# tusen-ai/RangeDet

Measured on AMD Instinct MI355X. Metric: range-image frames/sec (64x2650, 8ch) at 1/2/4/8 GPU; Meta-Kernel HBM GB/s vs peak, higher is better.
Workload: dtype bf16

## Files before the change

rangedet_amd/csrc/k_block.h:

```cpp
#pragma once
#include "k_conv3.h"

namespace rd {

struct BlockArgs {
  const bf16_t* x; int x_cs, x_co; long x_bs;
  const unsigned char* w;
  const float* shift1; const float* shift2;
  const unsigned char* scw;
  bf16_t* y; int y_cs, y_co; long y_bs;
  const unsigned char* zero16;
  int H, W, B, ncol, nrow, ntiles, xcd;
  int nslots1;
};

constexpr int BK_R = 6;
constexpr int BK_XP = 36;
constexpr int BK_XPIECES = 7;
constexpr int BK_BUF = 4 * BK_XPIECES * 1024;
constexpr int BK_TP = 34;
constexpr int BK_SLAB = 4096;
constexpr size_t BK_LDS = 2 * BK_BUF + BK_R * BK_SLAB;

constexpr int bk_nsteps(bool first) { return first ? 23 : 36; }
constexpr int bk_unit(bool first, int g) { return first ? (g < 5 ? 0 : g < 14 ? 2 : 3) : g / 9; }
constexpr int bk_ord(bool first, int g) { return first ? (g < 5 ? g : (g - 5) % 9) : g % 9; }
constexpr bool bk_fetches(bool first, int g) { return bk_unit(first, g) == 3 || (!first && bk_unit(first, g) == 0); }
constexpr int bk_pieces_u(int s) { return s <= 1 ? 2 : s <= 4 ? 1 : 0; }
constexpr int bk_first_u(int s) { int n = 0; for (int t = 0; t < s; ++t) n += bk_pieces_u(t); return n; }
constexpr int bk_pieces(bool first, int g) { return bk_fetches(first, g) ? bk_pieces_u(bk_ord(first, g)) : 0; }
constexpr int bk_younger(bool first, int g) {
  const int G = bk_nsteps(first);
  int n = BK_R - 3;
  for (int d = 1; d <= BK_R - 2; ++d) n += bk_pieces(first, ((g - d) % G + G) % G);
  const int cap = 9 - 3 - 4;
  return (bk_fetches(first, g) && bk_ord(first, g) == 7 && n > cap) ? cap : n;
}

template <int DT, bool SC, bool FIRST = false, bool M16 = false>
__global__ __launch_bounds__(256, 2) void block64_stream_kernel(BlockArgs a) {
  static_assert(!FIRST || SC, "the first block changes the channel count: projection shortcut");
  static_assert(!(FIRST && M16), "the first block (five two-tap steps on one 16-channel slot) stays in the 32 x 32 x 16 form");
  HIP_DYNAMIC_SHARED(unsigned char, smem);
  constexpr int R = BK_R, SLAB = BK_SLAB, RING = 2 * BK_BUF, NCT = 2;
  constexpr int ROWB2 = BK_TP * 64;
  const int tid = threadIdx.x, lane = tid & 63, wave = __builtin_amdgcn_readfirstlane(tid >> 6);
  const int m = lane & 31, hi = lane >> 5;

  unsigned bz1[NCT], bz2[NCT];
#pragma unroll
  for (int j = 0; j < NCT; ++j) {
    const float t1 = a.shift1[32 * j + conv_row_perm(m)], t2 = a.shift2[32 * j + conv_row_perm(m)];
    const bf16_t h1 = H16<DT>::from_f32(t1), h2 = H16<DT>::from_f32(t2);
    const bf16_t l1 = H16<DT>::from_f32(t1 - H16<DT>::to_f32(h1)), l2 = H16<DT>::from_f32(t2 - H16<DT>::to_f32(h2));
    bz1[j] = hi ? 0u : ((unsigned)h1 | ((unsigned)l1 << 16));
    bz2[j] = hi ? 0u : ((unsigned)h2 | ((unsigned)l2 << 16));
  }

  unsigned bz1m = 0u, bz2m = 0u;
  if constexpr (M16) {
    const float t1 = a.shift1[conv_row16(lane >> 4, lane & 15)], t2 = a.shift2[conv_row16(lane >> 4, lane & 15)];
    const bf16_t h1 = H16<DT>::from_f32(t1), h2 = H16<DT>::from_f32(t2);
    const bf16_t l1 = H16<DT>::from_f32(t1 - H16<DT>::to_f32(h1)), l2 = H16<DT>::from_f32(t2 - H16<DT>::to_f32(h2));
    bz1m = (unsigned)h1 | ((unsigned)l1 << 16);
    bz2m = (unsigned)h2 | ((unsigned)l2 << 16);
  }

  const int G = gridDim.x, wg = blockIdx.x;
  const int ntl = (a.ntiles - wg + G - 1) / G;
  const int tiles_img = a.ncol * a.nrow;

#if defined(__HIP_DEVICE_COMPILE__)
  const unsigned lds0 = __builtin_amdgcn_readfirstlane((unsigned)(uintptr_t)(__attribute__((address_space(3))) void*)smem);
#endif
  auto dma_s = [&](const unsigned char* sbase, unsigned voff, int lds_off) {
#if defined(__HIP_DEVICE_COMPILE__)
    asm volatile("s_mov_b32 m0, %2\n\ts_nop 0\n\tglobal_load_lds_dwordx4 %0, %1"
                 :: "v"(voff), "s"(sbase), "s"(__builtin_amdgcn_readfirstlane(lds0 + (unsigned)lds_off)) : "memory");
#else
    __builtin_amdgcn_global_load_lds(sbase + voff, smem + lds_off, 16, 0, 0);
#endif
  };
  auto dma_v = [&](const void* vptr, int lds_off) {
#if defined(__HIP_DEVICE_COMPILE__)
    asm volatile("s_mov_b32 m0, %1\n\ts_nop 0\n\tglobal_load_lds_dwordx4 %0, off"
                 :: "v"(vptr), "s"(__builtin_amdgcn_readfirstlane(lds0 + (unsigned)lds_off)) : "memory");
#else
    __builtin_amdgcn_global_load_lds(vptr, smem + lds_off, 16, 0, 0);
#endif
  };

  const int xdq = (G >> 3) / a.nrow;
  const int g_ct = a.xcd ? (8 * xdq) % a.ncol : G % a.ncol, g_rb = a.xcd ? (G >> 3) % a.nrow : (G / a.ncol) % a.nrow,
            g_b = a.xcd ? (8 * xdq) / a.ncol : G / tiles_img;
  const int g_ct1 = (8 * xdq + 8) % a.ncol, g_b1 = (8 * xdq + 8) / a.ncol;
  auto tile_advance = [&](int& ct, int& rb, int& b) __attribute__((always_inline)) {
    int& d0 = a.xcd ? rb : ct;
    int& d1 = a.xcd ? ct : rb;
    const int r0 = a.xcd ? a.nrow : a.ncol, r1 = a.xcd ? a.ncol : a.nrow;
    d0 += a.xcd ? g_rb : g_ct;
    const int c1 = d0 >= r0 ? 1 : 0;
    d0 -= c1 ? r0 : 0;
    d1 += a.xcd ? (c1 ? g_ct1 : g_ct) : g_rb + c1;
    const int c2 = d1 >= r1 ? 1 : 0;
    d1 -= c2 ? r1 : 0;
    b += (a.xcd && c1 ? g_b1 : g_b) + c2;
  };
  const int xs0 = ((wg >> 3) / a.nrow) * 8 + (wg & 7);
  int f_ct = a.xcd ? xs0 % a.ncol : wg % a.ncol, f_rb = a.xcd ? (wg >> 3) % a.nrow : (wg / a.ncol) % a.nrow,
      f_b = a.xcd ? xs0 / a.ncol : wg / tiles_img;
  int c_ct = f_ct, c_rb = f_rb, c_b = f_b;

  int hk = 0, hc = 0;
  int hh0 = 0, hw0 = 0;
  const unsigned char* htile = nullptr;
  const unsigned char* hbase = nullptr;
  bool hnew = true;
  auto halo_begin = [&]() {
    if (hnew) {
      hh0 = f_rb * 8 - 2; hw0 = f_ct * 32 - 2;
      htile = (const unsigned char*)(a.x + (size_t)f_b * a.x_bs + a.x_co) + ((long)hh0 * a.W + hw0) * (long)a.x_cs * 2;
      hnew = false;
    }
    hbase = htile + hc * 64;
    if (!FIRST && hc == 0) hc = 1;
    else if (hk + 1 < ntl) { ++hk; hc = 0; tile_advance(f_ct, f_rb, f_b); hnew = true; }
  };
  auto halo_piece = [&](int buf, int j) {
    const int q = wave * BK_XPIECES + j;
    int ol = lane;
    asm volatile("" : "+v"(ol));
    const int pp = 16 * q + (ol >> 2), r = (pp * 1821) >> 16, cc = pp - BK_XP * r;
    const int hs = (ol & 3) ^ ((ol >> 4) & 3);
    const bool ok = pp < 12 * BK_XP && (unsigned)(hh0 + r) < (unsigned)a.H && (unsigned)(hw0 + cc) < (unsigned)a.W && (!FIRST || hs < a.nslots1);
    const unsigned char* src = hbase + (long)((r * a.W + cc) * a.x_cs * 2 + hs * 16);
    dma_v(ok ? (const void*)src : (const void*)a.zero16, buf + q * 1024);
  };
  int fslot = 0, fslab = 0;
  auto slab_piece = [&]() { dma_s(a.w + (size_t)fslab * SLAB + wave * 1024, lane * 16, RING + fslot * SLAB + wave * 1024); };
  auto slab_advance = [&]() {
    fslot = fslot + 1 == R ? 0 : fslot + 1;
    fslab = fslab + 1 == bk_nsteps(FIRST) ? 0 : fslab + 1;
  };

  int a1[3][3], a2[3];
#pragma unroll
  for (int dh = 0; dh < 3; ++dh)
#pragma unroll
    for (int dw = 0; dw < 3; ++dw) {
      const int P = 96 * wave + m + BK_XP * dh + dw;
      a1[dh][dw] = P * 64 + (((hi ^ (P >> 2)) & 3) << 4);
    }
#pragma unroll
  for (int d = 0; d < 3; ++d) {
    const int c = d + m;
    a2[d] = c * 64 + (((hi ^ (c >> 2)) & 3) << 4) + wave * 2 * ROWB2;
  }
  if constexpr (M16) {
    const int n16 = lane & 15, q16 = lane >> 4;
#pragma unroll
    for (int dh = 0; dh < 3; ++dh)
#pragma unroll
      for (int dw = 0; dw < 3; ++dw) {
        const int P = 96 * wave + n16 + BK_XP * dh + dw;
        a1[dh][dw] = P * 64 + (((q16 ^ (P >> 2)) & 3) << 4);
      }
#pragma unroll
    for (int d = 0; d < 3; ++d) {
      const int c = d + n16;
      a2[d] = c * 64 + (((q16 ^ (c >> 2)) & 3) << 4) + wave * 2 * ROWB2;
    }
  }
  const int boff = RING + lane * 16;

  f32x16 acc[M16 ? 1 : 3][M16 ? 1 : NCT];
  f32x4 acc6[M16 ? 6 : 1][M16 ? 4 : 1];
  s16x8 fa[2][3], fb[2][NCT];
  s16x8 fa16[6];
#define BK_FENCE() __builtin_amdgcn_sched_barrier(0)
#define BK_RD(F, FS, BUF, K, AADDR, BADDR, KS)                                                              \
  {                                                                                                         \
    if ((K) == 0) fa[BUF][0] = *(const s16x8*)(smem + (AADDR));                                              \
    else if ((K) <= NCT) fb[BUF][(K) - 1] = *(const s16x8*)(smem + (BADDR) + ((KS) * NCT + (K) - 1) * 1024);  \
    else fa[BUF][(K) - NCT] = *(const s16x8*)(smem + (AADDR) + ((K) - NCT) * (FS));                          \
    BK_FENCE();                                                                                             \
  }
#define BK_MM(BUF, N)                                                                                       \
  {                                                                                                         \
    acc[(N) / NCT][(N) % NCT] = H16<DT>::mfma(fb[BUF][(N) % NCT], fa[BUF][(N) / NCT], acc[(N) / NCT][(N) % NCT]); \
    BK_FENCE();                                                                                             \
  }
#define BK_SYNC(VMCNT, LGKM)                                      \
  {                                                               \
    asm volatile("" ::: "memory");                                \
    __builtin_amdgcn_s_waitcnt(C3_WAIT_IMM(VMCNT, LGKM));         \
    __builtin_amdgcn_s_barrier();                                 \
    asm volatile("" ::: "memory");                                \
    BK_FENCE();                                                   \
  }
#define BK_STEP(F, FS, G_, HB_, NF_, NFS_, A1_, ANEXT_)                                                            \
  {                                                                                                                \
    constexpr int NM_ = (F) * NCT, NR_ = (F) + NCT, NRN_ = (NF_) ? (NF_) + NCT : 0;                                \
    constexpr int NH_ = bk_pieces(FIRST, G_), NP_ = 1 + NH_, HF_ = bk_first_u(bk_ord(FIRST, G_)), YG_ = bk_younger(FIRST, G_); \
    const int acur_ = (A1_);                                                                                       \
    const int bcur_ = boff + rslot * SLAB;                                                                         \
    const int rnext_ = rslot + 1 == R ? 0 : rslot + 1;                                                             \
    const int anext_ = (ANEXT_);                                                                                   \
    const int bnext_ = boff + rnext_ * SLAB;                                                                       \
    BK_FENCE();                                                                                                    \
    _Pragma("unroll") for (int n = 0; n < NM_; ++n) {                                                              \
      BK_MM(0, n)                                                                                                  \
      if (n < NR_) BK_RD(F, FS, 1, n, acur_, bcur_, 1)                                                             \
    }                                                                                                              \
    _Pragma("unroll") for (int n = 0; n < NM_ / 2; ++n) {                                                          \
      BK_MM(1, n)                                                                                                  \
      if (n < NRN_) BK_RD(NF_, NFS_, 0, n, anext_, bnext_, 0)                                                      \
    }                                                                                                              \
    { _Pragma("unroll") for (int n = NM_ / 2; n < NRN_; ++n) BK_RD(NF_, NFS_, 0, n, anext_, bnext_, 0) }           \
    BK_SYNC(YG_, NRN_)                                                                                             \
    if (NH_ > 0 && bk_ord(FIRST, G_) == 0) halo_begin();                                                           \
    _Pragma("unroll") for (int n = NM_ / 2; n < NM_; ++n) {                                                        \
      BK_MM(1, n)                                                                                                  \
      _Pragma("unroll") for (int p = 0; p < NP_; ++p)                                                              \
        if (p * (NM_ / 2) / NP_ == n - NM_ / 2) {                                                                  \
          if (p == 0) slab_piece(); else halo_piece(HB_, HF_ + p - 1);                                             \
          BK_FENCE();                                                                                              \
        }                                                                                                          \
    }                                                                                                              \
    slab_advance();                                                                                                \
    rslot = rnext_;                                                                                                \
  }
#define BK_C1(U_, S_)                                                                                              \
  BK_STEP(3, 2048, 9 * (U_) + (S_), BK_BUF, (((U_) == 1 && (S_) == 8) ? 0 : 3), 2048,                              \
          (a1[(S_) / 3][(S_) % 3] + (U_) * BK_BUF) ^ 32,                                                           \
          ((S_) == 8 ? a1[0][0] + BK_BUF : a1[(((S_) + 1) % 9) / 3][((S_) + 1) % 3] + (U_) * BK_BUF))
#define BK_P1(S_)                                                                                                  \
  BK_STEP(3, 2048, (S_), 0, ((S_) == 4 ? 0 : 3), 2048, a1[((2 * (S_) + 1) % 9) / 3][(2 * (S_) + 1) % 3],           \
          a1[((2 * (S_) + 2) % 9) / 3][(2 * (S_) + 2) % 3])
#define BK_C2(C_, S_)                                                                                              \
  BK_STEP(2, ROWB2, (FIRST ? 5 : 18) + 9 * (C_) + (S_), 0, (((C_) == 1 && (S_) == 8) ? 3 : 2), (((C_) == 1 && (S_) == 8) ? 2048 : ROWB2), \
          (a2[(S_) % 3] + ((S_) / 3) * ROWB2 + (C_) * BK_BUF) ^ 32,                                                \
          ((S_) == 8 ? ((C_) == 1 ? a1[0][0] : a2[0] + BK_BUF) : a2[((S_) + 1) % 3] + ((((S_) + 1) % 9) / 3) * ROWB2 + (C_) * BK_BUF))

#define BK_RDW16(BUF, C, BADDR) { fb[BUF][C] = *(const s16x8*)(smem + (BADDR) + (C) * 1024); BK_FENCE(); }
#define BK_RDP16(HX, AADDR, FS) { fa16[HX] = *(const s16x8*)(smem + (AADDR) + ((HX) >> 1) * (FS) + ((HX) & 1) * 1024); BK_FENCE(); }
#define BK_MM16(BK, N)                                                                                             \
  {                                                                                                                \
    acc6[(N) >> 1][2 * (BK) + ((N) & 1)] = H16<DT>::mfma16(fb[BK][(N) & 1], fa16[(N) >> 1], acc6[(N) >> 1][2 * (BK) + ((N) & 1)]); \
    BK_FENCE();                                                                                                    \
  }
#define BK_STEP16(F, G_, HB_, NF_, NFS_, ANEXT_)                                                                   \
  {                                                                                                                \
    constexpr int NM_ = 2 * (F);                                                                                   \
    constexpr int NX_ = (NF_) > (F) ? (NF_) - (F) : 0;                                                             \
    constexpr int LG_ = (NF_) ? 2 + NX_ + ((NF_) < (F) / 2 ? (NF_) : (F) / 2) : 0;                                 \
    constexpr int NH_ = bk_pieces(FIRST, G_), NP_ = 1 + NH_, HF_ = bk_first_u(bk_ord(FIRST, G_)), YG_ = bk_younger(FIRST, G_); \
    const int bcur_ = boff + rslot * SLAB;                                                                         \
    const int rnext_ = rslot + 1 == R ? 0 : rslot + 1;                                                             \
    const int anext_ = (ANEXT_);                                                                                   \
    const int bnext_ = boff + rnext_ * SLAB;                                                                       \
    BK_FENCE();                                                                                                    \
    _Pragma("unroll") for (int n = 0; n < NM_; ++n) {                                                              \
      BK_MM16(0, n)                                                                                                \
      if (n < 2) BK_RDW16(1, n, bcur_ + 2048)                                                                      \
    }                                                                                                              \
    _Pragma("unroll") for (int n = 0; n < NM_ / 2; ++n) {                                                          \
      BK_MM16(1, n)                                                                                                \
      if ((NF_) && n < 2) BK_RDW16(0, n, bnext_)                                                                   \
      if (n < NX_) BK_RDP16((F) + n, anext_, NFS_)                                                                 \
      if ((n & 1) && (n >> 1) < (NF_)) BK_RDP16(n >> 1, anext_, NFS_)                                              \
    }                                                                                                              \
    BK_SYNC(YG_, LG_)                                                                                              \
    if (NH_ > 0 && bk_ord(FIRST, G_) == 0) halo_begin();                                                           \
    _Pragma("unroll") for (int n = NM_ / 2; n < NM_; ++n) {                                                        \
      BK_MM16(1, n)                                                                                                \
      _Pragma("unroll") for (int p = 0; p < NP_; ++p)                                                              \
        if (p * (NM_ / 2) / NP_ == n - NM_ / 2) {                                                                  \
          if (p == 0) slab_piece(); else halo_piece(HB_, HF_ + p - 1);                                             \
          BK_FENCE();                                                                                              \
        }                                                                                                          \
      if ((n & 1) && (n >> 1) < (NF_) && (n >> 1) < (F)) BK_RDP16(n >> 1, anext_, NFS_)                            \
    }                                                                                                              \
    slab_advance();                                                                                                \
    rslot = rnext_;                                                                                                \
  }
#define BK_C1M(U_, S_)                                                                                             \
  BK_STEP16(6, 9 * (U_) + (S_), BK_BUF, (((U_) == 1 && (S_) == 8) ? 0 : 6), 2048,                                  \
            ((S_) == 8 ? a1[0][0] + BK_BUF : a1[(((S_) + 1) % 9) / 3][((S_) + 1) % 3] + (U_) * BK_BUF))
#define BK_C2M(C_, S_)                                                                                             \
  BK_STEP16(4, 18 + 9 * (C_) + (S_), 0, (((C_) == 1 && (S_) == 8) ? 6 : 4), (((C_) == 1 && (S_) == 8) ? 2048 : ROWB2), \
            ((S_) == 8 ? ((C_) == 1 ? a1[0][0] : a2[0] + BK_BUF) : a2[((S_) + 1) % 3] + ((((S_) + 1) % 9) / 3) * ROWB2 + (C_) * BK_BUF))

  halo_begin();
#pragma unroll
  for (int j = 0; j < BK_XPIECES; ++j) halo_piece(0, j);
#pragma unroll 1
  for (int s0 = 0; s0 < R; ++s0) { slab_piece(); slab_advance(); }
  BK_SYNC(0, 0)
  int rslot = 0;
  if constexpr (M16) {
#pragma unroll
    for (int kk = 0; kk < 2; ++kk) BK_RDW16(0, kk, boff + rslot * SLAB)
#pragma unroll
    for (int kk = 0; kk < 6; ++kk) BK_RDP16(kk, a1[0][0], 2048)
  } else {
#pragma unroll
  for (int kk = 0; kk < 3 + NCT; ++kk) BK_RD(3, 2048, 0, kk, a1[0][0], boff + rslot * SLAB, 0)
  }

  for (int k = 0; k < ntl; ++k) {
    if constexpr (M16) {
      unsigned z0 = 0u, b1 = bz1m, b2 = bz2m;
      int oq = lane >> 4;
      asm volatile("" : "+v"(z0), "+v"(b1), "+v"(b2), "+v"(oq));
      typedef short s16x2 __attribute__((ext_vector_type(2)));
      typedef float f32x2 __attribute__((ext_vector_type(2)));
      auto init_acc = [&](unsigned bz, int NH) {
#pragma unroll
        for (int cb = 0; cb < 4; ++cb) {
          unsigned ob[4] = {oq == cb ? H16<DT>::ONE * 0x10001u : z0, z0, z0, z0};
          unsigned ab[4] = {bz, z0, z0, z0};
          s16x8 ones, bzv;
          memcpy(&ones, ob, 16);
          memcpy(&bzv, ab, 16);
          acc6[0][cb] = H16<DT>::mfma16(bzv, ones, f32x4{});
          BK_FENCE();
        }
#pragma unroll
        for (int h = 1; h < 6; ++h)
          if (h < NH) {
#pragma unroll
            for (int cb = 0; cb < 4; ++cb) acc6[h][cb] = acc6[0][cb];
          }
        BK_FENCE();
      };
      init_acc(b1, 6);
      BK_C1M(0, 0) BK_C1M(0, 1) BK_C1M(0, 2) BK_C1M(0, 3) BK_C1M(0, 4) BK_C1M(0, 5) BK_C1M(0, 6) BK_C1M(0, 7) BK_C1M(0, 8)
      BK_C1M(1, 0) BK_C1M(1, 1) BK_C1M(1, 2) BK_C1M(1, 3) BK_C1M(1, 4) BK_C1M(1, 5) BK_C1M(1, 6) BK_C1M(1, 7) BK_C1M(1, 8)
      const int ct = c_ct, rb = c_rb, b = c_b;
      tile_advance(c_ct, c_rb, c_b);
      {
        int el = lane;
        asm volatile("" : "+v"(el));
        const int en = el & 15, eq = el >> 4;
#pragma unroll
        for (int h = 0; h < 6; ++h) {
          const int J = 96 * wave + 16 * h + en, rr = (J * 1821) >> 16, cc = J - BK_XP * rr;
          const bool keep = cc < BK_TP && rr < 10;
          const bool inside = (unsigned)(rb * 8 - 1 + rr) < (unsigned)a.H && (unsigned)(ct * 32 - 1 + cc) < (unsigned)a.W;
          const int doff = (rr * BK_TP + cc) * 64 + (((eq ^ (cc >> 2)) & 3) << 4);
#pragma unroll
          for (int j = 0; j < 2; ++j) {
            BK_FENCE();
            unsigned pk[4];
#pragma unroll
            for (int w2 = 0; w2 < 4; ++w2) {
              const f32x4 av = acc6[h][2 * j + (w2 >> 1)];
              unsigned p2 = H16<DT>::pk(av[2 * (w2 & 1)], av[2 * (w2 & 1) + 1]);
              p2 = __builtin_bit_cast(unsigned, __builtin_elementwise_max(__builtin_bit_cast(s16x2, p2), (s16x2){0, 0}));
              pk[w2] = inside ? p2 : 0u;
            }
            if (keep) *(Slot16*)(smem + j * BK_BUF + doff) = Slot16{pk[0], pk[1], pk[2], pk[3]};
          }
        }
      }
      init_acc(b2, 4);
      BK_SYNC(63, 0)
#pragma unroll
      for (int kk = 0; kk < 2; ++kk) BK_RDW16(0, kk, boff + rslot * SLAB)
#pragma unroll
      for (int kk = 0; kk < 4; ++kk) BK_RDP16(kk, a2[0], ROWB2)
      BK_C2M(0, 0) BK_C2M(0, 1) BK_C2M(0, 2) BK_C2M(0, 3) BK_C2M(0, 4) BK_C2M(0, 5) BK_C2M(0, 6) BK_C2M(0, 7) BK_C2M(0, 8)
      BK_C2M(1, 0) BK_C2M(1, 1) BK_C2M(1, 2) BK_C2M(1, 3) BK_C2M(1, 4) BK_C2M(1, 5) BK_C2M(1, 6) BK_C2M(1, 7) BK_C2M(1, 8)
      {
        const int oh0 = rb * 8 + 2 * wave;
        int el = lane;
        asm volatile("" : "+v"(el));
        const int en = el & 15, eq = el >> 4;
        unsigned char* scr = smem + BK_BUF + wave * (BK_BUF / 4);
        bf16_t* __restrict__ yrow0 = a.y + (size_t)b * a.y_bs + (size_t)oh0 * a.W * a.y_cs + a.y_co;
        const bf16_t* __restrict__ rimg0 = a.x + (size_t)b * a.x_bs + a.x_co;
        if constexpr (SC) {
          const unsigned char* __restrict__ wq = a.scw + el * 16;
          s16x8 sxq[4][2];
#pragma unroll
          for (int h = 0; h < 4; ++h) {
            const int ow = ct * 32 + 16 * (h & 1) + en, oh = oh0 + (h >> 1);
            const bool live = ow < a.W && oh < a.H;
            const bf16_t* sp = rimg0 + (live ? ((size_t)oh * a.W + ow) * a.x_cs : 0) + 8 * eq;
#pragma unroll
            for (int ks = 0; ks < 2; ++ks) sxq[h][ks] = *(const s16x8*)(sp + 32 * ks);
          }
#pragma unroll
          for (int ks = 0; ks < 2; ++ks)
#pragma unroll
            for (int cb = 0; cb < 4; ++cb) {
              const s16x8 wf = *(const s16x8*)(wq + (size_t)(ks * 4 + cb) * 1024);
#pragma unroll
              for (int h = 0; h < 4; ++h) acc6[h][cb] = H16<DT>::mfma16(wf, sxq[h][ks], acc6[h][cb]);
            }
          BK_FENCE();
        }
        Slot16 rv[2][2][2];
        auto res_load = [&](int i, Slot16 (&dst)[2][2]) {
#pragma unroll
          for (int hf = 0; hf < 2; ++hf) {
            const int ow = ct * 32 + 16 * hf + en, oh = oh0 + i;
            const bool live = ow < a.W && oh < a.H;
            const bf16_t* rp = rimg0 + (live ? ((size_t)oh * a.W + (size_t)ow) * a.x_cs : 0) + 8 * eq;
#pragma unroll
            for (int p2 = 0; p2 < 2; ++p2) dst[hf][p2] = *(const Slot16*)(rp + 32 * p2);
          }
        };
        if constexpr (!SC) res_load(0, rv[0]);
#pragma unroll
        for (int i = 0; i < 2; ++i) {
          if constexpr (!SC) { if (i + 1 < 2) res_load(i + 1, rv[(i + 1) & 1]); }
#pragma unroll
          for (int hf = 0; hf < 2; ++hf)
#pragma unroll
            for (int p2 = 0; p2 < 2; ++p2) {
              BK_FENCE();
              unsigned pk[4];
#pragma unroll
              for (int w2 = 0; w2 < 4; ++w2) {
                const f32x4 av = acc6[2 * i + hf][2 * p2 + (w2 >> 1)];
                f32x2 v = {av[2 * (w2 & 1)], av[2 * (w2 & 1) + 1]};
                if constexpr (!SC) v += H16<DT>::unpk(rv[i & 1][hf][p2][w2]);
                const unsigned q2 = H16<DT>::pk(v[0], v[1]);
                pk[w2] = __builtin_bit_cast(unsigned, __builtin_elementwise_max(__builtin_bit_cast(s16x2, q2), (s16x2){0, 0}));
              }
              const int px = 16 * hf + en;
              *(Slot16*)(scr + px * 128 + (((4 * p2 + eq) ^ (px & 7)) << 4)) = Slot16{pk[0], pk[1], pk[2], pk[3]};
            }
          BK_FENCE();
          __builtin_amdgcn_wave_barrier();
#pragma unroll
          for (int it = 0; it < 4; ++it) {
            const int pr = it * 8 + el / 8, sl = el % 8;
            const Slot16 v = *(const Slot16*)(scr + pr * 128 + ((sl ^ (pr & 7)) << 4));
            const int ows = ct * 32 + pr;
            if (ows < a.W && oh0 + i < a.H)
              __builtin_nontemporal_store(v, (Slot16*)(yrow0 + (size_t)i * a.W * a.y_cs + (size_t)ows * a.y_cs + sl * 8));
          }
          __builtin_amdgcn_wave_barrier();
          BK_FENCE();
        }
      }
    } else {
    unsigned z0 = 0u;
    asm volatile("" : "+v"(z0));
    const unsigned one2 = hi ? z0 : H16<DT>::ONE * 0x10001u;
    s16x8 ones;
    {
      unsigned ob[4] = {one2, z0, z0, z0};
      memcpy(&ones, ob, 16);
    }
#pragma unroll
    for (int n = 0; n < 3 * NCT; ++n) {
      unsigned ab[4] = {bz1[n % NCT], z0, z0, z0};
      s16x8 bz;
      memcpy(&bz, ab, 16);
      acc[n / NCT][n % NCT] = H16<DT>::mfma(bz, ones, f32x16{});
    }
    BK_FENCE();
    if constexpr (FIRST) {
      BK_P1(0) BK_P1(1) BK_P1(2) BK_P1(3) BK_P1(4)
    } else {
      BK_C1(0, 0) BK_C1(0, 1) BK_C1(0, 2) BK_C1(0, 3) BK_C1(0, 4) BK_C1(0, 5) BK_C1(0, 6) BK_C1(0, 7) BK_C1(0, 8)
      BK_C1(1, 0) BK_C1(1, 1) BK_C1(1, 2) BK_C1(1, 3) BK_C1(1, 4) BK_C1(1, 5) BK_C1(1, 6) BK_C1(1, 7) BK_C1(1, 8)
    }

    const int ct = c_ct, rb = c_rb, b = c_b;
    tile_advance(c_ct, c_rb, c_b);
    {
      int em = m, ehi = hi;
      asm volatile("" : "+v"(em), "+v"(ehi));
      typedef short s16x2 __attribute__((ext_vector_type(2)));
#pragma unroll
      for (int i = 0; i < 3; ++i) {
        const int J = 96 * wave + 32 * i + em, rr = (J * 1821) >> 16, cc = J - BK_XP * rr;
        const bool keep = cc < BK_TP && rr < 10;
        const bool inside = (unsigned)(rb * 8 - 1 + rr) < (unsigned)a.H && (unsigned)(ct * 32 - 1 + cc) < (unsigned)a.W;
        const int doff = (rr * BK_TP + cc) * 64 + ((((2 * ehi) ^ (cc >> 2)) & 3) << 4);
#pragma unroll
        for (int j = 0; j < NCT; ++j) {
          BK_FENCE();
          unsigned pk[8];
#pragma unroll
          for (int q = 0; q < 8; ++q) {
            unsigned p2 = H16<DT>::pk(acc[i][j][2 * q], acc[i][j][2 * q + 1]);
            p2 = __builtin_bit_cast(unsigned, __builtin_elementwise_max(__builtin_bit_cast(s16x2, p2), (s16x2){0, 0}));
            pk[q] = inside ? p2 : 0u;
          }
          if (keep) {
            *(Slot16*)(smem + j * BK_BUF + doff) = Slot16{pk[0], pk[1], pk[2], pk[3]};
            *(Slot16*)(smem + j * BK_BUF + (doff ^ 16)) = Slot16{pk[4], pk[5], pk[6], pk[7]};
          }
        }
      }
    }
#pragma unroll
    for (int n = 0; n < 2 * NCT; ++n) {
      unsigned ab[4] = {bz2[n % NCT], z0, z0, z0};
      s16x8 bz;
      memcpy(&bz, ab, 16);
      acc[n / NCT][n % NCT] = H16<DT>::mfma(bz, ones, f32x16{});
    }
    BK_FENCE();
    BK_SYNC(63, 0)
#pragma unroll
    for (int kk = 0; kk < 2 + NCT; ++kk) BK_RD(2, ROWB2, 0, kk, a2[0], boff + rslot * SLAB, 0)
    BK_C2(0, 0) BK_C2(0, 1) BK_C2(0, 2) BK_C2(0, 3) BK_C2(0, 4) BK_C2(0, 5) BK_C2(0, 6) BK_C2(0, 7) BK_C2(0, 8)
    BK_C2(1, 0) BK_C2(1, 1) BK_C2(1, 2) BK_C2(1, 3) BK_C2(1, 4) BK_C2(1, 5) BK_C2(1, 6) BK_C2(1, 7) BK_C2(1, 8)

    {
      const int oh0 = rb * 8 + 2 * wave;
      int em = m, ehi = hi, el = lane;
      asm volatile("" : "+v"(em), "+v"(ehi), "+v"(el));
      typedef float f32x2 __attribute__((ext_vector_type(2)));
      typedef short s16x2 __attribute__((ext_vector_type(2)));
      unsigned char* scr = smem + BK_BUF + wave * (BK_BUF / 4);
      bf16_t* __restrict__ yrow0 = a.y + (size_t)b * a.y_bs + (size_t)oh0 * a.W * a.y_cs + a.y_co;
      const bf16_t* __restrict__ rimg0 = a.x + (size_t)b * a.x_bs + a.x_co;
      if constexpr (SC) {
        const bf16_t* __restrict__ sb = a.x + (size_t)b * a.x_bs + a.x_co + 8 * ehi;
        const unsigned char* __restrict__ wq = a.scw + el * 16;
        constexpr int SNK = FIRST ? 1 : 4;
        s16x8 sxq[2][SNK];
#pragma unroll
        for (int i = 0; i < 2; ++i) {
          const int ow = ct * 32 + em, oh = oh0 + i;
          const bool live = ow < a.W && oh < a.H;
          const bf16_t* sp = sb + (live ? ((size_t)oh * a.W + ow) * a.x_cs : 0);
#pragma unroll
          for (int ks = 0; ks < SNK; ++ks) sxq[i][ks] = *(const s16x8*)(sp + 16 * ks);
        }
#pragma unroll
        for (int ks = 0; ks < SNK; ++ks)
#pragma unroll
          for (int j = 0; j < NCT; ++j) {
            const s16x8 wf = *(const s16x8*)(wq + (size_t)(ks * NCT + j) * 1024);
#pragma unroll
            for (int i = 0; i < 2; ++i) acc[i][j] = H16<DT>::mfma(wf, sxq[i][ks], acc[i][j]);
          }
        BK_FENCE();
      }
      Slot16 rv[2][NCT][2];
      auto res_load = [&](int i, Slot16 (&dst)[NCT][2]) {
        const int ow = ct * 32 + em, oh = oh0 + i;
        const bool live = ow < a.W && oh < a.H;
        const bf16_t* rp = rimg0 + (live ? ((size_t)oh * a.W + (size_t)ow) * a.x_cs : 0) + 16 * ehi;
#pragma unroll
        for (int j = 0; j < NCT; ++j) {
          dst[j][0] = *(const Slot16*)(rp + j * 32);
          dst[j][1] = *(const Slot16*)(rp + j * 32 + 8);
        }
      };
      if constexpr (!SC) res_load(0, rv[0]);
#pragma unroll
      for (int i = 0; i < 2; ++i) {
        if constexpr (!SC) { if (i + 1 < 2) res_load(i + 1, rv[(i + 1) & 1]); }
#pragma unroll
        for (int j = 0; j < NCT; ++j) {
          BK_FENCE();
          const int cb = j * 32 + 16 * ehi;
          unsigned pk[8];
#pragma unroll
          for (int q = 0; q < 8; ++q) {
            f32x2 v = {acc[i][j][2 * q], acc[i][j][2 * q + 1]};
            if constexpr (!SC) v += H16<DT>::unpk(rv[i & 1][j][q >> 2][q & 3]);
            unsigned p2 = H16<DT>::pk(v[0], v[1]);
            pk[q] = __builtin_bit_cast(unsigned, __builtin_elementwise_max(__builtin_bit_cast(s16x2, p2), (s16x2){0, 0}));
          }
#pragma unroll
          for (int u = 0; u < 2; ++u)
            *(Slot16*)(scr + em * 128 + ((((cb >> 3) + u) ^ (em & 7)) << 4)) = Slot16{pk[4 * u], pk[4 * u + 1], pk[4 * u + 2], pk[4 * u + 3]};
        }
        BK_FENCE();
        __builtin_amdgcn_wave_barrier();
#pragma unroll
        for (int it = 0; it < 4; ++it) {
          const int pr = it * 8 + el / 8, sl = el % 8;
          const Slot16 v = *(const Slot16*)(scr + pr * 128 + ((sl ^ (pr & 7)) << 4));
          const int ows = ct * 32 + pr;
          if (ows < a.W && oh0 + i < a.H)
            __builtin_nontemporal_store(v, (Slot16*)(yrow0 + (size_t)i * a.W * a.y_cs + (size_t)ows * a.y_cs + sl * 8));
        }
        __builtin_amdgcn_wave_barrier();
        BK_FENCE();
      }
    }
    }
  }
  __builtin_amdgcn_s_waitcnt(RD_VMCNT_IMM(0));
#undef BK_C2M
#undef BK_C1M
#undef BK_STEP16
#undef BK_MM16
#undef BK_RDP16
#undef BK_RDW16
#undef BK_C2
#undef BK_P1
#undef BK_C1
#undef BK_STEP
#undef BK_SYNC
#undef BK_MM
#undef BK_RD
#undef BK_FENCE
}

inline bool block64_first(int cin) { return cin <= 16; }
inline size_t block64_body_bytes(int cin) { return (size_t)bk_nsteps(block64_first(cin)) * BK_SLAB; }
inline size_t block64_packed_bytes(int cin) { return block64_body_bytes(cin) + RD_CONV_TAIL; }
inline void pack_block64_m16(const float* w1, const float* s1, const float* w2, const float* s2, int dt, void* out) {
  memset(out, 0, block64_packed_bytes(64));
  pack_taps_frag16(9, 64, 64, out, [&](int co, int ci, int t) { return (s1 ? s1[co] : 1.f) * w1[((size_t)co * 64 + ci) * 9 + t]; }, dt);
  pack_taps_frag16(9, 64, 64, (unsigned char*)out + 18 * BK_SLAB, [&](int co, int ci, int t) { return (s2 ? s2[co] : 1.f) * w2[((size_t)co * 64 + ci) * 9 + t]; }, dt);
}
inline void pack_sc_frag16(const float* w, const float* scale, void* out, int dt = RD_BF16) {
  bf16_t* o = (bf16_t*)out;
  for (int ks = 0; ks < 2; ++ks)
    for (int cb = 0; cb < 4; ++cb)
      for (int lane = 0; lane < 64; ++lane) {
        const int co = conv_row16(cb, lane & 15);
        for (int j = 0; j < 8; ++j) {
          const int ci = 32 * ks + 8 * (lane >> 4) + j;
          *o++ = h16_from_f32(dt, (scale ? scale[co] : 1.f) * w[(size_t)co * 64 + ci]);
        }
      }
}
inline void pack_block64(const float* w1, const float* s1, const float* w2, const float* s2, int cin, int dt, void* out) {
  memset(out, 0, block64_packed_bytes(cin));
  if (block64_first(cin))
    pack_body_frag(3, cin, 64, out, [&](int co, int ci, int dh, int dw) { return (s1 ? s1[co] : 1.f) * w1[(((size_t)co * cin + ci) * 3 + dh) * 3 + dw]; }, dt);
  else
    pack_taps_frag(9, 64, 64, out, [&](int co, int ci, int t) { return (s1 ? s1[co] : 1.f) * w1[((size_t)co * 64 + ci) * 9 + t]; }, dt);
  pack_taps_frag(9, 64, 64, (unsigned char*)out + block64_body_bytes(cin) - 18 * BK_SLAB,
                 [&](int co, int ci, int t) { return (s2 ? s2[co] : 1.f) * w2[((size_t)co * 64 + ci) * 9 + t]; }, dt);
}

inline int launch_block64(const void* x, int x_cs, int x_co, int cin, const void* w, const float* shift1, const float* shift2, const void* sc_w,
                          void* y, int y_cs, int y_co, int B, int H, int W, int dt, hipStream_t st, bool m16 = false) {
  RD_REQUIRE(is_h16(dt), RD_EINVAL, "block64: dtype %d (RD_BF16 or RD_F16)", dt);
  const bool first = block64_first(cin);
  RD_REQUIRE(!m16 || !first, RD_ESHAPE, "block64: the 16 x 16 x 32 form takes 64 input channels");
  RD_REQUIRE(cin == 64 || (first && cin >= 1), RD_ESHAPE, "block64: %d input channels (64, or at most 16 for the network's first block)", cin);
  RD_REQUIRE(!first || sc_w, RD_EINVAL, "block64: a block that changes the channel count needs its projection shortcut");
  BlockArgs a;
  memset(&a, 0, sizeof(a));
  a.x = (const bf16_t*)x; a.x_cs = x_cs; a.x_co = x_co; a.x_bs = (long)H * W * x_cs;
  a.w = (const unsigned char*)w; a.shift1 = shift1; a.shift2 = shift2; a.scw = (const unsigned char*)sc_w;
  a.y = (bf16_t*)y; a.y_cs = y_cs; a.y_co = y_co; a.y_bs = (long)H * W * y_cs;
  a.zero16 = (const unsigned char*)w + block64_body_bytes(cin);
  a.H = H; a.W = W; a.B = B;
  a.nslots1 = std::min(2, (x_cs - x_co) / 8);
  a.ncol = (W + 31) / 32; a.nrow = (H + 7) / 8; a.ntiles = a.ncol * a.nrow * B;
  const int grid = std::min(a.ntiles, conv_num_cus() * 2);
  a.xcd = dev_switches().conv_xcd && (a.ncol * B) % 8 == 0 && grid % 8 == 0;
  ProfScope ps(RD_PROF_BLOCK, st);
  static std::atomic<unsigned long long> seen{0};
  once_per_device(seen, [] {
    allow_big_lds(block64_stream_kernel<RD_F16, false>); allow_big_lds(block64_stream_kernel<RD_BF16, false>);
    allow_big_lds(block64_stream_kernel<RD_F16, true>); allow_big_lds(block64_stream_kernel<RD_BF16, true>);
    allow_big_lds(block64_stream_kernel<RD_F16, true, true>); allow_big_lds(block64_stream_kernel<RD_BF16, true, true>);
    allow_big_lds(block64_stream_kernel<RD_F16, false, false, true>); allow_big_lds(block64_stream_kernel<RD_BF16, false, false, true>);
    allow_big_lds(block64_stream_kernel<RD_F16, true, false, true>); allow_big_lds(block64_stream_kernel<RD_BF16, true, false, true>);
  });
#define BK_GO(DT_)                                                                                                         \
  {                                                                                                                        \
    if (m16 && sc_w) hipLaunchKernelGGL((block64_stream_kernel<DT_, true, false, true>), dim3(grid), dim3(256), BK_LDS, st, a);  \
    else if (m16) hipLaunchKernelGGL((block64_stream_kernel<DT_, false, false, true>), dim3(grid), dim3(256), BK_LDS, st, a);    \
    else if (first) hipLaunchKernelGGL((block64_stream_kernel<DT_, true, true>), dim3(grid), dim3(256), BK_LDS, st, a);    \
    else if (sc_w) hipLaunchKernelGGL((block64_stream_kernel<DT_, true>), dim3(grid), dim3(256), BK_LDS, st, a);           \
    else hipLaunchKernelGGL((block64_stream_kernel<DT_, false>), dim3(grid), dim3(256), BK_LDS, st, a);                    \
  }
  if (dt == RD_F16) BK_GO(RD_F16) else BK_GO(RD_BF16)
#undef BK_GO
  return check_launch("block64_stream_kernel");
}

}
```

rangedet_amd/csrc/k_conv3.h:

```cpp
#pragma once
#include "k_conv.h"

namespace rd {

struct Conv3Args {
  const bf16_t* x; int x_cs, x_co; long x_bs;
  const unsigned char* w;
  const float* scale; const float* shift;
  const bf16_t* res; int r_cs, r_co; long r_bs;
  bf16_t* y; int y_cs, y_co; long y_bs;
  const unsigned char* zero16;
  int H, W, B, nslots, nchunk, flags, ncol, nrow, ntiles;
  int sw, Wo;
  int xcd;
  unsigned long long* trace;
  const unsigned char* hw;
  const float* hb;
  float* ho; long ho_bs, ho_off; int hn;
  const bf16_t* sx; int s_cs, s_co; long s_bs;
  const unsigned char* scw;
  int s_nks;
  int ngrp;
  long g_x, g_res, g_y, g_w, g_shift, g_hw, g_hb, g_ho, g_ho_bs;
  int g_hn;
  int nph, ts_mask, y_pc, r_pc;
  long w_pb;
  const bf16_t* x2; int x2_cs, x2_co, nchunk1, nslots2; long x2_bs;
};

enum C3Tile { C3_8x62 = 0, C3_8x32 = 1 };
template <int NCT, C3Tile TILE = C3_8x62> struct C3Cfg {
  static constexpr bool WIDE = TILE == C3_8x32;
  static constexpr int RW = 2;
  static constexpr int FC = WIDE ? 1 : 2;
  static constexpr int FPW = RW * FC;
  static constexpr int TH = 4 * RW;
  static constexpr int COLS = WIDE ? 34 : 64;
  static constexpr int TW = WIDE ? 32 : 62;
  static constexpr int ROWB = COLS * 64;
  static constexpr int HROWS = TH + 2;
  static constexpr int NPX = HROWS * COLS;
  static constexpr int HPW = (NPX + 63) / 64;
  static constexpr int HALO = HPW * 4096;
  static constexpr int R = WIDE ? (NCT == 4 ? 4 : 8) : (NCT == 4 ? 7 : 10);
  static constexpr int IPW = NCT / 2;
  static constexpr int SLAB = NCT * 2048;
  static constexpr size_t LDS = 2 * (size_t)HALO + (size_t)R * SLAB + (WIDE ? 0 : 2 * NCT * 32 * sizeof(float));
};

template <class F>
inline void pack_taps_frag(int ntaps, int cin, int cout, void* out, F get, int dt = RD_BF16) {
  const int nchunk = (cin + 31) / 32, ncb = cout / 32;
  bf16_t* o = (bf16_t*)out;
  for (int c = 0; c < nchunk; ++c)
    for (int t = 0; t < ntaps; ++t)
      for (int ks = 0; ks < 2; ++ks)
        for (int cb = 0; cb < ncb; ++cb)
          for (int lane = 0; lane < 64; ++lane) {
            const int co = cb * 32 + conv_row_perm(lane & 31);
            for (int j = 0; j < 8; ++j) {
              const int ci = c * 32 + ks * 16 + (lane >> 5) * 8 + j;
              *o++ = h16_from_f32(dt, ci < cin ? get(co, ci, t) : 0.f);
            }
          }
}

__host__ __device__ inline int conv_row16(int cb, int mm) { return 32 * (cb >> 1) + 8 * (mm >> 2) + 4 * (cb & 1) + (mm & 3); }
template <class F>
inline void pack_taps_frag16(int ntaps, int cin, int cout, void* out, F get, int dt = RD_BF16) {
  const int nchunk = (cin + 31) / 32, ncb = cout / 16;
  bf16_t* o = (bf16_t*)out;
  for (int c = 0; c < nchunk; ++c)
    for (int t = 0; t < ntaps; ++t)
      for (int cb = 0; cb < ncb; ++cb)
        for (int lane = 0; lane < 64; ++lane) {
          const int co = conv_row16(cb, lane & 15);
          for (int j = 0; j < 8; ++j) {
            const int ci = c * 32 + (lane >> 4) * 8 + j;
            *o++ = h16_from_f32(dt, ci < cin ? get(co, ci, t) : 0.f);
          }
        }
}

inline void pack_head_frag(const float* w, int nout, int cin, void* out, int dt = RD_BF16) {
  bf16_t* o = (bf16_t*)out;
  for (int part = 0; part < 2; ++part)
    for (int ks = 0; ks < 8; ++ks)
      for (int lane = 0; lane < 64; ++lane)
        for (int j = 0; j < 8; ++j) {
          const int mm = lane & 31, c = 16 * ks + 8 * (lane >> 5) + j;
          const float v = (mm < nout && c < cin) ? w[(size_t)mm * cin + c] : 0.f;
          const bf16_t h = h16_from_f32(dt, v);
          *o++ = part == 0 ? h : h16_from_f32(dt, v - h16_to_f32(dt, h));
        }
}

inline void pack_head_frag16(const float* w, int nout, int cin, void* out, int dt = RD_BF16) {
  bf16_t* o = (bf16_t*)out;
  for (int part = 0; part < 2; ++part)
    for (int p = 0; p < 4; ++p)
      for (int lane = 0; lane < 64; ++lane)
        for (int j = 0; j < 8; ++j) {
          const int mm = lane & 15, c = 32 * p + 8 * (lane >> 4) + j;
          const float v = (mm < nout && c < cin) ? w[(size_t)mm * cin + c] : 0.f;
          const bf16_t h = h16_from_f32(dt, v);
          *o++ = part == 0 ? h : h16_from_f32(dt, v - h16_to_f32(dt, h));
        }
}

inline size_t sc_frag_bytes(int cin, int cout) { return (size_t)((cin + 15) / 16) * (cout / 32) * 1024; }
inline void pack_sc_frag(const float* w, const float* scale, int cin, int cout, void* out, int dt = RD_BF16) {
  bf16_t* o = (bf16_t*)out;
  const int nks = (cin + 15) / 16;
  for (int ks = 0; ks < nks; ++ks)
    for (int cb = 0; cb < cout / 32; ++cb)
      for (int lane = 0; lane < 64; ++lane) {
        const int co = cb * 32 + conv_row_perm(lane & 31);
        for (int j = 0; j < 8; ++j) {
          const int ci = ks * 16 + (lane >> 5) * 8 + j;
          *o++ = h16_from_f32(dt, ci < cin ? (scale ? scale[co] : 1.f) * w[(size_t)co * cin + ci] : 0.f);
        }
      }
}

constexpr int c3_nsteps(int TS) { return TS == 0 ? 9 : 6; }
constexpr int c3_tap(int TS, int s) {
  return TS == 0 ? s : 3 * (s / 2) + (s % 2) + (TS == 2 ? 1 : 0);
}
constexpr int c3_halo_last(int NS) { return NS == 9 ? 4 : 2; }
constexpr int c3_halo_pieces(int s, int NS, C3Tile tile) {
  return tile == C3_8x32 ? (NS == 9 ? (s == 0 ? 2 : s <= 4 ? 1 : 0) : (s <= 2 ? 2 : 0))
                         : (NS == 9 ? (s <= 4 ? 2 : 0) : (s <= 1 ? 4 : (s == 2 ? 2 : 0)));
}
constexpr int c3_halo_first(int s, int NS, C3Tile tile) { int n = 0; for (int t = 0; t < s; ++t) n += c3_halo_pieces(t, NS, tile); return n; }
constexpr int c3_younger(int R, int IPW, int s, int NS, C3Tile tile) {
  int n = (R - 3) * IPW;
  for (int d = 1; d <= R - 2; ++d) n += c3_halo_pieces((((s - d) % NS) + NS) % NS, NS, tile);
  const int cap = (NS - 3 - c3_halo_last(NS)) * IPW;
  if (s == NS - 2 && n > cap) n = cap;
  return n;
}
constexpr int C3_BODY_M16 = 16;
enum { UK_T9 = 0, UK_T6A = 1, UK_T6B = 2, UK_T6R = 3, UK_T3 = 4, UK_P5 = 5 };
constexpr int uk_nsteps(int k) { return k == UK_T9 ? 9 : k == UK_T3 ? 3 : k == UK_P5 ? 5 : 6; }
struct C3KStep { int dh, dw, slot; };
constexpr C3KStep uk_kstep(int k, int s, int ks) {
  if (k == UK_P5) { const int t = 2 * s + ks > 8 ? 8 : 2 * s + ks; return C3KStep{t / 3, t % 3, 0}; }
  const int T = k == UK_T9 ? s : k == UK_T3 ? 3 * s + 1 : 3 * (s / 2) + (s % 2) + (k == UK_T6B ? 1 : 0);
  return C3KStep{T / 3, T % 3, ks};
}
struct C3Body { int nu; int kind[4]; };
constexpr C3Body c3_body(int BODY) {
  return BODY == 1 ? C3Body{4, {UK_T6A, UK_T3, UK_T3, UK_T6A}} : BODY == 2 ? C3Body{3, {UK_T9, UK_T9, UK_P5, 0}} : C3Body{1, {UK_P5, 0, 0, 0}};
}
constexpr int c3b_steps(int BODY) { int n = 0; for (int u = 0; u < c3_body(BODY).nu; ++u) n += uk_nsteps(c3_body(BODY).kind[u]); return n; }
constexpr int c3b_unit(int BODY, int g) { int u = 0; while (g >= uk_nsteps(c3_body(BODY).kind[u])) { g -= uk_nsteps(c3_body(BODY).kind[u]); ++u; } return u; }
constexpr int c3b_ord(int BODY, int g) { int u = 0; while (g >= uk_nsteps(c3_body(BODY).kind[u])) { g -= uk_nsteps(c3_body(BODY).kind[u]); ++u; } return g; }
constexpr int uk_halo_pieces(int NS, int s) {
  return NS == 9 ? (s == 0 ? 2 : s <= 4 ? 1 : 0) : NS == 6 ? (s <= 2 ? 2 : 0) : NS == 5 ? (s <= 1 ? 3 : 0) : (s == 0 ? 6 : 0);
}
constexpr int uk_halo_last(int NS) { return NS == 9 ? 4 : NS == 6 ? 2 : NS == 5 ? 1 : 0; }
constexpr int c3b_pieces(int BODY, int g) { return uk_halo_pieces(uk_nsteps(c3_body(BODY).kind[c3b_unit(BODY, g)]), c3b_ord(BODY, g)); }
constexpr int c3b_first(int BODY, int g) { int n = 0; for (int t = g - c3b_ord(BODY, g); t < g; ++t) n += c3b_pieces(BODY, t); return n; }
constexpr int c3b_younger(int BODY, int R, int IPW, int g) {
  const int G = c3b_steps(BODY);
  int n = (R - 3) * IPW;
  for (int d = 1; d <= R - 2; ++d) n += c3b_pieces(BODY, ((g - d) % G + G) % G);
  const int NS = uk_nsteps(c3_body(BODY).kind[c3b_unit(BODY, g)]), s = c3b_ord(BODY, g);
  const int cap = (NS - 3 - uk_halo_last(NS)) * IPW;
  return (s == NS - 2 && n > cap) ? cap : n;
}
__host__ __device__ inline int c3b_chunk(int BODY, int i, int nchunk) {
  if (BODY != 1) return i;
  const int r2 = (i >> 2) * 2, j = i & 3, ne = nchunk >> 1;
  return j == 0 ? ne + r2 : j == 1 ? r2 : j == 2 ? r2 + 1 : ne + r2 + 1;
}
template <class F>
inline void pack_body_frag(int BODY, int cin, int cout, void* out, F get, int dt = RD_BF16) {
  const C3Body bd = c3_body(BODY);
  const int nchunk = (cin + 31) / 32, ncb = cout / 32;
  bf16_t* o = (bf16_t*)out;
  for (int i = 0; i < nchunk; ++i) {
    const int kind = bd.kind[i % bd.nu], chunk = c3b_chunk(BODY, i, nchunk);
    for (int s = 0; s < uk_nsteps(kind); ++s)
      for (int ks = 0; ks < 2; ++ks) {
        const C3KStep k = uk_kstep(kind, s, ks);
        const bool zero_tap = kind == UK_P5 && 2 * s + ks > 8;
        for (int cb = 0; cb < ncb; ++cb)
          for (int lane = 0; lane < 64; ++lane) {
            const int co = cb * 32 + conv_row_perm(lane & 31);
            for (int j = 0; j < 8; ++j) {
              const int ci = chunk * 32 + k.slot * 16 + (lane >> 5) * 8 + j;
              *o++ = h16_from_f32(dt, (ci < cin && !zero_tap) ? get(co, ci, k.dh, k.dw) : 0.f);
            }
          }
      }
  }
}
inline bool conv3_bodies_on() { return dev_switches().conv_body && !dev_switches().conv_v1; }
inline int conv3_body_s2(int cin, int x_cstride, bool folded) { return folded && conv3_bodies_on() && x_cstride % 64 == 0 && cin == x_cstride ? 1 : 0; }
inline int conv3_body_small(int cin, bool folded) { return folded && conv3_bodies_on() && cin <= 16 ? 3 : 0; }
inline int conv3_body_cat(int cin1, int cin2, bool folded) { return folded && conv3_bodies_on() && cin1 == 64 && cin2 <= 16 ? 2 : 0; }
#define C3_WAIT_IMM(vm, lgkm) (((vm) & 15) | (((vm) >> 4) << 14) | (7 << 4) | ((lgkm) << 8))

template <int NCT, int DBG = 0, int TS = 0, bool HEAD = false, bool SC = false, bool FOLD = false, C3Tile TILE = C3_8x62,
          int DT = RD_BF16, bool GRP = false, int BODY = 0, bool M16 = false>
__global__ __launch_bounds__(256, (TILE == C3_8x32 ? 2 : 1)) void conv3x3_stream_kernel(Conv3Args a) {
  using Cfg = C3Cfg<NCT, TILE>;
  constexpr bool WD = Cfg::WIDE;
  constexpr int FPW = Cfg::FPW, FC = Cfg::FC;
  static_assert(!M16 || (NCT == 4 && WD && FOLD && !SC && !GRP && TS == 0 && BODY == 0 && DBG == 0),
                "16 x 16 x 32 form: cout 128 on the 8 x 32 tiles, folded scales, all nine taps");
  static_assert(BODY == 0 || (WD && FOLD && !GRP && !HEAD && (TS == 0 || TS == 1)), "heterogeneous tile bodies: 8 x 32 tiles, folded scales");
  static_assert(!GRP || (WD && FOLD && !SC), "two problems per launch: 8 x 32 tiles (output-conv weights from L2), folded scales, no shortcut");
  static_assert(!WD || FOLD, "8 x 32 tile: no room for the scale / shift array");
  static_assert(!HEAD || (NCT == 4 && TS == 0), "fused output conv: cout 128, all nine taps");
  constexpr bool PH = TS == 3;
  static_assert(!PH || (FOLD && !SC && !HEAD && !GRP), "all-phase transposed conv: folded scales, no shortcut / output conv / second problem");
  static_assert(!(HEAD && SC), "a head tower has no shortcut");
  constexpr int R = Cfg::R, IPW = Cfg::IPW, SLAB = Cfg::SLAB, COUT = NCT * 32;
  constexpr int C3_HALO = Cfg::HALO, C3_HPW = Cfg::HPW, C3_TH = Cfg::TH;
  constexpr int C3_TW = Cfg::TW, C3_ROWB = Cfg::ROWB, RW = Cfg::RW;
  constexpr int NR = FPW + NCT;
  constexpr int NM = FPW * NCT;
  constexpr int NS = c3_nsteps(TS);
  constexpr int BG = BODY ? c3b_steps(BODY) : NS;
  constexpr int BNU = BODY ? c3_body(BODY).nu : 1;
  HIP_DYNAMIC_SHARED(unsigned char, smem);
  const int tid = threadIdx.x, lane = tid & 63, wave = __builtin_amdgcn_readfirstlane(tid >> 6);
  const int m = lane & 31, hi = lane >> 5;
  constexpr int RING = 2 * C3_HALO;
  auto hflip = [](int a_) { return C3_HALO - a_; };
  float* Sc = (float*)(smem + RING + R * SLAB);
  constexpr int HWOFF = RING + R * SLAB + 2 * COUT * (int)sizeof(float);
  if (!WD && tid < COUT) {
    Sc[tid] = a.scale ? a.scale[tid] : 1.f;
    Sc[COUT + tid] = a.shift ? a.shift[tid] : 0.f;
  }
  unsigned bzw[NCT];
  auto load_shift = [&](const float* shp) {
#pragma unroll
    for (int j = 0; j < NCT; ++j) {
      const float t = shp ? shp[32 * j + conv_row_perm(m)] : 0.f;
      const bf16_t th = H16<DT>::from_f32(t);
      const bf16_t tl = H16<DT>::from_f32(t - H16<DT>::to_f32(th));
      bzw[j] = hi ? 0u : ((unsigned)th | ((unsigned)tl << 16));
    }
  };
  if constexpr (FOLD && !GRP && !M16) load_shift(a.shift);
  unsigned bzw1[GRP ? NCT : 1];
  if constexpr (GRP) {
    load_shift(a.shift ? a.shift + a.g_shift : nullptr);
#pragma unroll
    for (int j = 0; j < NCT; ++j) bzw1[j] = bzw[j];
    load_shift(a.shift);
  }
  unsigned bzw16[M16 ? 2 : 1];
  if constexpr (M16) {
#pragma unroll
    for (int g = 0; g < 2; ++g) {
      const float t = a.shift ? a.shift[conv_row16(4 * g + (lane >> 4), lane & 15)] : 0.f;
      const bf16_t th = H16<DT>::from_f32(t);
      const bf16_t tl = H16<DT>::from_f32(t - H16<DT>::to_f32(th));
      bzw16[g] = (unsigned)th | ((unsigned)tl << 16);
    }
  }
  int tpt = 0;
#define C3_TRACE() { if (a.trace && tid == 0 && tpt < 7) a.trace[(size_t)blockIdx.x * 8 + tpt++] = wall_clock64(); }
  C3_TRACE()
  const unsigned long long clk0 = __builtin_readcyclecounter();

  const int G = gridDim.x, wg = blockIdx.x;
  const int nph = PH ? a.nph : 1;
  const int ntl = ((a.ntiles - wg + G - 1) / G) * nph;
  const int tiles_img = a.ncol * a.nrow;

#if defined(__HIP_DEVICE_COMPILE__)
  const unsigned lds0 = __builtin_amdgcn_readfirstlane((unsigned)(uintptr_t)(__attribute__((address_space(3))) void*)smem);
#endif
  auto dma_s = [&](const unsigned char* sbase, unsigned voff, int lds_off) {
#if defined(__HIP_DEVICE_COMPILE__)
    asm volatile("s_mov_b32 m0, %2\n\ts_nop 0\n\tglobal_load_lds_dwordx4 %0, %1"
                 :: "v"(voff), "s"(sbase), "s"(__builtin_amdgcn_readfirstlane(lds0 + (unsigned)lds_off)) : "memory");
#else
    __builtin_amdgcn_global_load_lds(sbase + voff, smem + lds_off, 16, 0, 0);
#endif
  };
  auto dma_v = [&](const void* vptr, int lds_off) {
#if defined(__HIP_DEVICE_COMPILE__)
    asm volatile("s_mov_b32 m0, %1\n\ts_nop 0\n\tglobal_load_lds_dwordx4 %0, off"
                 :: "v"(vptr), "s"(__builtin_amdgcn_readfirstlane(lds0 + (unsigned)lds_off)) : "memory");
#else
    __builtin_amdgcn_global_load_lds(vptr, smem + lds_off, 16, 0, 0);
#endif
  };
  const int hs = (lane & 3) ^ ((lane >> 4) & 3);
  const int l4 = lane >> 2;
  const unsigned hlane = (unsigned)(l4 * a.x_cs + hs * 8) * 2;
  int hk = 0, hc = 0;
  int hh0 = 0, hlo = 0, hlim = 0;
  const unsigned char* hbase = nullptr;
  bool hsok = false;
  int hcur = 0;
  const int xdq = (G >> 3) / a.nrow;
  const int g_ct = a.xcd ? (8 * xdq) % a.ncol : G % a.ncol, g_rb = a.xcd ? (G >> 3) % a.nrow : (G / a.ncol) % a.nrow,
            g_b = a.xcd ? (8 * xdq) / a.ncol : G / tiles_img;
  const int g_ct1 = (8 * xdq + 8) % a.ncol, g_b1 = (8 * xdq + 8) / a.ncol;
  auto tile_advance = [&](int& ct, int& rb, int& b) __attribute__((always_inline)) {
    int& d0 = a.xcd ? rb : ct;
    int& d1 = a.xcd ? ct : rb;
    const int r0 = a.xcd ? a.nrow : a.ncol, r1 = a.xcd ? a.ncol : a.nrow;
    d0 += a.xcd ? g_rb : g_ct;
    const int c1 = d0 >= r0 ? 1 : 0;
    d0 -= c1 ? r0 : 0;
    d1 += a.xcd ? (c1 ? g_ct1 : g_ct) : g_rb + c1;
    const int c2 = d1 >= r1 ? 1 : 0;
    d1 -= c2 ? r1 : 0;
    b += (a.xcd && c1 ? g_b1 : g_b) + c2;
  };
  const int xs0 = ((wg >> 3) / a.nrow) * 8 + (wg & 7);
  int f_ct = a.xcd ? xs0 % a.ncol : wg % a.ncol, f_rb = a.xcd ? (wg >> 3) % a.nrow : (wg / a.ncol) % a.nrow,
      f_b = a.xcd ? xs0 / a.ncol : wg / tiles_img;
  int c_ct = f_ct, c_rb = f_rb, c_b = f_b;
  int f_ph = 0, c_ph = 0, s_ph = 0;
  const unsigned char* htile = nullptr;
  const unsigned char* htile2 = nullptr;
  int hpxb = a.x_cs * 2, hns = 0;
  auto halo_tile = [&]() {
    const int hw0 = f_ct * C3_TW - 1;
    hh0 = f_rb * C3_TH - 1;
    hlo = hw0 < 0 ? -hw0 : 0;
    hlim = a.W - hw0;
    const bool fg = GRP && f_b >= a.B;
    htile = (const unsigned char*)(a.x + (size_t)(fg ? f_b - a.B : f_b) * a.x_bs + a.x_co + (fg ? a.g_x : 0)) +
            ((long)hh0 * a.W + hw0) * (long)a.x_cs * 2;
    if constexpr (WD) {
      if (a.x2) htile2 = (const unsigned char*)(a.x2 + (size_t)f_b * a.x2_bs + a.x2_co) + ((long)hh0 * a.W + hw0) * (long)a.x2_cs * 2;
    }
  };
  bool hnew = true;
  auto halo_begin = [&]() {
    if (hnew) { halo_tile(); hnew = false; }
    const int hcm = c3b_chunk(BODY, hc, a.nchunk);
    hbase = htile + hcm * 64;
    hsok = hcm * 4 + hs < a.nslots;
    hcur = hcm;
    if constexpr (WD) {
      hpxb = a.x_cs * 2; hns = a.nslots - 4 * hcm;
      if (a.x2 && hcm >= a.nchunk1) { hbase = htile2 + (hcm - a.nchunk1) * 64; hpxb = a.x2_cs * 2; hns = a.nslots2 - 4 * (hcm - a.nchunk1); }
    }
    if (hc + 1 < a.nchunk) ++hc;
    else if (hk + 1 < ntl) {
      ++hk; hc = 0;
      if constexpr (PH) {
        if (++f_ph == nph) { f_ph = 0; tile_advance(f_ct, f_rb, f_b); hnew = true; }
      } else { tile_advance(f_ct, f_rb, f_b); hnew = true; }
    }
  };
  auto halo_piece = [&](int buf, int j) {
    const int q = wave * C3_HPW + j;
    bool ok;
    const unsigned char* src;
    if constexpr (WD) {
      int ol = lane;
      asm volatile("" : "+v"(ol));
      const int pp = 16 * q + (ol >> 2), r = (pp * 1928) >> 16, cc = pp - 34 * r;
      const int hsp = (ol & 3) ^ ((cc >> 2) & 3);
      ok = hsp < hns && (unsigned)(hh0 + r) < (unsigned)a.H && cc >= hlo && cc < hlim && pp < Cfg::NPX && !(DBG & 16);
      src = hbase + (long)((r * a.W + cc) * hpxb + hsp * 16);
    } else {
    const int r = q >> 2, c16 = (q & 3) * 16;
    const int cc = c16 + l4;
    ok = hsok && (unsigned)(hh0 + r) < (unsigned)a.H && cc >= hlo && cc < hlim && !(DBG & 16);
    const unsigned char* sp = hbase + ((long)r * a.W + c16) * (long)a.x_cs * 2;
    src = sp + hlane;
    }
    if constexpr ((DBG & 256) != 0)
      src = (const unsigned char*)a.x + ((size_t)(src - (const unsigned char*)a.x) & 0xFFFF0);
    dma_v(ok ? (const void*)src : (const void*)a.zero16, buf + q * 1024);
  };
  int fslot = 0, fslab = 0;
  const int nslab_tile = BODY ? (a.nchunk / BNU) * BG : a.nchunk * NS;
  const int t0_ = tiles_img * a.B;
  const int n0 = GRP ? (wg < t0_ ? (t0_ - wg + G - 1) / G : 0) : 0;
  int stile = 0;
  const unsigned char* wsrc = a.w + (GRP && n0 == 0 ? a.g_w : 0);
  auto slab_piece = [&](int j) {
    dma_s(wsrc + (size_t)fslab * SLAB + (wave * IPW + j) * 1024, lane * 16, RING + fslot * SLAB + (wave * IPW + j) * 1024);
  };
  auto slab_advance = [&]() {
    fslot = fslot + 1 == R ? 0 : fslot + 1;
    fslab = fslab + 1 == nslab_tile ? 0 : fslab + 1;
    if constexpr (GRP) {
      if (fslab == 0) {
        ++stile;
        wsrc = a.w + (stile >= n0 ? a.g_w : 0);
      }
    }
    if constexpr (PH) {
      if (fslab == 0) {
        s_ph = s_ph + 1 == nph ? 0 : s_ph + 1;
        wsrc = a.w + (size_t)s_ph * a.w_pb;
      }
    }
  };

  int aoff[3];
#pragma unroll
  for (int d = 0; d < 3; ++d) {
    const int c = d + m;
    aoff[d] = c * 64 + (((hi ^ (c >> 2)) & 3) << 4) + wave * RW * C3_ROWB;
    if constexpr (M16) {
      const int c16 = d + (lane & 15);
      aoff[d] = c16 * 64 + ((((lane >> 4) ^ (c16 >> 2)) & 3) << 4) + wave * RW * C3_ROWB;
    }
  }
  const int boff = RING + lane * 16;
  auto side2 = [&](int ph) { return (a.ts_mask >> ph) & 1; };
  int pcol[2] = {aoff[0], aoff[1]}, pq0 = aoff[0];
  if constexpr (PH) {
    const int s0_ = side2(0), s1_ = side2(nph > 1 ? 1 : 0);
    pcol[0] = s0_ ? aoff[1] : aoff[0]; pcol[1] = s0_ ? aoff[2] : aoff[1];
    pq0 = s1_ ? aoff[1] : aoff[0];
  }
  bool lastc = false;
#define C3_AO(D) (PH ? pcol[(D)] : aoff[(D)])

  f32x16 acc[M16 ? 1 : FPW][M16 ? 1 : NCT];
  f32x4 acc6[M16 ? 4 : 1][M16 ? 8 : 1];
  s16x8 fa[2][FPW], fb[2][NCT];
  s16x8 fa16[4];
#define C3_FENCE() __builtin_amdgcn_sched_barrier(0)
#define C3_RD(BUF, K, AADDR, BADDR, KS)                                                                   \
  {                                                                                                       \
    if ((K) == 0) fa[BUF][0] = *(const s16x8*)(smem + (AADDR));                                            \
    else if ((K) <= NCT) fb[BUF][(K) - 1] = *(const s16x8*)(smem + (BADDR) + ((KS) * NCT + (K) - 1) * 1024); \
    else fa[BUF][(K) - NCT] = *(const s16x8*)(smem + (AADDR) + (((K) - NCT) / FC) * C3_ROWB + (((K) - NCT) % FC) * 2048); \
    C3_FENCE();                                                                                           \
  }
#define C3_MM(BUF, N)                                                                                     \
  {                                                                                                       \
    if (!(DBG & 8))                                                                                       \
      acc[(N) / NCT][(N) % NCT] = H16<DT>::mfma(fb[BUF][(N) % NCT], fa[BUF][(N) / NCT], \
                                                                          acc[(N) / NCT][(N) % NCT]);    \
    C3_FENCE();                                                                                           \
  }
#define C3_MMZ(BUF, N)                                                                                    \
  {                                                                                                       \
    if (!(DBG & 8))                                                                                       \
      acc[(N) / NCT][(N) % NCT] = H16<DT>::mfma(fb[BUF][(N) % NCT], fa[BUF][(N) / NCT], \
                                                                          f32x16{});             \
    C3_FENCE();                                                                                           \
  }
#define C3_RDW16(BUF, C, BADDR) { fb[BUF][C] = *(const s16x8*)(smem + (BADDR) + (C) * 1024); C3_FENCE(); }
#define C3_RDP16(HX, AADDR) { fa16[HX] = *(const s16x8*)(smem + (AADDR) + ((HX) >> 1) * C3_ROWB + ((HX) & 1) * 1024); C3_FENCE(); }
#define C3_MM16(BK, N)                                                                                                   \
  {                                                                                                                      \
    acc6[(N) >> 2][4 * (BK) + ((N) & 3)] = H16<DT>::mfma16(fb[BK][(N) & 3], fa16[(N) >> 2], acc6[(N) >> 2][4 * (BK) + ((N) & 3)]); \
    C3_FENCE();                                                                                                          \
  }
#define C3_SYNC(VMCNT, LGKM)                                      \
  {                                                               \
    asm volatile("" ::: "memory");                                \
    __builtin_amdgcn_s_waitcnt(C3_WAIT_IMM((DBG & 32) ? 63 : (VMCNT), LGKM)); \
    if (!(DBG & 2)) __builtin_amdgcn_s_barrier();                 \
    asm volatile("" ::: "memory");                                \
    C3_FENCE();                                                   \
  }

  halo_begin();
#pragma unroll
  for (int j = 0; j < C3_HPW; ++j) halo_piece(0, j);
  if constexpr (HEAD && !WD) {
#pragma unroll
    for (int j = 0; j < 4; ++j) dma_s(a.hw + (wave * 4 + j) * 1024, lane * 16, HWOFF + (wave * 4 + j) * 1024);
  }
#pragma unroll 1
  for (int s0 = 0; s0 < R; ++s0) {
#pragma unroll
    for (int j = 0; j < IPW; ++j) slab_piece(j);
    slab_advance();
  }
  C3_SYNC(0, 0)
  C3_TRACE()
  constexpr C3KStep K00 = BODY ? uk_kstep(c3_body(BODY ? BODY : 3).kind[0], 0, 0) : C3KStep{c3_tap(TS, 0) / 3, c3_tap(TS, 0) % 3, 0};
  constexpr int K00DW = K00.dw, K00DH = K00.dh;
  int rslot = 0;
  int abuf = 0;
  if constexpr (M16) {
#pragma unroll
    for (int k = 0; k < 4; ++k) C3_RDW16(0, k, boff + rslot * SLAB)
#pragma unroll
    for (int k = 0; k < 4; ++k) C3_RDP16(k, aoff[K00DW] + abuf + K00DH * C3_ROWB)
  } else {
#pragma unroll
  for (int k = 0; k < NR; ++k)
    C3_RD(0, k, C3_AO(K00DW) + abuf + K00DH * C3_ROWB, boff + rslot * SLAB, 0)
  }

#define C3_STEP(S) C3_STEP_(S, C3_MM)
#define C3_STEP_(S, MM0)                                                                                             \
  {                                                                                                                  \
    constexpr int T_ = c3_tap(TS, (S)), TN_ = c3_tap(TS, ((S) + 1) % NS);                                            \
    constexpr int dh_ = T_ / 3, dw_ = T_ % 3, ndh_ = TN_ / 3, ndw_ = TN_ % 3;                                        \
    constexpr int NH_ = c3_halo_pieces((S), NS, TILE), NP_ = IPW + NH_;                       \
    const int acur_ = (C3_AO(dw_) + abuf + dh_ * C3_ROWB) ^ 32;                                                        \
    const int bcur_ = boff + rslot * SLAB;                                                                           \
    const int rnext_ = rslot + 1 == R ? 0 : rslot + 1;                                                               \
    const int anext_ = ((S) == NS - 1 && PH && lastc ? pq0 : C3_AO(ndw_)) + ((S) == NS - 1 ? hflip(abuf) : abuf) + ndh_ * C3_ROWB; \
    const int bnext_ = boff + rnext_ * SLAB;                                                                         \
    const int hbuf_ = hflip(abuf);                                                    \
    C3_FENCE();                                                                                                      \
    _Pragma("unroll") for (int n = 0; n < NM; ++n) {                                                                 \
      MM0(0, n)                                                                                                      \
      if (n < NR) C3_RD(1, n, acur_, bcur_, 1)                                                                       \
    }                                                                                                                \
    _Pragma("unroll") for (int n = 0; n < NM / 2; ++n) {                                                             \
      C3_MM(1, n)                                                                                                    \
      if (n < NR) C3_RD(0, n, anext_, bnext_, 0)                                                                     \
    }                                                                                                                \
    if (NR > NM / 2) { _Pragma("unroll") for (int n = NM / 2; n < NR; ++n) C3_RD(0, n, anext_, bnext_, 0) }          \
    C3_SYNC(c3_younger(R, IPW, (S), NS, TILE), NR)                                                            \
    if ((S) == 0) halo_begin();                                                                                      \
    _Pragma("unroll") for (int n = NM / 2; n < NM; ++n) {                                                            \
      C3_MM(1, n)                                                                                                    \
      if (!(DBG & 4)) {    \
        _Pragma("unroll") for (int p = 0; p < NP_; ++p)                                                              \
          if (p * (NM / 2) / NP_ == n - NM / 2) {                                                                    \
            if (p < IPW) slab_piece(p); else halo_piece(hbuf_, c3_halo_first((S), NS, TILE) + p - IPW);                    \
            C3_FENCE();                                                                                              \
          }                                                                                                          \
      }                                                                                                              \
    }                                                                                                                \
    slab_advance();                                                                                                  \
    rslot = rnext_;                                                                                                  \
  }

#define C3_STEP16(S)                                                                                                 \
  {                                                                                                                  \
    constexpr int TN_ = c3_tap(TS, ((S) + 1) % NS), ndh_ = TN_ / 3, ndw_ = TN_ % 3;                                  \
    constexpr int NH_ = c3_halo_pieces((S), NS, TILE), NP_ = IPW + NH_;                                               \
    const int bcur_ = boff + rslot * SLAB;                                                                           \
    const int rnext_ = rslot + 1 == R ? 0 : rslot + 1;                                                               \
    const int anext_ = aoff[ndw_] + ((S) == NS - 1 ? hflip(abuf) : abuf) + ndh_ * C3_ROWB;                           \
    const int bnext_ = boff + rnext_ * SLAB;                                                                         \
    const int hbuf_ = hflip(abuf);                                                                                   \
    C3_FENCE();                                                                                                      \
    _Pragma("unroll") for (int n = 0; n < 16; ++n) {                                                                 \
      C3_MM16(0, n)                                                                                                  \
      if (n < 4) C3_RDW16(1, n, bcur_ + 4096)                                                                        \
    }                                                                                                                \
    _Pragma("unroll") for (int n = 0; n < 8; ++n) {                                                                  \
      C3_MM16(1, n)                                                                                                  \
      if (n < 4) C3_RDW16(0, n, bnext_)                                                                              \
      if (n == 3) C3_RDP16(0, anext_)                                                                                \
      if (n == 7) C3_RDP16(1, anext_)                                                                                \
    }                                                                                                                \
    C3_SYNC(c3_younger(R, IPW, (S), NS, TILE), 6)                                                                \
    if ((S) == 0) halo_begin();                                                                                      \
    _Pragma("unroll") for (int n = 8; n < 16; ++n) {                                                                 \
      C3_MM16(1, n)                                                                                                  \
      _Pragma("unroll") for (int p = 0; p < NP_; ++p)                                                                \
        if (p * 8 / NP_ == n - 8) {                                                                                  \
          if (p < IPW) slab_piece(p); else halo_piece(hbuf_, c3_halo_first((S), NS, TILE) + p - IPW);                 \
          C3_FENCE();                                                                                                \
        }                                                                                                            \
      if (n == 11) C3_RDP16(2, anext_)                                                                               \
      if (n == 15) C3_RDP16(3, anext_)                                                                               \
    }                                                                                                                \
    slab_advance();                                                                                                  \
    rslot = rnext_;                                                                                                  \
  }

#define C3_GSTEP(G_, MM0)                                                                                            \
  if constexpr (BODY != 0 && (G_) < BG) {                                                                            \
    constexpr int U_ = c3b_unit(BODY, (G_)), S_ = c3b_ord(BODY, (G_)), K_ = c3_body(BODY).kind[U_], NSU_ = uk_nsteps(K_); \
    constexpr int GN_ = ((G_) + 1) % BG, KN_ = c3_body(BODY).kind[c3b_unit(BODY, GN_)];                              \
    constexpr C3KStep k1_ = uk_kstep(K_, S_, 1), kn_ = uk_kstep(KN_, c3b_ord(BODY, GN_), 0);                         \
    constexpr bool lastS_ = S_ == NSU_ - 1;                                                                          \
    constexpr int NH_ = c3b_pieces(BODY, (G_)), NP_ = IPW + NH_, HF_ = c3b_first(BODY, (G_)), YG_ = c3b_younger(BODY, R, IPW, (G_)); \
    const int acur_ = (aoff[k1_.dw] + abuf + k1_.dh * C3_ROWB) ^ (k1_.slot << 5);                                    \
    const int bcur_ = boff + rslot * SLAB;                                                                           \
    const int rnext_ = rslot + 1 == R ? 0 : rslot + 1;                                                               \
    const int anext_ = (aoff[kn_.dw] + (lastS_ ? hflip(abuf) : abuf) + kn_.dh * C3_ROWB) ^ (kn_.slot << 5);          \
    const int bnext_ = boff + rnext_ * SLAB;                                                                         \
    const int hbuf_ = hflip(abuf);                                                                                   \
    C3_FENCE();                                                                                                      \
    _Pragma("unroll") for (int n = 0; n < NM; ++n) {                                                                 \
      MM0(0, n)                                                                                                      \
      if (n < NR) C3_RDX(1, n, acur_, bcur_, 1)                                                                      \
    }                                                                                                                \
    _Pragma("unroll") for (int n = 0; n < NM / 2; ++n) {                                                             \
      C3_MM(1, n)                                                                                                    \
      if (n < NR) C3_RDX(0, n, anext_, bnext_, 0)                                                                    \
    }                                                                                                                \
    if (NR > NM / 2) { _Pragma("unroll") for (int n = NM / 2; n < NR; ++n) C3_RDX(0, n, anext_, bnext_, 0) }         \
    C3_SYNC(YG_, NR)                                                                                                 \
    if (S_ == 0) halo_begin();                                                                                       \
    _Pragma("unroll") for (int n = NM / 2; n < NM; ++n) {                                                            \
      C3_MM(1, n)                                                                                                    \
      _Pragma("unroll") for (int p = 0; p < NP_; ++p)                                                                \
        if (p * (NM / 2) / NP_ == n - NM / 2) {                                                                      \
          if (p < IPW) slab_piece(p); else halo_piece(hbuf_, HF_ + p - IPW);                                         \
          C3_FENCE();                                                                                                \
        }                                                                                                            \
    }                                                                                                                \
    slab_advance();                                                                                                  \
    rslot = rnext_;                                                                                                  \
    if (lastS_) abuf = hflip(abuf);                                                                                  \
  }
#define C3_RDX(BUF, K, AADDR, BADDR, KS) C3_RD(BUF, K, AADDR, BADDR, KS)
#define C3_GBODY_FROM1(MM) C3_GSTEP(1, MM) C3_GSTEP(2, MM) C3_GSTEP(3, MM) C3_GSTEP(4, MM) C3_GSTEP(5, MM) C3_GSTEP(6, MM) C3_GSTEP(7, MM) \
  C3_GSTEP(8, MM) C3_GSTEP(9, MM) C3_GSTEP(10, MM) C3_GSTEP(11, MM) C3_GSTEP(12, MM) C3_GSTEP(13, MM) C3_GSTEP(14, MM) C3_GSTEP(15, MM)      \
  C3_GSTEP(16, MM) C3_GSTEP(17, MM) C3_GSTEP(18, MM) C3_GSTEP(19, MM) C3_GSTEP(20, MM) C3_GSTEP(21, MM) C3_GSTEP(22, MM)
  static_assert(BG <= 23, "C3_GBODY_FROM1 unrolls 23 steps");

  for (int k = 0; k < ntl; ++k) {
    if constexpr (PH) lastc = a.nchunk == 1;
    if constexpr (M16) {
      unsigned z0 = 0u;
      asm volatile("" : "+v"(z0));
      int oq = lane >> 4;
      asm volatile("" : "+v"(oq));
      unsigned bq2[2] = {bzw16[0], bzw16[1]};
      asm volatile("" : "+v"(bq2[0]), "+v"(bq2[1]));
#pragma unroll
      for (int cb = 0; cb < 8; ++cb) {
        unsigned ob[4] = {oq == (cb & 3) ? H16<DT>::ONE * 0x10001u : z0, z0, z0, z0};
        unsigned ab[4] = {bq2[cb >> 2], z0, z0, z0};
        s16x8 ones, bz;
        memcpy(&ones, ob, 16);
        memcpy(&bz, ab, 16);
        acc6[0][cb] = H16<DT>::mfma16(bz, ones, f32x4{});
        C3_FENCE();
      }
#pragma unroll
      for (int h = 1; h < 4; ++h)
#pragma unroll
        for (int cb = 0; cb < 8; ++cb) acc6[h][cb] = acc6[0][cb];
      C3_FENCE();
#pragma unroll 1
      for (int c = 0; c < a.nchunk; ++c) {
        C3_STEP16(0) C3_STEP16(1) C3_STEP16(2) C3_STEP16(3) C3_STEP16(4) C3_STEP16(5) C3_STEP16(6) C3_STEP16(7) C3_STEP16(8)
        abuf = hflip(abuf);
      }
    } else {
    {
      if constexpr (FOLD) {
        unsigned z0 = 0u;
        asm volatile("" : "+v"(z0));
        const unsigned one2 = hi ? z0 : H16<DT>::ONE * 0x10001u;
        unsigned ob[4] = {one2, z0, z0, z0};
        s16x8 ones;
        memcpy(&ones, ob, 16);
#pragma unroll
        for (int n = 0; n < NM; ++n) {
          unsigned ab[4] = {GRP && k >= n0 ? bzw1[GRP ? n % NCT : 0] : bzw[n % NCT], z0, z0, z0};
          s16x8 bz;
          memcpy(&bz, ab, 16);
          acc[n / NCT][n % NCT] = H16<DT>::mfma(bz, ones, f32x16{});
        }
        C3_FENCE();
        if constexpr (BODY != 0) { C3_GSTEP(0, C3_MM) } else {
        C3_STEP(0)
        }
      } else {
        C3_STEP_(0, C3_MMZ)
      }
      if constexpr (BODY != 0) { C3_GBODY_FROM1(C3_MM) } else {
      C3_STEP(1) C3_STEP(2) C3_STEP(3) C3_STEP(4) C3_STEP(5)
      if constexpr (NS == 9) { C3_STEP(6) C3_STEP(7) C3_STEP(8) }
      abuf = hflip(abuf);
      }
    }
    if constexpr (BODY != 0) {
#pragma unroll 1
      for (int c = BNU; c < a.nchunk; c += BNU) { C3_GSTEP(0, C3_MM) C3_GBODY_FROM1(C3_MM) }
    } else {
#pragma unroll 1
    for (int c = 1; c < a.nchunk; ++c) {
      if constexpr (PH) lastc = c == a.nchunk - 1;
      C3_STEP(0) C3_STEP(1) C3_STEP(2) C3_STEP(3) C3_STEP(4) C3_STEP(5)
      if constexpr (NS == 9) { C3_STEP(6) C3_STEP(7) C3_STEP(8) }
      abuf = hflip(abuf);
    }
    }
    }
    if (k == 0) C3_TRACE()

    const int ct = c_ct, rb = c_rb;
    const bool eg = GRP && c_b >= a.B;
    const int b = eg ? c_b - a.B : c_b;
    const int e_ph = c_ph;
    if constexpr (PH) {
      if (++c_ph == nph) { c_ph = 0; tile_advance(c_ct, c_rb, c_b); }
      const int sn_ = side2(c_ph), sq_ = side2(c_ph + 1 == nph ? 0 : c_ph + 1);
      pcol[0] = sn_ ? aoff[1] : aoff[0]; pcol[1] = sn_ ? aoff[2] : aoff[1];
      pq0 = sq_ ? aoff[1] : aoff[0];
    } else
    tile_advance(c_ct, c_rb, c_b);
    const int oh0 = rb * C3_TH + RW * wave;
    int em = m, ehi = hi, el = lane;
    if constexpr (M16) {
      asm volatile("" : "+v"(el));
      em = el & 31; ehi = el >> 5;
    } else
    asm volatile("" : "+v"(em), "+v"(ehi), "+v"(el));
    constexpr int JW = (32 * COUT * 2 <= C3_HALO / 4) ? NCT : NCT / 2, CW = JW * 32, NPASS = NCT / JW;
    static_assert(32 * CW * 2 <= C3_HALO / 4, "transpose scratch");
    constexpr int ROWB = CW * 2, SPR = CW / 8, RPI = 64 / SPR;
    unsigned char* scr = smem + hflip(abuf) + wave * (C3_HALO / 4);
    bf16_t* __restrict__ yrow0 = a.y + (eg ? a.g_y : 0) + (size_t)b * a.y_bs + (size_t)oh0 * a.Wo * a.y_cs + a.y_co + (PH ? e_ph * a.y_pc : 0);
    const bf16_t* __restrict__ rimg0 = a.res + (eg ? a.g_res : 0) + (size_t)b * a.r_bs + a.r_co + (PH ? e_ph * a.r_pc : 0);
    const unsigned char* __restrict__ e_hw = a.hw + (eg ? a.g_hw : 0);
    const float* __restrict__ e_hb = a.hb + (eg ? a.g_hb : 0);
    float* __restrict__ e_ho = a.ho + (eg ? a.g_ho : 0);
    const long e_ho_bs = a.ho_bs + (eg ? a.g_ho_bs : 0);
    const int e_hn = a.hn + (eg ? a.g_hn : 0);
    const int sh = a.sw - 1;
    if constexpr (SC) {
      const bf16_t* __restrict__ sb = a.sx + (size_t)b * a.s_bs + a.s_co + 8 * ehi;
      const unsigned char* __restrict__ wq = a.scw + el * 16;
      auto shortcut = [&](auto MKc) {
        constexpr int MK = decltype(MKc)::value;
#pragma unroll
        for (int kh = 0; kh < 8 / MK; ++kh) {
          if (kh * MK < a.s_nks) {
            s16x8 sxq[FPW][MK];
#pragma unroll
            for (int i = 0; i < FPW; ++i) {
              const int tc = 32 * (i % FC) + em, ow = ct * C3_TW + tc, oh = oh0 + i / FC;
              const bool live = tc < C3_TW && ow < a.W && oh < a.H;
              const bf16_t* sp = sb + (live ? ((size_t)oh * a.W + ow) * a.s_cs : 0) + 16 * MK * kh;
#pragma unroll
              for (int ks = 0; ks < MK; ++ks)
                if (kh * MK + ks < a.s_nks) sxq[i][ks] = *(const s16x8*)(sp + 16 * ks);
            }
#pragma unroll
            for (int ks = 0; ks < MK; ++ks)
              if (kh * MK + ks < a.s_nks) {
#pragma unroll
                for (int j = 0; j < NCT; ++j) {
                  const s16x8 wf = *(const s16x8*)(wq + (size_t)((kh * MK + ks) * NCT + j) * 1024);
#pragma unroll
                  for (int i = 0; i < FPW; ++i)
                    acc[i][j] = H16<DT>::mfma(wf, sxq[i][ks], acc[i][j]);
                }
              }
          }
          C3_FENCE();
        }
      };
      shortcut(std::integral_constant<int, 4>{});
      C3_FENCE();
    }
    auto epilogue = [&](auto FL) {
      constexpr int F = decltype(FL)::value;
      const bool relu_pre = F >= 0 ? (F & RD_RELU_PRE) != 0 : (a.flags & RD_RELU_PRE) != 0;
      const bool do_add = F >= 0 ? (F & RD_ADD) != 0 : (a.flags & RD_ADD) != 0;
      const bool relu_post = F >= 0 ? (F & RD_RELU_POST) != 0 : (a.flags & RD_RELU_POST) != 0;
      Slot16 rv[2][NCT][2];
      auto res_load = [&](int i, Slot16 (&dst)[NCT][2]) {
        const int tc = 32 * (i % FC) + em, ow = ct * C3_TW + tc, oh = oh0 + i / FC;
        const bool live = tc < C3_TW && ow < a.W && oh < a.H && !(ow & sh) && !(DBG & 64);
        const bf16_t* rp = rimg0 + (live ? ((size_t)oh * a.Wo + (size_t)(ow >> sh)) * a.r_cs : 0) + 16 * ehi;
#pragma unroll
        for (int j = 0; j < NCT; ++j) {
          if (DBG & 128) { dst[j][0] = Slot16{0, 0, 0, 0}; dst[j][1] = Slot16{0, 0, 0, 0}; continue; }
          dst[j][0] = *(const Slot16*)(rp + j * 32);
          dst[j][1] = *(const Slot16*)(rp + j * 32 + 8);
        }
      };
      if (do_add) res_load(0, rv[0]);
      const bool relu_f32 = relu_pre && do_add;
      const bool relu_i16 = relu_post || (relu_pre && !do_add);
      typedef float f32x2 __attribute__((ext_vector_type(2)));
      typedef short s16x2 __attribute__((ext_vector_type(2)));
      constexpr bool SC_HOIST = NCT == 2;
      f32x4 scq[2][4], shq[2][4];
      auto sc_load = [&](int j, f32x4 (&sc)[4], f32x4 (&sh)[4]) {
#pragma unroll
        for (int g4 = 0; g4 < 4; ++g4) {
          sc[g4] = *(const f32x4*)(Sc + j * 32 + 16 * ehi + 4 * g4);
          sh[g4] = *(const f32x4*)(Sc + COUT + j * 32 + 16 * ehi + 4 * g4);
        }
      };
      if constexpr (!FOLD) {
        sc_load(0, scq[0], shq[0]);
        if constexpr (SC_HOIST) sc_load(1, scq[1], shq[1]);
      }
#pragma unroll
      for (int i = 0; i < FPW; ++i) {
        if (do_add && i + 1 < FPW) res_load(i + 1, rv[(i + 1) & 1]);
        f32x16 h0, h1;
        if constexpr (HEAD) {
#pragma unroll
          for (int r = 0; r < 16; ++r) { h0[r] = 0.f; h1[r] = 0.f; }
        }
#pragma unroll
        for (int jp = 0; jp < NPASS; ++jp) {
        constexpr int KSP = 8 / NPASS;
        s16x8 hwq[HEAD && NPASS == 2 ? 2 : 1][HEAD && NPASS == 2 ? KSP : 1];
        if constexpr (HEAD && NPASS == 2) {
#pragma unroll
          for (int part = 0; part < 2; ++part)
#pragma unroll
            for (int ks = 0; ks < KSP; ++ks)
              hwq[part][ks] = *(const s16x8*)(e_hw + part * 8192 + (jp * KSP + ks) * 1024 + el * 16);
        }
#pragma unroll
        for (int j = jp * JW; j < (jp + 1) * JW; ++j) {
          C3_FENCE();
          const int cur = SC_HOIST ? j : (i * NCT + j) & 1;
          if constexpr (!SC_HOIST && !FOLD) sc_load((j + 1) % NCT, scq[cur ^ 1], shq[cur ^ 1]);
          const int cb = j * 32 + 16 * ehi;
          unsigned pk[8];
#pragma unroll
          for (int g4 = 0; g4 < 4; ++g4) {
#pragma unroll
            for (int h2 = 0; h2 < 2; ++h2) {
              const int r = 4 * g4 + 2 * h2;
              const f32x2 av = {acc[i][j][r], acc[i][j][r + 1]};
              f32x2 v = av;
              if constexpr (!FOLD) {
                const f32x2 s2 = {scq[cur][g4][2 * h2], scq[cur][g4][2 * h2 + 1]};
                const f32x2 t2 = {shq[cur][g4][2 * h2], shq[cur][g4][2 * h2 + 1]};
                v = av * s2 + t2;
              }
              if (relu_f32) v = f32x2{fmaxf(v[0], 0.f), fmaxf(v[1], 0.f)};
              if (do_add) {
                const unsigned w2 = rv[i & 1][j][r >> 3][(r >> 1) & 3];
                v += H16<DT>::unpk(w2);
              }
              unsigned p2 = H16<DT>::pk(v[0], v[1]);
              if (relu_i16) p2 = __builtin_bit_cast(unsigned, __builtin_elementwise_max(__builtin_bit_cast(s16x2, p2), (s16x2){0, 0}));
              pk[2 * g4 + h2] = p2;
            }
          }
#pragma unroll
          for (int u = 0; u < 2; ++u)
            *(Slot16*)(scr + em * ROWB + (((((cb - jp * CW) >> 3) + u) ^ (em & (SPR - 1))) << 4)) =
                Slot16{pk[4 * u], pk[4 * u + 1], pk[4 * u + 2], pk[4 * u + 3]};
        }
        C3_FENCE();
        __builtin_amdgcn_wave_barrier();
        if constexpr (HEAD) {
#pragma unroll
          for (int ks = 0; ks < KSP; ++ks) {
            const s16x8 bq = *(const s16x8*)(scr + em * ROWB + (((2 * ks + ehi) ^ (em & (SPR - 1))) << 4));
            s16x8 wh, wl;
            if constexpr (NPASS == 2) { wh = hwq[0][ks]; wl = hwq[1][ks]; }
            else {
              wh = *(const s16x8*)(smem + HWOFF + ks * 1024 + el * 16);
              wl = *(const s16x8*)(smem + HWOFF + 8192 + ks * 1024 + el * 16);
            }
            h0 = H16<DT>::mfma(wl, bq, h0);
            h1 = H16<DT>::mfma(wh, bq, h1);
          }
          const int tcs = 32 * (i % FC) + em, ows = ct * C3_TW + tcs, ohs = oh0 + i / FC;
          if (jp == NPASS - 1 && tcs < C3_TW && ows < a.W && ohs < a.H) {
            float* o = e_ho + (size_t)b * e_ho_bs + (a.ho_off + (size_t)ohs * a.W + ows) * e_hn + 4 * ehi;
            if (e_hn == 8 && !((size_t)o & 15)) {
              const f32x4 bv = *(const f32x4*)(e_hb + 4 * ehi);
              *(f32x4*)o = f32x4{(h0[0] + h1[0]) + bv[0], (h0[1] + h1[1]) + bv[1], (h0[2] + h1[2]) + bv[2], (h0[3] + h1[3]) + bv[3]};
            } else {
#pragma unroll
              for (int r = 0; r < 4; ++r)
                if (4 * ehi + r < e_hn) o[r] = (h0[r] + h1[r]) + e_hb[4 * ehi + r];
            }
          }
        } else {
#pragma unroll
          for (int it = 0; it < 32 / RPI; ++it) {
            const int pr = it * RPI + el / SPR, sl = el % SPR;
            const Slot16 v = *(const Slot16*)(scr + pr * ROWB + ((sl ^ (pr & (SPR - 1))) << 4));
            const int tcs = 32 * (i % FC) + pr, ows = ct * C3_TW + tcs;
            if (tcs < C3_TW && ows < a.W && oh0 + i / FC < a.H && !(ows & sh) && (!(DBG & 1) || a.B < 0))
              __builtin_nontemporal_store(v, (Slot16*)(yrow0 + (size_t)(i / FC) * a.Wo * a.y_cs + (size_t)(ows >> sh) * a.y_cs + jp * CW + sl * 8));
          }
        }
        __builtin_amdgcn_wave_barrier();
        C3_FENCE();
        }
      }
    };
    auto epilogue16 = [&](auto FL) {
      constexpr int F = decltype(FL)::value;
      const bool relu_pre = F >= 0 ? (F & RD_RELU_PRE) != 0 : (a.flags & RD_RELU_PRE) != 0;
      const bool do_add = F >= 0 ? (F & RD_ADD) != 0 : (a.flags & RD_ADD) != 0;
      const bool relu_post = F >= 0 ? (F & RD_RELU_POST) != 0 : (a.flags & RD_RELU_POST) != 0;
      const bool relu_f32 = relu_pre && do_add;
      const bool relu_i16 = relu_post || (relu_pre && !do_add);
      typedef float f32x2 __attribute__((ext_vector_type(2)));
      typedef short s16x2 __attribute__((ext_vector_type(2)));
      const int en = el & 15, eq = el >> 4;
      Slot16 rv[2][2][JW];
      auto res_load = [&](int t, Slot16 (&dst)[2][JW]) {
        const int i = t / NPASS, jp = t % NPASS;
#pragma unroll
        for (int hf = 0; hf < 2; ++hf) {
          const int ow = ct * C3_TW + 16 * hf + en, oh = oh0 + i;
          const bool live = ow < a.W && oh < a.H;
          const bf16_t* rp = rimg0 + (live ? ((size_t)oh * a.Wo + (size_t)ow) * a.r_cs : 0) + 8 * eq + jp * CW;
#pragma unroll
          for (int pp = 0; pp < JW; ++pp) dst[hf][pp] = *(const Slot16*)(rp + 32 * pp);
        }
      };
      if (do_add) res_load(0, rv[0]);
#pragma unroll
      for (int i = 0; i < FPW; ++i) {
        f32x4 hh[HEAD ? 2 : 1][HEAD ? 2 : 1];
        if constexpr (HEAD) {
#pragma unroll
          for (int hf = 0; hf < 2; ++hf)
#pragma unroll
            for (int part = 0; part < 2; ++part) hh[hf][part] = f32x4{0.f, 0.f, 0.f, 0.f};
        }
#pragma unroll
        for (int jp = 0; jp < NPASS; ++jp) {
          const int t = NPASS * i + jp;
          if (do_add && t + 1 < NPASS * FPW) res_load(t + 1, rv[(t + 1) & 1]);
          s16x8 hwq[HEAD ? 2 : 1][HEAD ? JW : 1];
          if constexpr (HEAD) {
#pragma unroll
            for (int part = 0; part < 2; ++part)
#pragma unroll
              for (int pp = 0; pp < JW; ++pp)
                hwq[part][pp] = *(const s16x8*)(e_hw + part * 4096 + (jp * JW + pp) * 1024 + el * 16);
          }
#pragma unroll
          for (int hf = 0; hf < 2; ++hf)
#pragma unroll
            for (int pp = 0; pp < JW; ++pp) {
              C3_FENCE();
              const int p = jp * JW + pp, h = 2 * i + hf;
              unsigned pk[4];
#pragma unroll
              for (int w2 = 0; w2 < 4; ++w2) {
                const f32x4 av = acc6[h][2 * p + (w2 >> 1)];
                f32x2 v = {av[2 * (w2 & 1)], av[2 * (w2 & 1) + 1]};
                if (relu_f32) v = f32x2{fmaxf(v[0], 0.f), fmaxf(v[1], 0.f)};
                if (do_add) v += H16<DT>::unpk(rv[t & 1][hf][pp][w2]);
                unsigned p2 = H16<DT>::pk(v[0], v[1]);
                if (relu_i16) p2 = __builtin_bit_cast(unsigned, __builtin_elementwise_max(__builtin_bit_cast(s16x2, p2), (s16x2){0, 0}));
                pk[w2] = p2;
              }
              if constexpr (HEAD) {
                s16x8 bq;
                memcpy(&bq, pk, 16);
                hh[hf][0] = H16<DT>::mfma16(hwq[1][pp], bq, hh[hf][0]);
                hh[hf][1] = H16<DT>::mfma16(hwq[0][pp], bq, hh[hf][1]);
              } else {
                const int px = 16 * hf + en;
                *(Slot16*)(scr + px * ROWB + (((4 * pp + eq) ^ (px & (SPR - 1))) << 4)) = Slot16{pk[0], pk[1], pk[2], pk[3]};
              }
            }
          C3_FENCE();
          if constexpr (!HEAD) {
          __builtin_amdgcn_wave_barrier();
#pragma unroll
          for (int it = 0; it < 32 / RPI; ++it) {
            const int pr = it * RPI + el / SPR, sl = el % SPR;
            const Slot16 v = *(const Slot16*)(scr + pr * ROWB + ((sl ^ (pr & (SPR - 1))) << 4));
            const int ows = ct * C3_TW + pr;
            if (ows < a.W && oh0 + i < a.H)
              __builtin_nontemporal_store(v, (Slot16*)(yrow0 + (size_t)i * a.Wo * a.y_cs + (size_t)ows * a.y_cs + jp * CW + sl * 8));
          }
          __builtin_amdgcn_wave_barrier();
          C3_FENCE();
          }
        }
        if constexpr (HEAD) {
#pragma unroll
          for (int hf = 0; hf < 2; ++hf) {
            const int ows = ct * C3_TW + 16 * hf + en, ohs = oh0 + i;
            if (eq < 2 && ows < a.W && ohs < a.H) {
              float* o = e_ho + (size_t)b * e_ho_bs + (a.ho_off + (size_t)ohs * a.W + ows) * e_hn + 4 * eq;
              if (e_hn == 8 && !((size_t)o & 15)) {
                const f32x4 bv = *(const f32x4*)(e_hb + 4 * eq);
                *(f32x4*)o = f32x4{(hh[hf][0][0] + hh[hf][1][0]) + bv[0], (hh[hf][0][1] + hh[hf][1][1]) + bv[1],
                                   (hh[hf][0][2] + hh[hf][1][2]) + bv[2], (hh[hf][0][3] + hh[hf][1][3]) + bv[3]};
              } else {
#pragma unroll
                for (int r = 0; r < 4; ++r)
                  if (4 * eq + r < e_hn) o[r] = (hh[hf][0][r] + hh[hf][1][r]) + e_hb[4 * eq + r];
              }
            }
          }
          C3_FENCE();
        }
      }
    };
    if constexpr (M16) {
      static_assert(!M16 || (NPASS == 2 && JW == 2 && CW == 64), "M16 epilogue: two passes of 64 channels");
      if (a.flags == RD_RELU_POST) epilogue16(std::integral_constant<int, RD_RELU_POST>{});
      else if (a.flags == (RD_ADD | RD_RELU_POST)) epilogue16(std::integral_constant<int, RD_ADD | RD_RELU_POST>{});
      else epilogue16(std::integral_constant<int, -1>{});
    } else {
    if (a.flags == RD_RELU_POST) epilogue(std::integral_constant<int, RD_RELU_POST>{});
    else if (a.flags == (RD_ADD | RD_RELU_POST)) epilogue(std::integral_constant<int, RD_ADD | RD_RELU_POST>{});
    else if (TS != 0 && a.flags == (RD_RELU_PRE | RD_ADD)) epilogue(std::integral_constant<int, RD_RELU_PRE | RD_ADD>{});
    else epilogue(std::integral_constant<int, -1>{});
    }
    if (k == 0) C3_TRACE()
  }
  __builtin_amdgcn_s_waitcnt(RD_VMCNT_IMM(0));
  C3_TRACE()
  if (a.trace && tid == 0) a.trace[(size_t)blockIdx.x * 8 + 7] = __builtin_readcyclecounter() - clk0;
#undef C3_STEP16
#undef C3_MM16
#undef C3_RDP16
#undef C3_RDW16
#undef C3_GBODY_FROM1
#undef C3_RDX
#undef C3_GSTEP
#undef C3_AO
#undef C3_STEP
#undef C3_STEP_
#undef C3_MMZ
#undef C3_SYNC
#undef C3_MM
#undef C3_RD
#undef C3_FENCE
#undef C3_TRACE
}

inline int conv_num_cus() {
#ifdef RD_BUILD_NUM_CUS
  return RD_BUILD_NUM_CUS;
#else
  int dev = 0, v = 0;
  if (hipGetDevice(&dev) != hipSuccess || hipDeviceGetAttribute(&v, hipDeviceAttributeMultiprocessorCount, dev) != hipSuccess || v <= 0) v = 256;
  return v;
#endif
}

template <int NCT, int TS, bool HEAD, bool SC, bool FOLD, C3Tile TILE, int DT, bool GRP = false, int BODY = 0, bool M16 = false>
inline int c3_go(int grid, hipStream_t st, const Conv3Args& a) {
  auto k = conv3x3_stream_kernel<NCT, 0, TS, HEAD, SC, FOLD, TILE, DT, GRP, BODY, M16>;
  static std::atomic<unsigned long long> seen{0};
  once_per_device(seen, [&] { allow_big_lds(k); });
  constexpr size_t lds = C3Cfg<NCT, TILE>::LDS + (HEAD && TILE == C3_8x62 ? 16384 : 0);
  hipLaunchKernelGGL(k, dim3(grid), dim3(256), lds, st, a);
  return check_launch("conv3x3_stream_kernel");
}

#ifdef RD_BUILD_F16_PRODUCTION_FORMS_ONLY
constexpr bool kF16AllForms = false;
#else
constexpr bool kF16AllForms = true;
#endif
inline bool conv3_has_form(int dt, bool fold) { return kF16AllForms || dt == RD_BF16 || fold; }

inline bool conv3_eligible(const TapList& tl, int in_stride, int out_stride, int cout, int dt, int Win, int Wq, int Wout) {
  if (!is_h16(dt) || !conv3_has_form(dt, false) || tl.n != 9 || (in_stride != 1 && in_stride != 2) || out_stride != 1) return false;
  if (Wq != (Win - 1) / in_stride + 1 || Wout != Wq) return false;
  if (cout != 64 && cout != 128) return false;
  for (int t = 0; t < 9; ++t)
    if (tl.dh[t] != t / 3 - 1 || tl.dw[t] != t % 3 - 1) return false;
  return !dev_switches().conv_v1;
}

struct Conv3Second {
  const void* x; int x_co;
  const void* w; const float* shift;
  const void* res; int r_co;
  void* y; int y_co;
  const void* hw; const float* hb; float* ho; long ho_bs; int hn;
};
struct Conv3Phases { int nph, ts_mask, y_pc, r_pc; long w_pb; };
struct Conv3Src2 { const void* x; int cs, co, cin1, cin2; };
inline bool conv3_phases_eligible(int cout, int flags) {
  return (cout == 64 || cout == 128) && (flags & RD_SCALE_FOLDED) && !dev_switches().conv_v1;
}
inline bool conv3_mfma16_ok(int cin, int cout, int stride_w) {
  return cout == 128 && stride_w == 1 && cin >= 32 && cin % 32 == 0 && !dev_switches().conv_v1;
}

template <int DT>
inline int launch_conv3_dt(const void* x, int x_cs, int x_co, const void* w, const float* scale, const float* shift,
                           const void* res, int r_cs, int r_co, void* y, int y_cs, int y_co, int B, int H, int W, int cin,
                           int cout, int flags, int sw, hipStream_t st, int ts, const Conv3Args* head, const Conv3Second* g1,
                           const Conv3Phases* ph, const Conv3Src2* s2, int body);
inline int launch_conv3(const void* x, int x_cs, int x_co, const void* w, const float* scale, const float* shift,
                        const void* res, int r_cs, int r_co, void* y, int y_cs, int y_co, int B, int H, int W, int cin,
                        int cout, int flags, int sw, hipStream_t st, int ts, const Conv3Args* head, int dt,
                        const Conv3Second* g1, const Conv3Phases* ph, const Conv3Src2* s2, int body) {
  RD_REQUIRE(is_h16(dt), RD_EINVAL, "conv3: dtype %d (the persistent 3x3 kernel takes RD_BF16 or RD_F16)", dt);
  if (dt == RD_F16) return launch_conv3_dt<RD_F16>(x, x_cs, x_co, w, scale, shift, res, r_cs, r_co, y, y_cs, y_co, B, H, W, cin, cout, flags, sw, st, ts, head, g1, ph, s2, body);
  return launch_conv3_dt<RD_BF16>(x, x_cs, x_co, w, scale, shift, res, r_cs, r_co, y, y_cs, y_co, B, H, W, cin, cout, flags, sw, st, ts, head, g1, ph, s2, body);
}

template <int DT>
inline int launch_conv3_dt(const void* x, int x_cs, int x_co, const void* w, const float* scale, const float* shift,
                           const void* res, int r_cs, int r_co, void* y, int y_cs, int y_co, int B, int H, int W, int cin,
                           int cout, int flags, int sw, hipStream_t st, int ts, const Conv3Args* head, const Conv3Second* g1,
                           const Conv3Phases* ph, const Conv3Src2* s2, int body) {
  Conv3Args a;
  memset(&a, 0, sizeof(a));
  a.ngrp = g1 ? 2 : 1;
  a.nph = 1;
  if (ph) { a.nph = ph->nph; a.ts_mask = ph->ts_mask; a.y_pc = ph->y_pc; a.r_pc = ph->r_pc; a.w_pb = ph->w_pb; }
  if (head) { a.hw = head->hw; a.hb = head->hb; a.ho = head->ho; a.ho_bs = head->ho_bs; a.ho_off = head->ho_off; a.hn = head->hn; }
  const bool sc = head && head->sx;
  const bool fold = (flags & RD_SCALE_FOLDED) != 0;
  RD_REQUIRE(!fold || !scale, RD_EINVAL, "conv3: RD_SCALE_FOLDED takes no scale array (the packer folded it into the weights)");
  flags &= ~RD_SCALE_FOLDED;
  if (sc) { a.sx = head->sx; a.s_cs = head->s_cs; a.s_co = head->s_co; a.s_bs = head->s_bs; a.scw = head->scw; a.s_nks = head->s_nks; }
  a.sw = sw; a.Wo = (W - 1) / sw + 1;
  a.x = (const bf16_t*)x; a.x_cs = x_cs; a.x_co = x_co; a.x_bs = (long)H * W * x_cs;
  a.w = (const unsigned char*)w; a.scale = scale; a.shift = shift;
  a.res = (const bf16_t*)res; a.r_cs = r_cs; a.r_co = r_co; a.r_bs = (long)H * a.Wo * r_cs;
  a.y = (bf16_t*)y; a.y_cs = y_cs; a.y_co = y_co; a.y_bs = (long)H * a.Wo * y_cs;
  a.zero16 = (const unsigned char*)w + conv_packed_body_bytes(c3_nsteps(ts), cin, cout, RD_BF16);
  a.H = H; a.W = W; a.B = B; a.nslots = cin_slots(cin, RD_BF16); a.nchunk = (cin + 31) / 32; a.flags = flags;
  const bool headfuse = head && !sc;
  RD_REQUIRE(!headfuse || cout == 128, RD_ESHAPE, "conv3 + output conv: cout %d (128)", cout);
  const bool wide = fold && (!headfuse || W <= 1400 || body == C3_BODY_M16 || g1);
  const int tw = wide ? C3Cfg<4, C3_8x32>::TW : C3Cfg<4, C3_8x62>::TW, th = C3Cfg<4>::TH;
  a.ncol = (W + tw - 1) / tw; a.nrow = (H + th - 1) / th; a.ntiles = a.ncol * a.nrow * B * a.ngrp;
  if (g1) {
    RD_REQUIRE(wide && fold && !sc && ts == 0 && cout == 128 && sw == 1, RD_ESHAPE,
               "conv3: two problems per launch need the 8 x 32 tile form (cout 128, folded scales, stride 1, no shortcut)");
    RD_REQUIRE(!headfuse == !g1->hw && !res == !g1->res && !shift == !g1->shift, RD_EINVAL,
               "conv3: the two problems of a launch must have the same structure (output conv / residual / shift)");
    a.g_x = ((const bf16_t*)g1->x + g1->x_co) - ((const bf16_t*)x + x_co);
    a.g_w = (const unsigned char*)g1->w - (const unsigned char*)w;
    a.g_shift = shift ? g1->shift - shift : 0;
    a.g_res = res ? ((const bf16_t*)g1->res + g1->r_co) - ((const bf16_t*)res + r_co) : 0;
    a.g_y = y ? ((bf16_t*)g1->y + g1->y_co) - ((bf16_t*)y + y_co) : 0;
    if (headfuse) {
      a.g_hw = (const unsigned char*)g1->hw - a.hw; a.g_hb = g1->hb - a.hb; a.g_ho = g1->ho - a.ho;
      a.g_ho_bs = g1->ho_bs - a.ho_bs; a.g_hn = g1->hn - a.hn;
    }
  }
  if (s2) {
    RD_REQUIRE(wide && !g1 && sw == 1 && s2->cin1 > 0 && s2->cin1 % 32 == 0 && s2->cin1 + s2->cin2 == cin && s2->cin2 > 0, RD_ESHAPE,
               "conv3: a two-tensor input needs the 8 x 32 tile form and cin1 a multiple of 32 (cin1 %d, cin2 %d, cin %d)", s2->cin1, s2->cin2, cin);
    a.x2 = (const bf16_t*)s2->x; a.x2_cs = s2->cs; a.x2_co = s2->co; a.x2_bs = (long)H * W * s2->cs;
    a.nchunk1 = s2->cin1 / 32; a.nslots2 = cin_slots(s2->cin2, RD_BF16); a.nslots = a.nchunk1 * 4;
  }
  const int grid = std::min(a.ntiles, conv_num_cus() * (wide ? 2 : 1));
  a.xcd = dev_switches().conv_xcd && !g1 && (a.ncol * B) % 8 == 0 && grid % 8 == 0;
  if (conv_trace_buf() && (size_t)grid * 8 <= (1u << 20)) a.trace = conv_trace_buf();
  ProfScope ps(RD_PROF_CONV3, st);
#ifdef RD_CONV3_DEV
  static const int dbg = getenv("RD_CONV3_DBG") ? atoi(getenv("RD_CONV3_DBG")) : 0;
#define C3_DBG_CASE(D) if (cout == 128 && !fold && !head && ts == 0 && DT == RD_BF16 && dbg == D) { auto k = conv3x3_stream_kernel<4, D>; allow_big_lds(k); hipLaunchKernelGGL(k, dim3(grid), dim3(256), C3Cfg<4>::LDS, st, a); return check_launch("conv3x3_stream_kernel<dbg>"); }
  C3_DBG_CASE(2) C3_DBG_CASE(4) C3_DBG_CASE(16) C3_DBG_CASE(32)
#undef C3_DBG_CASE
#define C3_DBG(N, D)                                                                                                    \
  if (cout == 32 * N && wide && !head && !g1 && !ph && !s2 && !body && sw == 1 && ts == 0 && DT == RD_BF16 && dbg == D) { \
    auto k = conv3x3_stream_kernel<N, D, 0, false, false, true, C3_8x32>; allow_big_lds(k);                             \
    hipLaunchKernelGGL(k, dim3(grid), dim3(256), (C3Cfg<N, C3_8x32>::LDS), st, a);                                      \
    return check_launch("conv3x3_stream_kernel<dbg>");                                                                  \
  }
  C3_DBG(2, 4) C3_DBG(2, 8) C3_DBG(2, 16) C3_DBG(2, 64) C3_DBG(2, 128) C3_DBG(2, 256) C3_DBG(2, 257)
  C3_DBG(4, 4) C3_DBG(4, 8) C3_DBG(4, 16) C3_DBG(4, 2) C3_DBG(4, 32) C3_DBG(4, 256) C3_DBG(4, 257)
#undef C3_DBG
#endif
#ifdef RD_CONV3_DEV_M16_ONLY
  RD_REQUIRE(wide && !sc && !g1 && !ph && !s2 && sw == 1 && ts == 0 && cout == 128 && DT == RD_BF16 && (!headfuse || body == C3_BODY_M16), RD_ESHAPE, "conv16_dev: plain bf16 cout-128 form only");
  if (body == C3_BODY_M16 && headfuse) return c3_go<4, 0, true, false, true, C3_8x32, RD_BF16, false, 0, true>(grid, st, a);
  if (body == C3_BODY_M16) return c3_go<4, 0, false, false, true, C3_8x32, RD_BF16, false, 0, true>(grid, st, a);
  return c3_go<4, 0, false, false, true, C3_8x32, RD_BF16>(grid, st, a);
#else
  constexpr bool kAllForms = kF16AllForms || DT == RD_BF16;
  RD_REQUIRE(kAllForms || fold, RD_ESHAPE, "conv3: this fp16 launch form is not instantiated in the emulator build (conv3_has_form)");
  if (sc) {
    RD_REQUIRE(ts == 0 || ts == 1, RD_ESHAPE, "conv3 + shortcut: tap set %d", ts);
    RD_REQUIRE(fold, RD_EINVAL, "conv3 + shortcut: the weights must carry the folded scales (RD_SCALE_FOLDED)");
  }
  if (body == C3_BODY_M16) {
    RD_REQUIRE(wide && !sc && !g1 && !ph && !s2 && sw == 1 && ts == 0 && cout == 128 && cin % 32 == 0, RD_ESHAPE,
               "conv3: the 16 x 16 x 32 form needs the 8 x 32 tile form: cout 128, folded scales, stride 1, cin a multiple of 32 (cin %d)%s", cin,
               headfuse ? " (rd_conv3x3_mfma16_ok)" : "");
    if (headfuse) return c3_go<4, 0, true, false, true, C3_8x32, DT, false, 0, true>(grid, st, a);
    return c3_go<4, 0, false, false, true, C3_8x32, DT, false, 0, true>(grid, st, a);
  }
  if (body) {
    RD_REQUIRE(wide && !headfuse && !g1 && !ph && sw == 1 && a.nchunk % c3_body(body).nu == 0, RD_ESHAPE,
               "conv3: tile body %d needs the 8 x 32 tile form with folded scales (%d chunks)", body, a.nchunk);
    if (body == 1) {
      RD_REQUIRE(ts == 1 && !s2, RD_ESHAPE, "conv3: body 1 is the stride-2 pair view");
      if (sc) { if (cout == 128) return c3_go<4, 1, false, true, true, C3_8x32, DT, false, 1>(grid, st, a); return c3_go<2, 1, false, true, true, C3_8x32, DT, false, 1>(grid, st, a); }
      if (cout == 128) return c3_go<4, 1, false, false, true, C3_8x32, DT, false, 1>(grid, st, a);
      return c3_go<2, 1, false, false, true, C3_8x32, DT, false, 1>(grid, st, a);
    }
    RD_REQUIRE(ts == 0 && !sc, RD_ESHAPE, "conv3: tile body %d takes all nine taps, no shortcut", body);
    if (body == 2) { if (cout == 128) return c3_go<4, 0, false, false, true, C3_8x32, DT, false, 2>(grid, st, a); return c3_go<2, 0, false, false, true, C3_8x32, DT, false, 2>(grid, st, a); }
    if (cout == 128) return c3_go<4, 0, false, false, true, C3_8x32, DT, false, 3>(grid, st, a);
    return c3_go<2, 0, false, false, true, C3_8x32, DT, false, 3>(grid, st, a);
  }
  if (ph) {
    RD_REQUIRE(wide && !sc && !head && !g1 && ts == 3 && sw == 1 && ph->nph >= 1 && ph->nph <= 8, RD_ESHAPE,
               "conv3: all phases per launch need the 8 x 32 tile form (folded scales, no shortcut / output conv)");
    if (cout == 128) return c3_go<4, 3, false, false, true, C3_8x32, DT>(grid, st, a);
    return c3_go<2, 3, false, false, true, C3_8x32, DT>(grid, st, a);
  }
  if (wide && g1) {
    if (headfuse) return c3_go<4, 0, true, false, true, C3_8x32, DT, true>(grid, st, a);
    return c3_go<4, 0, false, false, true, C3_8x32, DT, true>(grid, st, a);
  }
  if (wide) {
    if (headfuse) return c3_go<4, 0, true, false, true, C3_8x32, DT>(grid, st, a);
#define C3_BODY(N)                                                                                        \
  {                                                                                                       \
    if (sc) return ts == 0 ? c3_go<N, 0, false, true, true, C3_8x32, DT>(grid, st, a)                     \
                           : c3_go<N, 1, false, true, true, C3_8x32, DT>(grid, st, a);                    \
    return ts == 0 ? c3_go<N, 0, false, false, true, C3_8x32, DT>(grid, st, a)                            \
         : ts == 1 ? c3_go<N, 1, false, false, true, C3_8x32, DT>(grid, st, a)                            \
                   : c3_go<N, 2, false, false, true, C3_8x32, DT>(grid, st, a);                           \
  }
    if (cout == 128) C3_BODY(4)
    C3_BODY(2)
#undef C3_BODY
  }
  if (headfuse && fold) return c3_go<4, 0, true, false, true, C3_8x62, DT>(grid, st, a);
  if constexpr (kAllForms) {
    if (headfuse) return c3_go<4, 0, true, false, false, C3_8x62, DT>(grid, st, a);
    RD_REQUIRE(!fold, RD_ESHAPE, "conv3: folded scales without an output conv take the 8 x 32 tile");
#define C3_PLAIN(N) return ts == 0 ? c3_go<N, 0, false, false, false, C3_8x62, DT>(grid, st, a) : ts == 1 ? c3_go<N, 1, false, false, false, C3_8x62, DT>(grid, st, a) : c3_go<N, 2, false, false, false, C3_8x62, DT>(grid, st, a);
    if (cout == 128) { C3_PLAIN(4) }
    C3_PLAIN(2)
#undef C3_PLAIN
  }
  return rd::fail(RD_ESHAPE, "conv3: launch form not available");
#endif
}

}
```

rangedet_amd/csrc/rd_api.hip:

```cpp
#include "k_conv1.h"
#include "k_block.h"
#include "k_assign.h"
#include "k_input.h"
#include "k_target.h"
#include "k_nms3d.h"
#include "k_meta.h"
#include "k_misc.h"
#include "k_riou.h"
#include "k_sort.h"
#include "k_wnms.h"

#include <algorithm>
#include <string>
#include <numeric>

using namespace rd;

namespace rd {
inline size_t align256(size_t v) { return (v + 255) & ~(size_t)255; }
inline size_t wnms_ws_bytes(int cap) {
  const size_t nw = (size_t)(cap + 63) / 64;
  return align256((size_t)cap * PREP_F * 4) + 3 * align256((size_t)cap * nw * 8) + 4 * align256((size_t)cap * 4) +
         align256(((size_t)cap + 2) * 8 + 3 * ((size_t)cap / 32 + 2) * 4) + align256(nw * 8) + 256 + align256(sort_ws_bytes(cap)) + 256;
}
inline WnmsWs wnms_ws_carve(void* ws, int cap) {
  WnmsWs w;
  const size_t nw = (size_t)(cap + 63) / 64;
  unsigned char* p = (unsigned char*)(((uintptr_t)ws + 255) & ~(uintptr_t)255);
  w.nwcap = (int)nw;
  w.prep = (float*)p; p += align256((size_t)cap * PREP_F * 4);
  w.thr = (unsigned long long*)p; p += align256((size_t)cap * nw * 8);
  w.vote = (unsigned long long*)p; p += align256((size_t)cap * nw * 8);
  w.snap = (unsigned long long*)p; p += align256((size_t)cap * nw * 8);
  w.keep_q = (int*)p; p += align256((size_t)cap * 4);
  w.order = (int*)p; p += align256((size_t)cap * 4);
  w.alive = (int*)p; p += align256((size_t)cap * 4);
  w.ovf = (int*)p; p += align256((size_t)cap * 4);
  w.scratch = (int*)p; p += align256(((size_t)cap + 2) * 8 + 3 * ((size_t)cap / 32 + 2) * 4);
  w.supp_state = (unsigned long long*)p; p += align256(nw * 8);
  w.nalive = (int*)p; w.novf = (int*)p + 1; p += 256;
  w.sort_ws = p;
  return w;
}
inline void allow_conv_lds() {
  static std::atomic<unsigned long long> seen{0};
  once_per_device(seen, [] {
    allow_big_lds(conv_taps_kernel<RD_BF16, 4, 3>); allow_big_lds(conv_taps_kernel<RD_BF16, 4, 8>);
    allow_big_lds(conv_taps_kernel<RD_F16, 4, 3>); allow_big_lds(conv_taps_kernel<RD_F16, 4, 8>);
    allow_big_lds(conv_taps_kernel<RD_F32, 4, 8>); allow_big_lds(conv_taps_kernel<RD_F32, 4, 3>);
  });
}
}

extern "C" {

int rd_version(void) { return 100; }
const char* rd_last_error_string(void) { return rd::err_buf(); }

int rd_nchw_to_nhwc(const float* src, void* dst, int B, int C, int H, int W, int dst_cstride, int dst_coff,
                    int zero_pad, int dst_dtype, void* stream) {
  RD_REQUIRE(src && dst, RD_EINVAL, "nchw_to_nhwc: null pointer");
  RD_REQUIRE(B > 0 && C > 0 && H > 0 && W > 0 && zero_pad >= 0, RD_ESHAPE, "nchw_to_nhwc: bad shape");
  RD_REQUIRE(dst_coff >= 0 && dst_coff + C + zero_pad <= dst_cstride, RD_ESHAPE, "nchw_to_nhwc: channels exceed stride");
  hipStream_t st = (hipStream_t)stream;
  const long HW = (long)H * W, total = (long)B * (C + zero_pad) * HW;
  const int grid = (int)std::min<long>((total + 255) / 256, 8192);
  ProfScope ps(RD_PROF_LAYOUT, st);
  {
    const int ch = ch_per_slot(dst_dtype), ctot = C + zero_pad;
    if ((is_h16(dst_dtype) || dst_dtype == RD_F32) && ctot % ch == 0 && ctot / ch <= 2 && dst_cstride % ch == 0 && dst_coff % ch == 0) {
      const long npix = (long)B * HW;
      const int g2 = (int)std::min<long>((npix + 255) / 256, 8192);
#define RD_PX(DT, NS) hipLaunchKernelGGL((nchw_to_nhwc_px_kernel<DT, NS>), dim3(g2), dim3(256), 0, st, src, dst, C, HW, dst_cstride, dst_coff, npix)
      if (dst_dtype == RD_BF16) { if (ctot / ch == 1) RD_PX(RD_BF16, 1); else RD_PX(RD_BF16, 2); }
      else if (dst_dtype == RD_F16) { if (ctot / ch == 1) RD_PX(RD_F16, 1); else RD_PX(RD_F16, 2); }
      else { if (ctot / ch == 1) RD_PX(RD_F32, 1); else RD_PX(RD_F32, 2); }
#undef RD_PX
      return check_launch("nchw_to_nhwc");
    }
  }
  if (dst_dtype == RD_BF16)
    hipLaunchKernelGGL(nchw_to_nhwc_kernel<RD_BF16>, dim3(grid), dim3(256), 0, st, src, dst, C, HW, dst_cstride, dst_coff, zero_pad, total);
  else if (dst_dtype == RD_F16)
    hipLaunchKernelGGL(nchw_to_nhwc_kernel<RD_F16>, dim3(grid), dim3(256), 0, st, src, dst, C, HW, dst_cstride, dst_coff, zero_pad, total);
  else if (dst_dtype == RD_F32)
    hipLaunchKernelGGL(nchw_to_nhwc_kernel<RD_F32>, dim3(grid), dim3(256), 0, st, src, dst, C, HW, dst_cstride, dst_coff, zero_pad, total);
  else
    return rd::fail(RD_EINVAL, "nchw_to_nhwc: dtype %d", dst_dtype);
  return check_launch("nchw_to_nhwc");
}
int rd_copy_rows(const void* src, long src_row_bytes, void* dst, long dst_row_bytes, long dst_offset_bytes, long bytes,
                 int rows, void* stream) {
  RD_REQUIRE(src && dst, RD_EINVAL, "copy_rows: null pointer");
  RD_REQUIRE(rows > 0 && bytes > 0 && src_row_bytes >= bytes && dst_row_bytes >= dst_offset_bytes + bytes && dst_offset_bytes >= 0,
             RD_ESHAPE, "copy_rows: bad geometry");
  ProfScope ps(RD_PROF_LAYOUT, (hipStream_t)stream);
  if (hipMemcpy2DAsync((char*)dst + dst_offset_bytes, (size_t)dst_row_bytes, src, (size_t)src_row_bytes, (size_t)bytes,
                       (size_t)rows, hipMemcpyDeviceToDevice, (hipStream_t)stream) != hipSuccess)
    return rd::fail(RD_EHIP, "copy_rows: hipMemcpy2DAsync failed");
  return RD_OK;
}
int rd_nhwc_to_nchw(const void* src, float* dst, int B, int C, int H, int W, int src_cstride, int src_coff,
                    int src_dtype, void* stream) {
  RD_REQUIRE(src && dst, RD_EINVAL, "nhwc_to_nchw: null pointer");
  RD_REQUIRE(B > 0 && C > 0 && H > 0 && W > 0, RD_ESHAPE, "nhwc_to_nchw: bad shape");
  RD_REQUIRE(src_coff >= 0 && src_coff + C <= src_cstride, RD_ESHAPE, "nhwc_to_nchw: channels exceed stride");
  hipStream_t st = (hipStream_t)stream;
  const long HW = (long)H * W, total = (long)B * C * HW;
  const int grid = (int)std::min<long>((total + 255) / 256, 8192);
  ProfScope ps(RD_PROF_LAYOUT, st);
  if (src_dtype == RD_BF16)
    hipLaunchKernelGGL(nhwc_to_nchw_kernel<RD_BF16>, dim3(grid), dim3(256), 0, st, src, dst, C, HW, src_cstride, src_coff, total);
  else if (src_dtype == RD_F16)
    hipLaunchKernelGGL(nhwc_to_nchw_kernel<RD_F16>, dim3(grid), dim3(256), 0, st, src, dst, C, HW, src_cstride, src_coff, total);
  else if (src_dtype == RD_F32)
    hipLaunchKernelGGL(nhwc_to_nchw_kernel<RD_F32>, dim3(grid), dim3(256), 0, st, src, dst, C, HW, src_cstride, src_coff, total);
  else
    return rd::fail(RD_EINVAL, "nhwc_to_nchw: dtype %d", src_dtype);
  return check_launch("nhwc_to_nchw");
}

size_t rd_conv_packed_bytes(int ntaps, int cin, int cout, int dtype) { return conv_packed_bytes(ntaps, cin, cout, dtype); }
int rd_pack_conv_weight_host(const float* w, int cout, int cin, int kh, int kw, int dtype, void* out) {
  RD_REQUIRE(w && out, RD_EINVAL, "pack_conv: null pointer");
  RD_REQUIRE(dtype == RD_F32 || is_h16(dtype), RD_EINVAL, "pack_conv: dtype");
  RD_REQUIRE(kh * kw >= 1 && kh * kw <= 9 && (kh & 1) && (kw & 1), RD_ESHAPE, "pack_conv: kernel (%d,%d)", kh, kw);
  TapList tl = conv_taps(kh, kw);
  auto get = [&](int co, int ci, int t) { return w[(((size_t)co * cin + ci) * kh + tl.kh[t]) * kw + tl.kw[t]]; };
  memset(out, 0, conv_packed_bytes(tl.n, cin, cout, dtype));
  if (is_h16(dtype)) pack_taps_frag(tl.n, cin, cout, out, get, dtype);
  else pack_taps(tl.n, cin, cout, dtype, out, get);
  return RD_OK;
}
static bool deconv_embeds_3x3(const TapList& tl) {
  for (int t = 0; t < tl.n; ++t)
    if (tl.dh[t] < -1 || tl.dh[t] > 1 || tl.dw[t] < -1 || tl.dw[t] > 1) return false;
  return tl.n >= 1 && tl.n <= 9;
}
static int deconv_tap_set(const TapList& tl) {
  if (tl.n != 6 || !deconv_embeds_3x3(tl)) return 0;
  for (int ts = 1; ts <= 2; ++ts) {
    bool seen[6] = {false, false, false, false, false, false};
    bool ok = true;
    for (int t = 0; t < 6 && ok; ++t) {
      const int c = tl.dw[t] - (ts == 1 ? -1 : 0);
      if (c < 0 || c > 1) ok = false;
      else seen[(tl.dh[t] + 1) * 2 + c] = true;
    }
    for (int i = 0; i < 6 && ok; ++i) ok = seen[i];
    if (ok) return ts;
  }
  return 0;
}
static TapList deconv_taps_sorted(int kh, int kw, int s, int pad_w, int phase) {
  TapList tl = deconv_taps(kh, kw, s, pad_w, phase);
  if (tl.n > 9) return tl;
  for (int i = 1; i < tl.n; ++i)
    for (int j = i; j > 0 && (tl.dh[j] < tl.dh[j - 1] || (tl.dh[j] == tl.dh[j - 1] && tl.dw[j] < tl.dw[j - 1])); --j) {
      std::swap(tl.dh[j], tl.dh[j - 1]); std::swap(tl.dw[j], tl.dw[j - 1]);
      std::swap(tl.kh[j], tl.kh[j - 1]); std::swap(tl.kw[j], tl.kw[j - 1]);
    }
  return tl;
}
int rd_deconv_phase_taps(int kh, int kw, int stride_w, int pad_w, int phase) {
  if (stride_w < 1 || phase < 0 || phase >= stride_w) return RD_EINVAL;
  TapList tl = deconv_taps(kh, kw, stride_w, pad_w, phase);
  if (tl.n > 9) return RD_ESHAPE;
  return (deconv_embeds_3x3(tl) && !deconv_tap_set(tl)) ? 9 : tl.n;
}
int rd_pack_deconv_weight_host(const float* w, int cin, int cout, int kh, int kw, int stride_w, int pad_w,
                               int phase, int dtype, void* out) {
  return rd_pack_deconv_weight_folded_host(w, nullptr, cin, cout, kh, kw, stride_w, pad_w, phase, dtype, out);
}
int rd_pack_deconv_weight_folded_host(const float* w, const float* fold_scale, int cin, int cout, int kh, int kw, int stride_w,
                                      int pad_w, int phase, int dtype, void* out) {
  RD_REQUIRE(w && out, RD_EINVAL, "pack_deconv: null pointer");
  RD_REQUIRE(dtype == RD_F32 || is_h16(dtype), RD_EINVAL, "pack_deconv: dtype");
  RD_REQUIRE(stride_w >= 1 && phase >= 0 && phase < stride_w, RD_EINVAL, "pack_deconv: phase");
  TapList tl = deconv_taps_sorted(kh, kw, stride_w, pad_w, phase);
  RD_REQUIRE(tl.n >= 1 && tl.n <= 9, RD_ESHAPE, "pack_deconv: %d taps", tl.n);
  const bool emb = deconv_embeds_3x3(tl) && !deconv_tap_set(tl);
  auto get = [&](int co, int ci, int t) -> float {
    if (emb) {
      int src = -1;
      for (int u = 0; u < tl.n; ++u)
        if (tl.dh[u] == t / 3 - 1 && tl.dw[u] == t % 3 - 1) src = u;
      if (src < 0) return 0.f;
      t = src;
    }
    return (fold_scale ? fold_scale[co] : 1.f) * w[(((size_t)ci * cout + co) * kh + tl.kh[t]) * kw + tl.kw[t]];
  };
  const int nt = emb ? 9 : tl.n;
  memset(out, 0, conv_packed_bytes(nt, cin, cout, dtype));
  if (is_h16(dtype)) pack_taps_frag(nt, cin, cout, out, get, dtype);
  else pack_taps(nt, cin, cout, dtype, out, get);
  return RD_OK;
}

int rd_conv2d_bn_act(const void* x, int x_cstride, int x_coff, const void* w_packed, const float* scale,
                     const float* shift, const void* residual, int r_cstride, int r_coff, void* y, int y_cstride,
                     int y_coff, int B, int H, int Win, int cin, int cout, int kh, int kw, int stride_w, int flags,
                     int dtype, void* stream) {
  RD_REQUIRE(x && w_packed && y, RD_EINVAL, "conv2d: null pointer");
  RD_REQUIRE((kh == 1 && kw == 1) || (kh == 3 && kw == 3), RD_ESHAPE, "conv2d: kernel (%d,%d) not in {1x1,3x3}", kh, kw);
  RD_REQUIRE(stride_w == 1 || stride_w == 2, RD_ESHAPE, "conv2d: stride_w %d", stride_w);
  RD_REQUIRE(y_coff >= 0 && y_coff + cout <= y_cstride, RD_ESHAPE, "conv2d: y channels exceed stride");
  const int pad = (kw - 1) / 2;
  const int Wout = (Win + 2 * pad - kw) / stride_w + 1;
  RD_REQUIRE(!(flags & RD_SCALE_FOLDED), RD_EINVAL, "conv2d: RD_SCALE_FOLDED is taken by rd_conv3x3_bn_act_ex / rd_conv2d_bn_act_head_out / rd_deconv2d_bn_act");
  TapList tl = conv_taps(kh, kw);
  allow_conv_lds();
  return launch_conv(tl, x, x_cstride, x_coff, w_packed, scale, shift, residual, r_cstride, r_coff, y, y_cstride,
                     y_coff, B, H, Win, Wout, Wout, cin, cout, stride_w, 1, 0, flags, dtype, (hipStream_t)stream);
}
static int ex_view_cin(int cin, int x_cstride, int stride_w) { return stride_w == 2 ? x_cstride + cin : cin; }
size_t rd_conv3x3_ex_packed_bytes(int cin, int cout, int stride_w, int x_cstride) {
  return conv_packed_bytes(stride_w == 2 ? 6 : 9, ex_view_cin(cin, x_cstride, stride_w), cout, RD_BF16);
}
int rd_pack_conv3x3_ex_host(const float* w, const float* fold_scale, int cout, int cin, int stride_w, int x_cstride, int dtype,
                            void* out) {
  RD_REQUIRE(w && out, RD_EINVAL, "pack_conv3x3_ex: null pointer");
  RD_REQUIRE(is_h16(dtype), RD_EINVAL, "pack_conv3x3_ex: dtype %d (RD_BF16 or RD_F16)", dtype);
  RD_REQUIRE(stride_w == 1 || stride_w == 2, RD_ESHAPE, "pack_conv3x3_ex: stride_w %d", stride_w);
  RD_REQUIRE(cout == 64 || cout == 128, RD_ESHAPE, "pack_conv3x3_ex: cout %d", cout);
  RD_REQUIRE(stride_w == 1 || (x_cstride >= cin && x_cstride % 8 == 0), RD_ESHAPE, "pack_conv3x3_ex: x_cstride %d for cin %d", x_cstride, cin);
  auto wv = [&](int co, int ci, int dh, int dw) {
    return (fold_scale ? fold_scale[co] : 1.f) * w[(((size_t)co * cin + ci) * 3 + (dh + 1)) * 3 + (dw + 1)];
  };
  memset(out, 0, rd_conv3x3_ex_packed_bytes(cin, cout, stride_w, x_cstride));
  auto wv2 = [&](int co, int c2, int dh, int dw2) -> float {
    if (c2 < cin) return dw2 == 0 ? wv(co, c2, dh, 0) : 0.f;
    if (c2 >= x_cstride && c2 - x_cstride < cin) return wv(co, c2 - x_cstride, dh, dw2 == -1 ? -1 : 1);
    return 0.f;
  };
  if (stride_w == 1) {
    if (conv3_body_small(cin, fold_scale != nullptr))
      pack_body_frag(3, cin, cout, out, [&](int co, int ci, int dh, int dw) { return wv(co, ci, dh - 1, dw - 1); }, dtype);
    else
      pack_taps_frag(9, cin, cout, out, [&](int co, int ci, int t) { return wv(co, ci, t / 3 - 1, t % 3 - 1); }, dtype);
  } else if (conv3_body_s2(cin, x_cstride, fold_scale != nullptr)) {
    pack_body_frag(1, x_cstride + cin, cout, out, [&](int co, int c2, int dh, int dw) { return wv2(co, c2, dh - 1, dw - 1); }, dtype);
  } else {
    pack_taps_frag(6, x_cstride + cin, cout, out, [&](int co, int c2, int s) -> float { return wv2(co, c2, s / 2 - 1, s % 2 - 1); }, dtype);
  }
  return RD_OK;
}
int rd_pack_conv3x3_m16_host(const float* w, const float* fold_scale, int cout, int cin, int dtype, void* out) {
  RD_REQUIRE(w && out, RD_EINVAL, "pack_conv3x3_m16: null pointer");
  RD_REQUIRE(is_h16(dtype), RD_EINVAL, "pack_conv3x3_m16: dtype %d (RD_BF16 or RD_F16)", dtype);
  RD_REQUIRE(cout == 128 && cin >= 32 && cin % 32 == 0, RD_ESHAPE, "pack_conv3x3_m16: cout %d (128), cin %d (a multiple of 32)", cout, cin);
  memset(out, 0, rd_conv3x3_ex_packed_bytes(cin, cout, 1, cin));
  pack_taps_frag16(9, cin, cout, out, [&](int co, int ci, int t) {
    return (fold_scale ? fold_scale[co] : 1.f) * w[(((size_t)co * cin + ci) * 3 + t / 3) * 3 + t % 3];
  }, dtype);
  return RD_OK;
}
int rd_conv3x3_mfma16_ok(int cin, int cout, int stride_w, int W, int fused_output_conv) {
  (void)W; (void)fused_output_conv;
  return conv3_mfma16_ok(cin, cout, stride_w) ? 1 : 0;
}
size_t rd_conv1x1_sc_packed_bytes(int cin, int cout) { return sc_frag_bytes(cin, cout); }
int rd_pack_conv1x1_sc_host(const float* w, const float* fold_scale, int cout, int cin, int dtype, void* out) {
  RD_REQUIRE(w && out, RD_EINVAL, "pack_conv1x1_sc: null pointer");
  RD_REQUIRE(is_h16(dtype), RD_EINVAL, "pack_conv1x1_sc: dtype %d (RD_BF16 or RD_F16)", dtype);
  RD_REQUIRE((cout == 64 || cout == 128) && cin >= 1 && cin <= 128, RD_ESHAPE, "pack_conv1x1_sc: cout %d, cin %d (1..128)", cout, cin);
  pack_sc_frag(w, fold_scale, cin, cout, out, dtype);
  return RD_OK;
}
int rd_conv3x3_bn_act_ex(const void* x, int x_cstride, int x_coff, const void* w_packed, const float* scale, const float* shift,
                         const void* residual, int r_cstride, int r_coff, const void* sc_x, int sc_cstride, int sc_coff,
                         int sc_cin, const void* sc_w_packed, void* y, int y_cstride, int y_coff, int B, int H, int Win, int cin,
                         int cout, int stride_w, int flags, int dtype, void* stream) {
  RD_REQUIRE(x && w_packed && y, RD_EINVAL, "conv3x3_ex: null pointer");
  RD_REQUIRE(is_h16(dtype), RD_EINVAL, "conv3x3_ex: dtype %d (RD_BF16 or RD_F16)", dtype);
  RD_REQUIRE(B > 0 && H > 0 && Win > 0 && cin > 0 && (cout == 64 || cout == 128), RD_ESHAPE, "conv3x3_ex: shape / cout %d", cout);
  RD_REQUIRE(stride_w == 1 || (stride_w == 2 && Win % 2 == 0), RD_ESHAPE, "conv3x3_ex: stride_w %d with Win %d (stride 2 needs an even width)", stride_w, Win);
  RD_REQUIRE(y_coff >= 0 && y_coff + cout <= y_cstride, RD_ESHAPE, "conv3x3_ex: y channels exceed stride");
  RD_REQUIRE(x_cstride % 8 == 0 && x_coff % 8 == 0 && x_coff + cin_slots(cin, RD_BF16) * 8 <= x_cstride, RD_ESHAPE, "conv3x3_ex: x channel stride/offset");
  RD_REQUIRE(!(sc_x && residual) && !(sc_x && !sc_w_packed), RD_EINVAL, "conv3x3_ex: shortcut conv and residual are exclusive");
  RD_REQUIRE(!((flags & RD_ADD) && !residual && !sc_x), RD_EINVAL, "conv3x3_ex: RD_ADD without residual / shortcut");
  RD_REQUIRE(!dev_switches().conv_v1, RD_EINVAL, "conv3x3_ex: needs the persistent 3x3 kernel (RD_CONV_V1 is set)");
  allow_conv_lds();
  const int v = stride_w;
  const int Wv = Win / v;
  Conv3Args e;
  memset(&e, 0, sizeof(e));
  int fl = flags;
  if (sc_x) {
    RD_REQUIRE(sc_cin >= 1 && sc_cin <= 128 && sc_cstride % 8 == 0 && sc_coff % 8 == 0 && sc_coff + ((sc_cin + 15) / 16) * 16 <= sc_cstride,
               RD_ESHAPE, "conv3x3_ex: shortcut input channels %d (stride %d, offset %d)", sc_cin, sc_cstride, sc_coff);
    e.sx = (const bf16_t*)sc_x; e.s_cs = sc_cstride * v; e.s_co = sc_coff; e.s_bs = (long)H * Wv * sc_cstride * v;
    e.scw = (const unsigned char*)sc_w_packed; e.s_nks = (sc_cin + 15) / 16;
    fl &= ~RD_ADD;
    fl |= RD_SCALE_FOLDED;
  }
  RD_REQUIRE(!(fl & RD_SCALE_FOLDED) || !scale, RD_EINVAL, "conv3x3_ex: folded weights take no scale array");
  const bool m16 = (fl & RD_MFMA16) != 0;
  fl &= ~RD_MFMA16;
  const bool folded = (fl & RD_SCALE_FOLDED) != 0;
  RD_REQUIRE(!m16 || (folded && !sc_x && conv3_mfma16_ok(cin, cout, stride_w)), RD_ESHAPE,
             "conv3x3_ex: RD_MFMA16 takes folded weights of rd_pack_conv3x3_m16_host: stride 1, cout 128, cin a multiple of 32, no fused shortcut (rd_conv3x3_mfma16_ok)");
  const int body = m16 ? C3_BODY_M16 : stride_w == 2 ? conv3_body_s2(cin, x_cstride, folded) : (sc_x ? 0 : conv3_body_small(cin, folded));
  RD_REQUIRE(!(stride_w == 1 && sc_x && conv3_body_small(cin, folded)), RD_ESHAPE, "conv3x3_ex: at most 16 input channels together with a fused shortcut is not a launch form");
  return launch_conv3(x, x_cstride * v, x_coff, w_packed, scale, shift, residual, r_cstride, r_coff, y, y_cstride, y_coff, B, H,
                      Wv, ex_view_cin(cin, x_cstride, stride_w), cout, fl, 1, (hipStream_t)stream, stride_w == 2 ? 1 : 0,
                      sc_x ? &e : nullptr, dtype, nullptr, nullptr, nullptr, body);
}

size_t rd_block64_packed_bytes(int cin) { return block64_packed_bytes(cin); }
int rd_pack_block64_host(const float* w1, const float* fold_scale1, const float* w2, const float* fold_scale2, int cin, int dtype, void* out) {
  RD_REQUIRE(w1 && w2 && out, RD_EINVAL, "pack_block64: null pointer");
  RD_REQUIRE(is_h16(dtype), RD_EINVAL, "pack_block64: dtype %d (RD_BF16 or RD_F16)", dtype);
  RD_REQUIRE(cin == 64 || (cin >= 1 && cin <= 16), RD_ESHAPE, "pack_block64: %d input channels (64, or at most 16)", cin);
  pack_block64(w1, fold_scale1, w2, fold_scale2, cin, dtype, out);
  return RD_OK;
}
int rd_block64_bn_act(const void* x, int x_cstride, int x_coff, int cin, const void* w_packed, const float* shift1, const float* shift2,
                      const void* sc_w_packed, void* y, int y_cstride, int y_coff, int B, int H, int W, int dtype, void* stream) {
  RD_REQUIRE(x && w_packed && shift1 && shift2 && y, RD_EINVAL, "block64: null pointer");
  RD_REQUIRE(is_h16(dtype), RD_EINVAL, "block64: dtype %d (RD_BF16 or RD_F16)", dtype);
  RD_REQUIRE(B > 0 && H > 0 && W > 0, RD_ESHAPE, "block64: shape");
  RD_REQUIRE(cin == 64 || (cin >= 1 && cin <= 16), RD_ESHAPE, "block64: %d input channels (64, or at most 16 for the network's first block)", cin);
  RD_REQUIRE(x_cstride % 8 == 0 && x_coff % 8 == 0 && x_coff >= 0 && x_coff + cin_slots(cin, RD_BF16) * 8 <= x_cstride, RD_ESHAPE, "block64: x channel stride / offset");
  RD_REQUIRE(cin > 16 || x_coff + 16 <= x_cstride, RD_ESHAPE, "block64: the first block reads 16 channels per pixel (x_coff %d + 16 > x_cstride %d)", x_coff, x_cstride);
  RD_REQUIRE(y_cstride % 8 == 0 && y_coff % 8 == 0 && y_coff >= 0 && y_coff + 64 <= y_cstride, RD_ESHAPE, "block64: y channel stride / offset");
  RD_REQUIRE(x != y, RD_EINVAL, "block64: in-place (a tile's halo is another tile's output)");
  return launch_block64(x, x_cstride, x_coff, cin, w_packed, shift1, shift2, sc_w_packed, y, y_cstride, y_coff, B, H, W, dtype, (hipStream_t)stream);
}

int rd_pack_block64_m16_host(const float* w1, const float* fold_scale1, const float* w2, const float* fold_scale2, int dtype, void* out) {
  RD_REQUIRE(w1 && w2 && out, RD_EINVAL, "pack_block64_m16: null pointer");
  RD_REQUIRE(is_h16(dtype), RD_EINVAL, "pack_block64_m16: dtype %d (RD_BF16 or RD_F16)", dtype);
  pack_block64_m16(w1, fold_scale1, w2, fold_scale2, dtype, out);
  return RD_OK;
}
int rd_pack_conv1x1_sc_m16_host(const float* w, const float* fold_scale, int dtype, void* out) {
  RD_REQUIRE(w && out, RD_EINVAL, "pack_conv1x1_sc_m16: null pointer");
  RD_REQUIRE(is_h16(dtype), RD_EINVAL, "pack_conv1x1_sc_m16: dtype %d (RD_BF16 or RD_F16)", dtype);
  pack_sc_frag16(w, fold_scale, out, dtype);
  return RD_OK;
}
int rd_block64_m16_bn_act(const void* x, int x_cstride, int x_coff, const void* w_packed, const float* shift1, const float* shift2,
                          const void* sc_w_packed, void* y, int y_cstride, int y_coff, int B, int H, int W, int dtype, void* stream) {
  RD_REQUIRE(x && w_packed && shift1 && shift2 && y, RD_EINVAL, "block64_m16: null pointer");
  RD_REQUIRE(is_h16(dtype), RD_EINVAL, "block64_m16: dtype %d (RD_BF16 or RD_F16)", dtype);
  RD_REQUIRE(B > 0 && H > 0 && W > 0, RD_ESHAPE, "block64_m16: shape");
  RD_REQUIRE(x_cstride % 8 == 0 && x_coff % 8 == 0 && x_coff >= 0 && x_coff + 64 <= x_cstride, RD_ESHAPE, "block64_m16: x channel stride / offset");
  RD_REQUIRE(y_cstride % 8 == 0 && y_coff % 8 == 0 && y_coff >= 0 && y_coff + 64 <= y_cstride, RD_ESHAPE, "block64_m16: y channel stride / offset");
  RD_REQUIRE(x != y, RD_EINVAL, "block64_m16: in-place (a tile's halo is another tile's output)");
  return launch_block64(x, x_cstride, x_coff, 64, w_packed, shift1, shift2, sc_w_packed, y, y_cstride, y_coff, B, H, W, dtype, (hipStream_t)stream, true);
}

size_t rd_conv3x3_cat_packed_bytes(int cin1, int cin2, int cout) { return conv_packed_bytes(9, cin1 + cin2, cout, RD_BF16); }
int rd_pack_conv3x3_cat_host(const float* w, const float* fold_scale, int cout, int cin1, int cin2, int dtype, void* out) {
  RD_REQUIRE(w && out, RD_EINVAL, "pack_conv3x3_cat: null pointer");
  RD_REQUIRE(is_h16(dtype), RD_EINVAL, "pack_conv3x3_cat: dtype %d (RD_BF16 or RD_F16)", dtype);
  RD_REQUIRE((cout == 64 || cout == 128) && cin1 > 0 && cin1 % 32 == 0 && cin2 > 0 && cin2 % 8 == 0, RD_ESHAPE,
             "pack_conv3x3_cat: cout %d, cin1 %d (multiple of 32), cin2 %d (multiple of 8)", cout, cin1, cin2);
  const int cin = cin1 + cin2;
  auto wv = [&](int co, int ci, int dh, int dw) {
    return (fold_scale ? fold_scale[co] : 1.f) * w[(((size_t)co * cin + ci) * 3 + (dh + 1)) * 3 + (dw + 1)];
  };
  memset(out, 0, rd_conv3x3_cat_packed_bytes(cin1, cin2, cout));
  const int body = conv3_body_cat(cin1, cin2, fold_scale != nullptr);
  if (body) pack_body_frag(body, cin, cout, out, [&](int co, int ci, int dh, int dw) { return wv(co, ci, dh - 1, dw - 1); }, dtype);
  else pack_taps_frag(9, cin, cout, out, [&](int co, int ci, int t) { return wv(co, ci, t / 3 - 1, t % 3 - 1); }, dtype);
  return RD_OK;
}
int rd_conv3x3_bn_act_cat(const void* x1, int x1_cstride, int x1_coff, int cin1, const void* x2, int x2_cstride, int x2_coff, int cin2,
                          const void* w_packed, const float* shift, void* y, int y_cstride, int y_coff, int B, int H, int W, int cout,
                          int flags, int dtype, void* stream) {
  RD_REQUIRE(x1 && x2 && w_packed && y && shift, RD_EINVAL, "conv3x3_cat: null pointer");
  RD_REQUIRE(is_h16(dtype), RD_EINVAL, "conv3x3_cat: dtype %d (RD_BF16 or RD_F16)", dtype);
  RD_REQUIRE((flags & RD_SCALE_FOLDED) && !(flags & RD_ADD), RD_EINVAL, "conv3x3_cat: needs RD_SCALE_FOLDED weights, takes no residual");
  RD_REQUIRE(B > 0 && H > 0 && W > 0 && (cout == 64 || cout == 128), RD_ESHAPE, "conv3x3_cat: shape / cout %d", cout);
  RD_REQUIRE(cin1 > 0 && cin1 % 32 == 0 && cin2 > 0 && cin2 % 8 == 0, RD_ESHAPE, "conv3x3_cat: cin1 %d (multiple of 32), cin2 %d (multiple of 8)", cin1, cin2);
  RD_REQUIRE(y_coff >= 0 && y_coff + cout <= y_cstride, RD_ESHAPE, "conv3x3_cat: y channels exceed stride");
  RD_REQUIRE(x1_cstride % 8 == 0 && x1_coff % 8 == 0 && x1_coff + cin1 <= x1_cstride && x2_cstride % 8 == 0 && x2_coff % 8 == 0 &&
             x2_coff + cin2 <= x2_cstride, RD_ESHAPE, "conv3x3_cat: channel stride/offset");
  RD_REQUIRE(!dev_switches().conv_v1, RD_ESHAPE, "conv3x3_cat: needs the persistent 3x3 kernel (RD_CONV_V1 is set)");
  allow_conv_lds();
  Conv3Src2 s2;
  s2.x = x2; s2.cs = x2_cstride; s2.co = x2_coff; s2.cin1 = cin1; s2.cin2 = cin2;
  return launch_conv3(x1, x1_cstride, x1_coff, w_packed, nullptr, shift, nullptr, 0, 0, y, y_cstride, y_coff, B, H, W, cin1 + cin2, cout, flags,
                      1, (hipStream_t)stream, 0, nullptr, dtype, nullptr, nullptr, &s2, conv3_body_cat(cin1, cin2, true));
}

size_t rd_head_packed_bytes(void) { return 16384; }
int rd_pack_head_weight_host(const float* w, int nout, int cin, int dtype, void* out_host) {
  RD_REQUIRE(w && out_host, RD_EINVAL, "pack_head_weight: null pointer");
  RD_REQUIRE(is_h16(dtype), RD_EINVAL, "pack_head_weight: dtype %d (RD_BF16 or RD_F16)", dtype);
  RD_REQUIRE(nout >= 1 && nout <= 8 && cin >= 1 && cin <= 128, RD_ESHAPE, "pack_head_weight: nout %d (1..8), cin %d (1..128)", nout, cin);
  pack_head_frag(w, nout, cin, out_host, dtype);
  return RD_OK;
}
size_t rd_head_m16_packed_bytes(void) { return 8192; }
int rd_pack_head_weight_m16_host(const float* w, int nout, int cin, int dtype, void* out_host) {
  RD_REQUIRE(w && out_host, RD_EINVAL, "pack_head_weight_m16: null pointer");
  RD_REQUIRE(is_h16(dtype), RD_EINVAL, "pack_head_weight_m16: dtype %d (RD_BF16 or RD_F16)", dtype);
  RD_REQUIRE(nout >= 1 && nout <= 8 && cin >= 1 && cin <= 128, RD_ESHAPE, "pack_head_weight_m16: nout %d (1..8), cin %d (1..128)", nout, cin);
  pack_head_frag16(w, nout, cin, out_host, dtype);
  return RD_OK;
}
int rd_conv2d_bn_act_head_out(const void* x, int x_cstride, int x_coff, const void* w_packed, const float* scale,
                              const float* shift, int B, int H, int W, int cin, int flags, const void* head_w_packed,
                              const float* head_bias, float* out, long out_batch_stride, long n_off, int nout, int dtype,
                              void* stream) {
  RD_REQUIRE(x && w_packed && head_w_packed && head_bias && out, RD_EINVAL, "conv2d_head_out: null pointer");
  RD_REQUIRE(is_h16(dtype), RD_EINVAL, "conv2d_head_out: dtype %d (RD_BF16 or RD_F16)", dtype);
  RD_REQUIRE(B > 0 && H > 0 && W > 0 && cin > 0 && nout >= 1 && nout <= 8, RD_ESHAPE, "conv2d_head_out: shape / nout %d (1..8)", nout);
  RD_REQUIRE(!(flags & RD_ADD), RD_EINVAL, "conv2d_head_out: no residual in a head tower");
  RD_REQUIRE(x_cstride % 8 == 0 && x_coff % 8 == 0 && x_coff + cin_slots(cin, RD_BF16) * 8 <= x_cstride, RD_ESHAPE,
             "conv2d_head_out: x channel stride/offset");
  RD_REQUIRE(!dev_switches().conv_v1, RD_EINVAL, "conv2d_head_out: needs the persistent 3x3 kernel (RD_CONV_V1 is set)");
  RD_REQUIRE(!conv3_body_small(cin, (flags & RD_SCALE_FOLDED) != 0), RD_ESHAPE, "conv2d_head_out: cin %d (the packed image of a conv with <= 16 input channels is not this launch form's)", cin);
  const bool m16 = (flags & RD_MFMA16) != 0;
  RD_REQUIRE(!m16 || ((flags & RD_SCALE_FOLDED) && conv3_mfma16_ok(cin, 128, 1)), RD_ESHAPE,
             "conv2d_head_out: RD_MFMA16 (weights of rd_pack_conv3x3_m16_host) is not a launch form for cin %d at width %d (rd_conv3x3_mfma16_ok)", cin, W);
  allow_conv_lds();
  Conv3Args h;
  memset(&h, 0, sizeof(h));
  h.hw = (const unsigned char*)head_w_packed; h.hb = head_bias; h.ho = out; h.ho_bs = out_batch_stride; h.ho_off = n_off; h.hn = nout;
  return launch_conv3(x, x_cstride, x_coff, w_packed, scale, shift, nullptr, 0, 0, nullptr, 128, 0, B, H, W, cin, 128, flags & ~RD_MFMA16, 1,
                      (hipStream_t)stream, 0, &h, dtype, nullptr, nullptr, nullptr, m16 ? C3_BODY_M16 : 0);
}

static int pair_checks(const char* fn, const void* x0, const void* x1, const void* w0, const void* w1, const float* shift0,
                       const float* shift1, int x_cstride, int x0_coff, int x1_coff, int B, int H, int W, int cin, int flags,
                       int dtype) {
  RD_REQUIRE(x0 && x1 && w0 && w1 && shift0 && shift1, RD_EINVAL, "%s: null pointer", fn);
  RD_REQUIRE(is_h16(dtype), RD_EINVAL, "%s: dtype %d (RD_BF16 or RD_F16)", fn, dtype);
  RD_REQUIRE(B > 0 && H > 0 && W > 0 && cin > 0, RD_ESHAPE, "%s: shape", fn);
  RD_REQUIRE((flags & RD_SCALE_FOLDED) && !(flags & RD_ADD), RD_EINVAL, "%s: needs RD_SCALE_FOLDED weights, takes no residual", fn);
  RD_REQUIRE(x_cstride % 8 == 0 && x0_coff % 8 == 0 && x1_coff % 8 == 0 && x0_coff + cin_slots(cin, RD_BF16) * 8 <= x_cstride &&
             x1_coff + cin_slots(cin, RD_BF16) * 8 <= x_cstride, RD_ESHAPE, "%s: x channel stride/offset", fn);
  RD_REQUIRE(!dev_switches().conv_v1, RD_EINVAL, "%s: needs the persistent 3x3 kernel (RD_CONV_V1 is set)", fn);
  RD_REQUIRE(cin > 16, RD_ESHAPE, "%s: cin %d (more than 16 input channels)", fn, cin);
  return RD_OK;
}
int rd_conv3x3_bn_act_pair(const void* x0, int x0_coff, const void* w0_packed, const float* shift0, void* y0, int y0_coff,
                           const void* x1, int x1_coff, const void* w1_packed, const float* shift1, void* y1, int y1_coff,
                           int x_cstride, int y_cstride, int B, int H, int W, int cin, int flags, int dtype, void* stream) {
  if (int rc = pair_checks("conv3x3_pair", x0, x1, w0_packed, w1_packed, shift0, shift1, x_cstride, x0_coff, x1_coff, B, H, W, cin, flags, dtype)) return rc;
  RD_REQUIRE(y0 && y1, RD_EINVAL, "conv3x3_pair: null output");
  RD_REQUIRE(y0_coff >= 0 && y1_coff >= 0 && y0_coff + 128 <= y_cstride && y1_coff + 128 <= y_cstride, RD_ESHAPE, "conv3x3_pair: y channels exceed stride");
  allow_conv_lds();
  Conv3Second g;
  memset(&g, 0, sizeof(g));
  g.x = x1; g.x_co = x1_coff; g.w = w1_packed; g.shift = shift1; g.y = y1; g.y_co = y1_coff;
  return launch_conv3(x0, x_cstride, x0_coff, w0_packed, nullptr, shift0, nullptr, 0, 0, y0, y_cstride, y0_coff, B, H, W, cin, 128, flags, 1,
                      (hipStream_t)stream, 0, nullptr, dtype, &g);
}
int rd_conv2d_bn_act_head_out_pair(const void* x0, int x0_coff, const void* w0_packed, const float* shift0, const void* head_w0_packed,
                                   const float* head_bias0, float* out0, long out0_batch_stride, int nout0,
                                   const void* x1, int x1_coff, const void* w1_packed, const float* shift1, const void* head_w1_packed,
                                   const float* head_bias1, float* out1, long out1_batch_stride, int nout1,
                                   int x_cstride, long n_off, int B, int H, int W, int cin, int flags, int dtype, void* stream) {
  if (int rc = pair_checks("conv2d_head_out_pair", x0, x1, w0_packed, w1_packed, shift0, shift1, x_cstride, x0_coff, x1_coff, B, H, W, cin, flags, dtype)) return rc;
  RD_REQUIRE(head_w0_packed && head_w1_packed && head_bias0 && head_bias1 && out0 && out1, RD_EINVAL, "conv2d_head_out_pair: null pointer");
  RD_REQUIRE(nout0 >= 1 && nout0 <= 8 && nout1 >= 1 && nout1 <= 8, RD_ESHAPE, "conv2d_head_out_pair: nout %d / %d (1..8)", nout0, nout1);
  allow_conv_lds();
  Conv3Args h;
  memset(&h, 0, sizeof(h));
  h.hw = (const unsigned char*)head_w0_packed; h.hb = head_bias0; h.ho = out0; h.ho_bs = out0_batch_stride; h.ho_off = n_off; h.hn = nout0;
  Conv3Second g;
  memset(&g, 0, sizeof(g));
  g.x = x1; g.x_co = x1_coff; g.w = w1_packed; g.shift = shift1;
  g.hw = head_w1_packed; g.hb = head_bias1; g.ho = out1; g.ho_bs = out1_batch_stride; g.hn = nout1;
  return launch_conv3(x0, x_cstride, x0_coff, w0_packed, nullptr, shift0, nullptr, 0, 0, nullptr, 128, 0, B, H, W, cin, 128, flags, 1,
                      (hipStream_t)stream, 0, &h, dtype, &g);
}

int rd_deconv2d_bn_act(const void* x, int x_cstride, int x_coff, const void* w_packed_phase, const float* scale,
                       const float* shift, const void* residual, int r_cstride, int r_coff, void* y, int y_cstride,
                       int y_coff, int B, int H, int Win, int cin, int cout, int kh, int kw, int stride_w, int pad_w,
                       int phase, int flags, int dtype, void* stream) {
  RD_REQUIRE(x && w_packed_phase && y, RD_EINVAL, "deconv2d: null pointer");
  RD_REQUIRE(kh == 3, RD_ESHAPE, "deconv2d: kernel height %d (only 3, pad 1, stride 1)", kh);
  RD_REQUIRE(stride_w >= 1 && phase >= 0 && phase < stride_w, RD_EINVAL, "deconv2d: phase %d of stride %d", phase, stride_w);
  RD_REQUIRE(y_coff >= 0 && y_coff + cout <= y_cstride, RD_ESHAPE, "deconv2d: y channels exceed stride");
  const int Wout = (Win - 1) * stride_w - 2 * pad_w + kw;
  RD_REQUIRE(Wout > phase, RD_ESHAPE, "deconv2d: empty phase");
  const int Wq = (Wout - phase + stride_w - 1) / stride_w;
  TapList tl = deconv_taps_sorted(kh, kw, stride_w, pad_w, phase);
  RD_REQUIRE(tl.n >= 1 && tl.n <= 9, RD_ESHAPE, "deconv2d: %d taps per phase unsupported", tl.n);
  allow_conv_lds();
  if (deconv_embeds_3x3(tl)) {
    const int ts = deconv_tap_set(tl);
    if (!ts) tl = conv_taps(3, 3);
    if (is_h16(dtype) && Wout == stride_w * Win && (cout == 64 || cout == 128) && !dev_switches().conv_v1 &&
        conv3_has_form(dtype, (flags & RD_SCALE_FOLDED) != 0)) {
      const bf16_t* r = (const bf16_t*)residual;
      return launch_conv3(x, x_cstride, x_coff, w_packed_phase, scale, shift, r, r_cstride * stride_w,
                          r_coff + phase * r_cstride, y, y_cstride * stride_w, y_coff + phase * y_cstride, B, H, Win, cin,
                          cout, flags, 1, (hipStream_t)stream, ts, nullptr, dtype);
    }
  }
  RD_REQUIRE(!(flags & RD_SCALE_FOLDED), RD_ESHAPE, "deconv2d: RD_SCALE_FOLDED needs the persistent 3x3 kernel (bf16, cout 64/128, "
             "taps inside the 3x3 window, Wout == stride_w * Win)");
  return launch_conv(tl, x, x_cstride, x_coff, w_packed_phase, scale, shift, residual, r_cstride, r_coff, y,
                     y_cstride, y_coff, B, H, Win, Wq, Wout, cin, cout, 1, stride_w, phase, flags, dtype,
                     (hipStream_t)stream);
}

int rd_deconv2d_all_phases_ok(int kh, int kw, int stride_w, int pad_w, int cout, int dtype) {
  if (!is_h16(dtype) || kh != 3 || stride_w < 2 || stride_w > 8 || !conv3_phases_eligible(cout, RD_SCALE_FOLDED)) return 0;
  if (kw - 2 * pad_w != stride_w) return 0;
  for (int p = 0; p < stride_w; ++p)
    if (!deconv_tap_set(deconv_taps_sorted(kh, kw, stride_w, pad_w, p))) return 0;
  return 1;
}
int rd_deconv2d_bn_act_all(const void* x, int x_cstride, int x_coff, const void* w_packed_all, long w_phase_bytes,
                           const float* shift, const void* residual, int r_cstride, int r_coff, void* y, int y_cstride,
                           int y_coff, int B, int H, int Win, int cin, int cout, int kh, int kw, int stride_w, int pad_w,
                           int flags, int dtype, void* stream) {
  RD_REQUIRE(x && w_packed_all && y, RD_EINVAL, "deconv2d_all: null pointer");
  RD_REQUIRE(is_h16(dtype), RD_EINVAL, "deconv2d_all: dtype %d (RD_BF16 or RD_F16)", dtype);
  RD_REQUIRE(flags & RD_SCALE_FOLDED, RD_EINVAL, "deconv2d_all: needs RD_SCALE_FOLDED weights (rd_pack_deconv_weight_folded_host)");
  RD_REQUIRE(!((flags & RD_ADD) && !residual), RD_EINVAL, "deconv2d_all: RD_ADD without residual");
  RD_REQUIRE(B > 0 && H > 0 && Win > 0 && cin > 0, RD_ESHAPE, "deconv2d_all: shape");
  RD_REQUIRE(y_coff >= 0 && y_coff + cout <= y_cstride, RD_ESHAPE, "deconv2d_all: y channels exceed stride");
  RD_REQUIRE(x_cstride % 8 == 0 && x_coff % 8 == 0 && x_coff + cin_slots(cin, RD_BF16) * 8 <= x_cstride, RD_ESHAPE, "deconv2d_all: x channel stride/offset");
  RD_REQUIRE(rd_deconv2d_all_phases_ok(kh, kw, stride_w, pad_w, cout, dtype), RD_ESHAPE,
             "deconv2d_all: kernel (%d,%d) stride %d pad %d cout %d is not a set of two-column 3x2 phases (use rd_deconv2d_bn_act per phase)",
             kh, kw, stride_w, pad_w, cout);
  RD_REQUIRE(w_phase_bytes >= (long)conv_packed_bytes(6, cin, cout, RD_BF16) && w_phase_bytes % 16 == 0, RD_EINVAL, "deconv2d_all: w_phase_bytes");
  allow_conv_lds();
  Conv3Phases ph;
  ph.nph = stride_w; ph.ts_mask = 0; ph.y_pc = y_cstride; ph.r_pc = r_cstride; ph.w_pb = w_phase_bytes;
  for (int p = 0; p < stride_w; ++p)
    if (deconv_tap_set(deconv_taps_sorted(kh, kw, stride_w, pad_w, p)) == 2) ph.ts_mask |= 1 << p;
  return launch_conv3(x, x_cstride, x_coff, w_packed_all, nullptr, shift, residual, r_cstride * stride_w, r_coff, y, y_cstride * stride_w,
                      y_coff, B, H, Win, cin, cout, flags, 1, (hipStream_t)stream, 3, nullptr, dtype, nullptr, &ph);
}

int rd_deconv2d_phase_pairs_ok(int kh, int kw, int stride_w, int pad_w, int cout, int dtype) {
  if (!rd_deconv2d_all_phases_ok(kh, kw, stride_w, pad_w, cout, dtype) || cout != 64 || stride_w % 2) return 0;
  if (!rd_deconv2d_all_phases_ok(kh, kw, stride_w, pad_w, 128, dtype)) return 0;
  for (int p = 0; p < stride_w; p += 2)
    if (deconv_tap_set(deconv_taps_sorted(kh, kw, stride_w, pad_w, p)) != deconv_tap_set(deconv_taps_sorted(kh, kw, stride_w, pad_w, p + 1))) return 0;
// ... 518 lines not shown
```

rangedet_amd/runtime.py:

```python
import os

import numpy as np

from . import devswitch, lib as rdlib
from .lower import FlatRef, TRef


class TorchAllocator:

    def __init__(self, device="cuda:0", stream=None):
        import torch
        if not torch.cuda.is_available():
            raise RuntimeError("rangedet_amd needs a ROCm GPU (torch.cuda.is_available() is False); there is no CPU fallback")
        self.torch = torch
        self.device = torch.device(device)
        torch.cuda.set_device(self.device)
        self._stream = stream

    @property
    def stream(self):
        st = self._stream or self.torch.cuda.current_stream(self.device)
        return st.cuda_stream

    def alloc(self, nbytes, zero=False):
        f = self.torch.zeros if zero else self.torch.empty
        return f(max(int(nbytes), 16), dtype=self.torch.uint8, device=self.device)

    def upload(self, arr):
        a = np.ascontiguousarray(arr)
        t = self.torch.from_numpy(a.view(np.uint8).reshape(-1)).to(self.device)
        return t

    def ptr(self, buf):
        return buf.data_ptr()

    def view_f32(self, buf, shape):
        n = int(np.prod(shape))
        return buf[: n * 4].view(self.torch.float32).view(*shape)

    def view_i32(self, buf, shape):
        n = int(np.prod(shape))
        return buf[: n * 4].view(self.torch.int32).view(*shape)

    def to_numpy(self, t):
        return t.detach().cpu().numpy()

    def as_device_f32(self, x):
        t = self.torch
        if isinstance(x, np.ndarray):
            return t.from_numpy(np.ascontiguousarray(x, dtype=np.float32)).to(self.device)
        return x.to(device=self.device, dtype=t.float32).contiguous()

    def assign(self, dst_view, src):
        dst_view.copy_(src.reshape(dst_view.shape))

    def new_stream(self, priority=0):
        return self.torch.cuda.Stream(device=self.device, priority=priority)

    def stream_ptr(self, stream):
        return stream.cuda_stream if stream is not None else self.stream

    def record_event(self, stream=None):
        ev = self.torch.cuda.Event()
        ev.record(stream if stream is not None else self.torch.cuda.current_stream(self.device))
        return ev

    def wait_event(self, ev, stream=None):
        (stream if stream is not None else self.torch.cuda.current_stream(self.device)).wait_event(ev)

    def sync(self):
        self.torch.cuda.synchronize(self.device)


def bn_affine(P, name, eps, pad_to=None):
    g, b, m, v = (np.asarray(P[name + s], np.float64) for s in ("_gamma", "_beta", "_moving_mean", "_moving_var"))
    s = g / np.sqrt(v + eps)
    s, t = s.astype(np.float32), (b - m * s).astype(np.float32)
    if pad_to is not None and pad_to > len(s):
        s = np.concatenate([s, np.ones(pad_to - len(s), np.float32)])
        t = np.concatenate([t, np.zeros(pad_to - len(t), np.float32)])
    return s, t


def pad_rows(w, n, axis=0):
    if w.shape[axis] >= n:
        return w
    shp = list(w.shape)
    shp[axis] = n - w.shape[axis]
    return np.concatenate([w, np.zeros(shp, w.dtype)], axis)


class Executor:
    def __init__(self, plan, params, lib=None, alloc=None, reuse_buffers=True, keep_sorted_idx=False):
        self.keep_sorted_idx = keep_sorted_idx
        self.plan = plan
        self.lib = lib or rdlib.get_lib()
        self.alloc = alloc or TorchAllocator()
        self.dtype = plan.dtype
        self.B = plan.batch
        self._phys = {}
        self._assign_buffers(reuse_buffers)
        self._bound = [self._bind(st, params) for st in plan.steps]

    def _assign_buffers(self, reuse):
        plan = self.plan
        last_use, first_def = {}, {}
        for i, st in enumerate(plan.steps):
            for v in st.values():
                if isinstance(v, (TRef, FlatRef)):
                    last_use[v.buf] = i
                    first_def.setdefault(v.buf, i)
        for kind, v in plan.outputs:
            if kind in ("flat", "flat_i32"):
                last_use[v.buf] = len(plan.steps) + 1
        free = {}
        release = {}
        for b, i in last_use.items():
            release.setdefault(i, []).append(b)
        order = sorted(plan.buffers, key=lambda b: first_def.get(b, 0))
        by_def = {}
        for b in order:
            by_def.setdefault(first_def.get(b, 0), []).append(b)
        for i in range(len(plan.steps) + 2):
            for b in by_def.get(i, []):
                info = plan.buffers[b]
                if reuse and not info["persistent"] and free.get(info["nbytes"]):
                    self._phys[b] = free[info["nbytes"]].pop()
                else:
                    self._phys[b] = self.alloc.alloc(info["nbytes"], zero=info["zero"])
            for b in release.get(i, []):
                info = plan.buffers[b]
                if reuse and not info["persistent"] and last_use[b] <= len(plan.steps):
                    free.setdefault(info["nbytes"], []).append(self._phys[b])
        self.device_bytes = sum(int(t.numel()) if hasattr(t, "numel") else len(t) for t in {id(v): v for v in self._phys.values()}.values())

    def p(self, ref):
        return self.alloc.ptr(self._phys[ref.buf])

    def _bind(self, st, P):
        L, A, dt = self.lib, self.alloc, self.dtype
        k = st["kind"]
        b = dict(st)
        if k == "conv_pair":
            b["a"], b["b"] = self._bind(st["a"], P), self._bind(st["b"], P)
            return b
        if k == "block":
            ca, cb = st["a"], st["b"]
            w1, w2 = (np.asarray(P[c["name"] + "_weight"], np.float32) for c in (ca, cb))
            if ca.get("cmap"):
                wp = np.zeros((w1.shape[0], len(ca["cmap"])) + w1.shape[2:], np.float32)
                for pc, lc in enumerate(ca["cmap"]):
                    if lc >= 0:
                        wp[:, pc] = w1[:, lc]
                w1 = wp
            (s1, t1), (s2, t2) = bn_affine(P, ca["bn"], ca["eps"]), bn_affine(P, cb["bn"], cb["eps"])
            m16 = bool(st.get("m16")) and w1.shape[1] == 64
            b["m16"] = m16
            b["w"] = A.upload(L.pack_block64(w1, s1, w2, s2, dtype=dt, m16=m16))
            b["shift1"] = A.upload(t1)
            b["sc_w"] = None
            if cb.get("sc"):
                sc = cb["sc"]
                wsc = np.asarray(P[sc["name"] + "_weight"], np.float32).reshape(64, -1)
                if sc.get("cmap"):
                    wq = np.zeros((64, len(sc["cmap"])), np.float32)
                    for pc, lc in enumerate(sc["cmap"]):
                        if lc >= 0:
                            wq[:, pc] = wsc[:, lc]
                    wsc = wq
                ss, ts = bn_affine(P, sc["bn"], sc["eps"])
                b["sc_w"] = A.upload(L.pack_conv1x1_sc_m16(wsc, ss, dtype=dt) if m16 else L.pack_conv1x1_sc(wsc, fold_scale=ss, dtype=dt))
                t2 = (t2.astype(np.float64) + ts).astype(np.float32)
            b["shift2"] = A.upload(t2)
            b["cin"] = w1.shape[1]
            return b
        if k == "conv":
            w = pad_rows(np.asarray(P[st["name"] + "_weight"], np.float32), st["cout"])
            if st.get("cmap"):
                wp = np.zeros((w.shape[0], len(st["cmap"])) + w.shape[2:], np.float32)
                for pc, lc in enumerate(st["cmap"]):
                    if lc >= 0:
                        wp[:, pc] = w[:, lc]
                w = wp
            s, t = bn_affine(P, st["bn"], st["eps"], pad_to=st["cout"])
            if st.get("sc"):
                sc = st["sc"]
                wsc = np.asarray(P[sc["name"] + "_weight"], np.float32)
                wsc = pad_rows(wsc.reshape(wsc.shape[0], -1), st["cout"])
                if sc.get("cmap"):
                    wq = np.zeros((w.shape[0], len(sc["cmap"])), np.float32)
                    for pc, lc in enumerate(sc["cmap"]):
                        if lc >= 0:
                            wq[:, pc] = wsc[:, lc]
                    wsc = wq
                ss, ts = bn_affine(P, sc["bn"], sc["eps"], pad_to=st["cout"])
                b["w"] = A.upload(L.pack_conv3x3_ex(w, st["stride_w"], st["x"].cs, fold_scale=s, dtype=dt))
                b["sc_w"] = A.upload(L.pack_conv1x1_sc(wsc, fold_scale=ss, dtype=dt))
                b["scale"], b["shift"] = None, A.upload((t.astype(np.float64) + ts).astype(np.float32))
            elif st.get("x2") is not None:
                b["w"] = A.upload(L.pack_conv3x3_cat(w, st["x"].C, st["x2"].cs, fold_scale=s, dtype=dt))
                b["scale"], b["shift"] = None, A.upload(t)
                b["flags"] = st["flags"] | rdlib.RD_SCALE_FOLDED
            elif st.get("ex") and st.get("fold") and st.get("m16") and \
                    L.raw("rd_conv3x3_mfma16_ok")(w.shape[1], st["cout"], 1, st["x"].W, 1 if st.get("head") else 0) == 1:
                b["w"] = A.upload(L.pack_conv3x3_m16(w, s, dtype=dt))
                b["scale"], b["shift"] = None, A.upload(t)
                b["flags"] = st["flags"] | rdlib.RD_SCALE_FOLDED | rdlib.RD_MFMA16
            elif st.get("ex") and st.get("fold"):
                b["w"] = A.upload(L.pack_conv3x3_ex(w, st["stride_w"], st["x"].cs, fold_scale=s, dtype=dt))
                b["scale"], b["shift"] = None, A.upload(t)
                b["flags"] = st["flags"] | rdlib.RD_SCALE_FOLDED
            elif st.get("ex"):
                b["w"] = A.upload(L.pack_conv3x3_ex(w, st["stride_w"], st["x"].cs, dtype=dt))
                b["scale"], b["shift"] = A.upload(s), A.upload(t)
            else:
                b["w"] = A.upload(L.pack_conv_weight(w, dt))
                b["scale"], b["shift"] = A.upload(s), A.upload(t)
        elif k == "deconv":
            w = pad_rows(np.asarray(P[st["name"] + "_weight"], np.float32), st["cout"], axis=1)
            s, t = bn_affine(P, st["bn"], st["eps"], pad_to=st["cout"])
            fs = s if st.get("fold") else None
            imgs = [L.pack_deconv_weight(w, st["stride_w"], st["pad_w"], ph, dt, fold_scale=fs) for ph in range(st["stride_w"])]
            b["all_phases"] = bool(st.get("one_launch")) and len({len(i) for i in imgs}) == 1 and \
                L.raw("rd_deconv2d_all_phases_ok")(st["k"][0], st["k"][1], st["stride_w"], st["pad_w"], st["cout"], dt) == 1
            if st.get("one_launch") and not b["all_phases"] and not L.raw("rd_deconv2d_all_phases_ok")(st["k"][0], st["k"][1], st["stride_w"], st["pad_w"], st["cout"], dt):
                b["one_launch"] = False
            if b["all_phases"]:
                b["w_all"], b["w_pb"] = A.upload(np.concatenate(imgs)), len(imgs[0])
            r_, o_ = st["res"], st["out"]
            b["pairs"] = b["all_phases"] and not devswitch.get("RD_DECONV_NO_PAIRS") and o_.cs == st["cout"] and o_.co == 0 and \
                (r_ is None or (r_.cs == st["cout"] and r_.co == 0)) and \
                L.raw("rd_deconv2d_phase_pairs_ok")(st["k"][0], st["k"][1], st["stride_w"], st["pad_w"], st["cout"], dt) == 1
            if b["pairs"]:
                pimgs = [L.pack_deconv_phase_pair(imgs[p], imgs[p + 1], st["cin"], dt) for p in range(0, st["stride_w"], 2)]
                b["w_pairs"], b["w_pairb"], b["shift2"] = A.upload(np.concatenate(pimgs)), len(pimgs[0]), A.upload(np.concatenate([t, t]))
            b["w"] = [A.upload(i) for i in imgs]
            b["scale"], b["shift"] = (None if st.get("fold") else A.upload(s)), A.upload(t)
            if st.get("fold"):
                b["flags"] = st["flags"] | rdlib.RD_SCALE_FOLDED
        elif k == "meta":
            s1, t1 = bn_affine(P, st["bn1"], st["eps1"])
            s2, t2 = bn_affine(P, st["bn2"], st["eps2"])
            pk = L.pack_meta(P[st["mlp0"] + "_weight"].reshape(32, 3), P[st["mlp0"] + "_bias"],
                             P[st["mlp1"] + "_weight"].reshape(64, 32), P[st["mlp1"] + "_bias"], s1, t1,
                             P[st["agg"] + "_weight"].reshape(64, 576), s2, t2, dt)
            b["packed"] = A.upload(pk)
        if k == "conv" and st.get("head"):
            h = st["head"]
            r0, r1 = h["rows"]
            hw = np.asarray(P[h["name"] + "_weight"], np.float32).reshape(-1, st["cout"])[r0:r1]
            b["head_w"] = A.upload(L.pack_head_weight(hw, dtype=dt, m16=bool(b.get("flags", 0) & rdlib.RD_MFMA16)))
            b["head_bias"] = A.upload(np.asarray(P[h["name"] + "_bias"], np.float32)[r0:r1])
        elif k == "head_out":
            r0, r1 = st["rows"]
            w = np.asarray(P[st["name"] + "_weight"], np.float32).reshape(-1, st["x"].C)[r0:r1]
            b["w"] = A.upload(w)
            b["bias"] = A.upload(np.asarray(P[st["name"] + "_bias"], np.float32)[r0:r1])
        elif k == "nms3d":
            nb = L.raw("rd_nms3d_workspace_bytes")(st["N"], self.B)
            b["ws"] = A.alloc(nb)
            b["ws_bytes"] = nb
        elif k == "sorted_fg":
            nb = L.raw("rd_sorted_foreground_workspace_bytes")(st["N"], st["k"]) * self.B
            b["ws"] = A.alloc(nb)
            b["ws_bytes"] = nb
            b["idx"] = A.alloc(self.B * st["k"] * 4) if self.keep_sorted_idx else None
        return b

    def forward(self, inputs, only=None, dev=None):
        L, A, dt, B = self.lib, self.alloc, self.dtype, self.B
        st_ = A.stream
        dev = {} if dev is None else dev

        def din(name):
            if name not in dev:
                dev[name] = A.as_device_f32(inputs[name])
            return dev[name]

        steps = self._bound if only is None else [self._bound[only]]
        for b in steps:
            k = b["kind"]
            if k == "nchw_in":
                o = b["out"]
                src = din(b["name"])
                assert tuple(src.shape) == (B, o.C, o.H, o.W), (b["name"], tuple(src.shape), (B, o.C, o.H, o.W))
                L.call("rd_nchw_to_nhwc", A.ptr(src), self.p(o), B, o.C, o.H, o.W, o.cs, o.co, b["zero_pad"], dt, st_)
            elif k == "block":
                x, o = b["x"], b["out"]
                if b.get("m16"):
                    L.call("rd_block64_m16_bn_act", self.p(x), x.cs, x.co, A.ptr(b["w"]), A.ptr(b["shift1"]), A.ptr(b["shift2"]),
                           A.ptr(b["sc_w"]) if b["sc_w"] is not None else None, self.p(o), o.cs, o.co, B, x.H, x.W, dt, st_)
                else:
                    L.call("rd_block64_bn_act", self.p(x), x.cs, x.co, b["cin"], A.ptr(b["w"]), A.ptr(b["shift1"]), A.ptr(b["shift2"]),
                           A.ptr(b["sc_w"]) if b["sc_w"] is not None else None, self.p(o), o.cs, o.co, B, x.H, x.W, dt, st_)
            elif k == "conv_pair":
                p, q = b["a"], b["b"]
                x0, x1 = p["x"], q["x"]
                cin = len(p["cmap"]) if p.get("cmap") else p["cin"]
                if p.get("head"):
                    h0, h1 = p["head"], q["head"]
                    L.call("rd_conv2d_bn_act_head_out_pair",
                           self.p(x0), x0.co, A.ptr(p["w"]), A.ptr(p["shift"]), A.ptr(p["head_w"]), A.ptr(p["head_bias"]),
                           self.p(h0["out"]), h0["N"] * h0["nout"], h0["nout"],
                           self.p(x1), x1.co, A.ptr(q["w"]), A.ptr(q["shift"]), A.ptr(q["head_w"]), A.ptr(q["head_bias"]),
                           self.p(h1["out"]), h1["N"] * h1["nout"], h1["nout"],
                           x0.cs, h0["n_off"], B, x0.H, x0.W, cin, p["flags"], dt, st_)
                else:
                    o0, o1 = p["out"], q["out"]
                    L.call("rd_conv3x3_bn_act_pair", self.p(x0), x0.co, A.ptr(p["w"]), A.ptr(p["shift"]), self.p(o0), o0.co,
                           self.p(x1), x1.co, A.ptr(q["w"]), A.ptr(q["shift"]), self.p(o1), o1.co, x0.cs, o0.cs, B, x0.H, x0.W, cin,
                           p["flags"], dt, st_)
            elif k == "conv" and b.get("head"):
                x, h = b["x"], b["head"]
                L.call("rd_conv2d_bn_act_head_out", self.p(x), x.cs, x.co, A.ptr(b["w"]),
                       A.ptr(b["scale"]) if b["scale"] is not None else None, A.ptr(b["shift"]), B,
                       x.H, x.W, b["cin"], b["flags"], A.ptr(b["head_w"]), A.ptr(b["head_bias"]), self.p(h["out"]),
                       h["N"] * h["nout"], h["n_off"], h["nout"], dt, st_)
            elif k == "conv" and b.get("x2") is not None:
                x, x2, o = b["x"], b["x2"], b["out"]
                L.call("rd_conv3x3_bn_act_cat", self.p(x), x.cs, x.co, x.C, self.p(x2), x2.cs, x2.co, x2.cs, A.ptr(b["w"]), A.ptr(b["shift"]),
                       self.p(o), o.cs, o.co, B, x.H, x.W, b["cout"], b["flags"], dt, st_)
            elif k == "conv" and b.get("ex"):
                x, o, r, sx = b["x"], b["out"], b["res"], b.get("sc_x")
                cin = len(b["cmap"]) if b.get("cmap") else b["cin"]
                L.call("rd_conv3x3_bn_act_ex", self.p(x), x.cs, x.co, A.ptr(b["w"]), A.ptr(b["scale"]) if b["scale"] is not None else None,
                       A.ptr(b["shift"]), self.p(r) if r else None, r.cs if r else 0, r.co if r else 0,
                       self.p(sx) if sx else None, sx.cs if sx else 0, sx.co if sx else 0,
                       (len(b["sc"]["cmap"]) if b["sc"].get("cmap") else b["sc"]["cin"]) if sx else 0,
                       A.ptr(b["sc_w"]) if sx else None, self.p(o), o.cs, o.co, B, x.H, x.W, cin, b["cout"], b["stride_w"],
                       b["flags"], dt, st_)
            elif k == "conv":
                x, o, r = b["x"], b["out"], b["res"]
                L.call("rd_conv2d_bn_act", self.p(x), x.cs, x.co, A.ptr(b["w"]), A.ptr(b["scale"]), A.ptr(b["shift"]),
                       self.p(r) if r else None, r.cs if r else 0, r.co if r else 0, self.p(o), o.cs, o.co, B, x.H, x.W,
                       b["cin"], b["cout"], b["k"][0], b["k"][1], b["stride_w"], b["flags"], dt, st_)
            elif k == "deconv":
                x, o, r = b["x"], b["out"], b["res"]
                if b.get("pairs"):
                    L.call("rd_deconv2d_bn_act_pairs", self.p(x), x.cs, x.co, A.ptr(b["w_pairs"]), b["w_pairb"], A.ptr(b["shift2"]), self.p(r), r.cs,
                           r.co, self.p(o), o.cs, o.co, B, x.H, x.W, b["cin"], b["cout"], b["k"][0], b["k"][1], b["stride_w"], b["pad_w"],
                           b["flags"], dt, st_)
                    continue
                if b.get("all_phases"):
                    L.call("rd_deconv2d_bn_act_all", self.p(x), x.cs, x.co, A.ptr(b["w_all"]), b["w_pb"], A.ptr(b["shift"]), self.p(r), r.cs,
                           r.co, self.p(o), o.cs, o.co, B, x.H, x.W, b["cin"], b["cout"], b["k"][0], b["k"][1], b["stride_w"], b["pad_w"],
                           b["flags"], dt, st_)
                    continue
                for ph in range(b["stride_w"]):
                    L.call("rd_deconv2d_bn_act", self.p(x), x.cs, x.co, A.ptr(b["w"][ph]),
                           A.ptr(b["scale"]) if b["scale"] is not None else None, A.ptr(b["shift"]), self.p(r), r.cs, r.co, self.p(o), o.cs, o.co, B, x.H, x.W, b["cin"],
                           b["cout"], b["k"][0], b["k"][1], b["stride_w"], b["pad_w"], ph, b["flags"], dt, st_)
            elif k == "meta":
                x, o = b["x"], b["out"]
                c = din(b["coord"])
                assert tuple(c.shape) == (B, 3, x.H, x.W)
                L.call("rd_meta_kernel_fwd", self.p(x), x.cs, x.co, A.ptr(c), A.ptr(b["packed"]), self.p(o), o.cs, o.co,
                       B, x.H, x.W, dt, st_)
            elif k == "head_out":
                x, o = b["x"], b["out"]
                L.call("rd_head_out", self.p(x), x.cs, x.co, A.ptr(b["w"]), A.ptr(b["bias"]), self.p(o),
                       b["N"] * b["nout"], b["n_off"], B, x.H, x.W, x.C, b["nout"], dt, st_)
            elif k == "concat_in":
                o = b["out"]
                row = b["N"] * b["last"] * 4
                off = 0
                for name, n in b["names"]:
                    src = din(name)
                    assert tuple(src.shape)[:2] == (B, n), (name, tuple(src.shape))
                    L.call("rd_copy_rows", A.ptr(src), n * b["last"] * 4, self.p(o), row, off * b["last"] * 4,
                           n * b["last"] * 4, B, st_)
                    off += n
            elif k == "sorted_fg":
                L.call("rd_sorted_foreground", self.p(b["score"]), self.p(b["delta"]), self.p(b["pc"]), self.p(b["mask"]),
                       B, b["N"], b["k"], b["D"], b["apply_sigmoid"], self.p(b["out_score"]), self.p(b["out_delta"]),
                       self.p(b["out_pc"]), A.ptr(b["idx"]) if b["idx"] is not None else None, A.ptr(b["ws"]), b["ws_bytes"], st_)
            elif k == "decode":
                L.call("rd_decode3d_bbox", self.p(b["delta"]), self.p(b["pc"]), self.p(b["out"]), B, b["k"],
                       b["box_type"], b["is_bin"], st_)
            elif k == "batch_riou":
                g = din(b["gt"])
                three_d = b.get("iou_type", "bev") == "3d"
                assert tuple(g.shape) == (B, b["n_gt"], 7 if three_d else 8), (b["gt"], tuple(g.shape))
                L.call("rd_batch_rotated_iou_3d" if three_d else "rd_batch_rotated_iou", self.p(b["boxes"]), 10, A.ptr(g), self.p(b["out"]),
                       None, B, b["N"], b["n_gt"], st_)
            elif k == "nms3d":
                L.call("rd_nms3d", self.p(b["boxes"]), B, b["N"], b["thr"], b["max_keep"], b["normal_iou"], self.p(b["keep"]),
                       self.p(b["out"]), A.ptr(b["ws"]), b["ws_bytes"], st_)
            else:
                raise RuntimeError("unknown plan step %r" % k)
        if only is not None:
            return None
        outs = []
        for kind, v in self.plan.outputs:
            if kind == "flat":
                outs.append(A.view_f32(self._phys[v.buf], (B,) + tuple(v.shape)))
            elif kind == "flat_i32":
                outs.append(A.view_i32(self._phys[v.buf], (B,) + tuple(v.shape)))
            elif kind == "input":
                outs.append(inputs.get(v))
            else:
                outs.append(np.zeros(v, np.float32))
        return outs

    def read_flat(self, ref):
        self.alloc.sync()
        return np.array(self.alloc.to_numpy(self.alloc.view_f32(self._phys[ref.buf], (self.B,) + tuple(ref.shape))))

    def sorted_idx(self, which=0):
        b = [x for x in self._bound if x["kind"] == "sorted_fg"][which]
        self.alloc.sync()
        return np.array(self.alloc.to_numpy(self.alloc.view_i32(b["idx"], (self.B, b["k"]))))

    def debug_tensor(self, ref):
        A, L = self.alloc, self.lib
        out = A.alloc(self.B * ref.C * ref.H * ref.W * 4)
        L.call("rd_nhwc_to_nchw", self.p(ref), A.ptr(out), self.B, ref.C, ref.H, ref.W, ref.cs, ref.co, self.dtype, A.stream)
        A.sync()
        return A.to_numpy(A.view_f32(out, (self.B, ref.C, ref.H, ref.W)))
```

Before: 995.7.

## Pack two 3x3 taps per MFMA k-step for inputs of at most 8 channels

Adds a paired-tap unit kind (P3) for 3x3 convolutions whose input has at most 8 channels. Each k-step's 16-wide reduction slot then carries two taps, one per lane half, so the nine taps take three k-steps instead of five. This applies to the first residual block, the small-input conv bodies and the concat conv's narrow second input. The aim is fewer zero-padded MFMA steps and LDS reads on the network's 8-channel input layers. In exchange it adds a new template instantiation, per-lane address selection and new packing layouts, and it relies on the concat input being trimmed to a multiple of 8 channels.

```diff
diff --git a/rangedet_amd/csrc/k_block.h b/rangedet_amd/csrc/k_block.h
--- a/rangedet_amd/csrc/k_block.h
+++ b/rangedet_amd/csrc/k_block.h
@@ -22,14 +22,14 @@
 constexpr int BK_SLAB = 4096;
 constexpr size_t BK_LDS = 2 * BK_BUF + BK_R * BK_SLAB;
 
-constexpr int bk_nsteps(bool first) { return first ? 23 : 36; }
-constexpr int bk_unit(bool first, int g) { return first ? (g < 5 ? 0 : g < 14 ? 2 : 3) : g / 9; }
-constexpr int bk_ord(bool first, int g) { return first ? (g < 5 ? g : (g - 5) % 9) : g % 9; }
-constexpr bool bk_fetches(bool first, int g) { return bk_unit(first, g) == 3 || (!first && bk_unit(first, g) == 0); }
+constexpr int bk_nsteps(int first) { return first ? first + 18 : 36; }
+constexpr int bk_unit(int first, int g) { return first ? (g < first ? 0 : g < first + 9 ? 2 : 3) : g / 9; }
+constexpr int bk_ord(int first, int g) { return first ? (g < first ? g : (g - first) % 9) : g % 9; }
+constexpr bool bk_fetches(int first, int g) { return bk_unit(first, g) == 3 || (!first && bk_unit(first, g) == 0); }
 constexpr int bk_pieces_u(int s) { return s <= 1 ? 2 : s <= 4 ? 1 : 0; }
 constexpr int bk_first_u(int s) { int n = 0; for (int t = 0; t < s; ++t) n += bk_pieces_u(t); return n; }
-constexpr int bk_pieces(bool first, int g) { return bk_fetches(first, g) ? bk_pieces_u(bk_ord(first, g)) : 0; }
-constexpr int bk_younger(bool first, int g) {
+constexpr int bk_pieces(int first, int g) { return bk_fetches(first, g) ? bk_pieces_u(bk_ord(first, g)) : 0; }
+constexpr int bk_younger(int first, int g) {
   const int G = bk_nsteps(first);
   int n = BK_R - 3;
   for (int d = 1; d <= BK_R - 2; ++d) n += bk_pieces(first, ((g - d) % G + G) % G);
@@ -37,10 +37,11 @@
   return (bk_fetches(first, g) && bk_ord(first, g) == 7 && n > cap) ? cap : n;
 }
 
-template <int DT, bool SC, bool FIRST = false, bool M16 = false>
+template <int DT, bool SC, int FIRST = 0, bool M16 = false>
 __global__ __launch_bounds__(256, 2) void block64_stream_kernel(BlockArgs a) {
   static_assert(!FIRST || SC, "the first block changes the channel count: projection shortcut");
-  static_assert(!(FIRST && M16), "the first block (five two-tap steps on one 16-channel slot) stays in the 32 x 32 x 16 form");
+  static_assert(FIRST == 0 || FIRST == 3 || FIRST == 5, "the first block's conv1 unit has five steps (9..16 channels) or three (<= 8)");
+  static_assert(!(FIRST && M16), "the first block (one short unit on one 16-channel slot) stays in the 32 x 32 x 16 form");
   HIP_DYNAMIC_SHARED(unsigned char, smem);
   constexpr int R = BK_R, SLAB = BK_SLAB, RING = 2 * BK_BUF, NCT = 2;
   constexpr int ROWB2 = BK_TP * 64;
@@ -171,6 +172,13 @@
       a2[d] = c * 64 + (((q16 ^ (c >> 2)) & 3) << 4) + wave * 2 * ROWB2;
     }
   }
+  int a1q[6];
+#pragma unroll
+  for (int q = 0; q < 6; ++q) {
+    const int ta = 2 * q > 8 ? 8 : 2 * q, tb = 2 * q + 1 > 8 ? 8 : 2 * q + 1;
+    a1q[q] = hi ? a1[tb / 3][tb % 3] ^ 16 : a1[ta / 3][ta % 3];
+  }
+  const int a1f = FIRST == 3 ? a1q[0] : a1[0][0];
   const int boff = RING + lane * 16;
 
   f32x16 acc[M16 ? 1 : 3][M16 ? 1 : NCT];
@@ -237,10 +245,11 @@
 #define BK_P1(S_)                                                                                                  \
   BK_STEP(3, 2048, (S_), 0, ((S_) == 4 ? 0 : 3), 2048, a1[((2 * (S_) + 1) % 9) / 3][(2 * (S_) + 1) % 3],           \
           a1[((2 * (S_) + 2) % 9) / 3][(2 * (S_) + 2) % 3])
+#define BK_P3(S_) BK_STEP(3, 2048, (S_), 0, ((S_) == 2 ? 0 : 3), 2048, a1q[2 * (S_) + 1], a1q[(2 * (S_) + 2) % 6])
 #define BK_C2(C_, S_)                                                                                              \
-  BK_STEP(2, ROWB2, (FIRST ? 5 : 18) + 9 * (C_) + (S_), 0, (((C_) == 1 && (S_) == 8) ? 3 : 2), (((C_) == 1 && (S_) == 8) ? 2048 : ROWB2), \
+  BK_STEP(2, ROWB2, (FIRST ? FIRST : 18) + 9 * (C_) + (S_), 0, (((C_) == 1 && (S_) == 8) ? 3 : 2), (((C_) == 1 && (S_) == 8) ? 2048 : ROWB2), \
           (a2[(S_) % 3] + ((S_) / 3) * ROWB2 + (C_) * BK_BUF) ^ 32,                                                \
-          ((S_) == 8 ? ((C_) == 1 ? a1[0][0] : a2[0] + BK_BUF) : a2[((S_) + 1) % 3] + ((((S_) + 1) % 9) / 3) * ROWB2 + (C_) * BK_BUF))
+          ((S_) == 8 ? ((C_) == 1 ? a1f : a2[0] + BK_BUF) : a2[((S_) + 1) % 3] + ((((S_) + 1) % 9) / 3) * ROWB2 + (C_) * BK_BUF))
 
 #define BK_RDW16(BUF, C, BADDR) { fb[BUF][C] = *(const s16x8*)(smem + (BADDR) + (C) * 1024); BK_FENCE(); }
 #define BK_RDP16(HX, AADDR, FS) { fa16[HX] = *(const s16x8*)(smem + (AADDR) + ((HX) >> 1) * (FS) + ((HX) & 1) * 1024); BK_FENCE(); }
@@ -305,7 +314,7 @@
     for (int kk = 0; kk < 6; ++kk) BK_RDP16(kk, a1[0][0], 2048)
   } else {
 #pragma unroll
-  for (int kk = 0; kk < 3 + NCT; ++kk) BK_RD(3, 2048, 0, kk, a1[0][0], boff + rslot * SLAB, 0)
+  for (int kk = 0; kk < 3 + NCT; ++kk) BK_RD(3, 2048, 0, kk, a1f, boff + rslot * SLAB, 0)
   }
 
   for (int k = 0; k < ntl; ++k) {
@@ -464,7 +473,9 @@
       acc[n / NCT][n % NCT] = H16<DT>::mfma(bz, ones, f32x16{});
     }
     BK_FENCE();
-    if constexpr (FIRST) {
+    if constexpr (FIRST == 3) {
+      BK_P3(0) BK_P3(1) BK_P3(2)
+    } else if constexpr (FIRST == 5) {
       BK_P1(0) BK_P1(1) BK_P1(2) BK_P1(3) BK_P1(4)
     } else {
       BK_C1(0, 0) BK_C1(0, 1) BK_C1(0, 2) BK_C1(0, 3) BK_C1(0, 4) BK_C1(0, 5) BK_C1(0, 6) BK_C1(0, 7) BK_C1(0, 8)
@@ -602,6 +613,7 @@
 #undef BK_RDW16
 #undef BK_C2
 #undef BK_P1
+#undef BK_P3
 #undef BK_C1
 #undef BK_STEP
 #undef BK_SYNC
@@ -610,7 +622,7 @@
 #undef BK_FENCE
 }
 
-inline bool block64_first(int cin) { return cin <= 16; }
+inline int block64_first(int cin) { return cin <= 8 ? 3 : cin <= 16 ? 5 : 0; }
 inline size_t block64_body_bytes(int cin) { return (size_t)bk_nsteps(block64_first(cin)) * BK_SLAB; }
 inline size_t block64_packed_bytes(int cin) { return block64_body_bytes(cin) + RD_CONV_TAIL; }
 inline void pack_block64_m16(const float* w1, const float* s1, const float* w2, const float* s2, int dt, void* out) {
@@ -633,7 +645,7 @@
 inline void pack_block64(const float* w1, const float* s1, const float* w2, const float* s2, int cin, int dt, void* out) {
   memset(out, 0, block64_packed_bytes(cin));
   if (block64_first(cin))
-    pack_body_frag(3, cin, 64, out, [&](int co, int ci, int dh, int dw) { return (s1 ? s1[co] : 1.f) * w1[(((size_t)co * cin + ci) * 3 + dh) * 3 + dw]; }, dt);
+    pack_body_frag(block64_first(cin) == 3 ? 5 : 3, cin, 64, out, [&](int co, int ci, int dh, int dw) { return (s1 ? s1[co] : 1.f) * w1[(((size_t)co * cin + ci) * 3 + dh) * 3 + dw]; }, dt);
   else
     pack_taps_frag(9, 64, 64, out, [&](int co, int ci, int t) { return (s1 ? s1[co] : 1.f) * w1[((size_t)co * 64 + ci) * 9 + t]; }, dt);
   pack_taps_frag(9, 64, 64, (unsigned char*)out + block64_body_bytes(cin) - 18 * BK_SLAB,
@@ -643,7 +655,7 @@
 inline int launch_block64(const void* x, int x_cs, int x_co, int cin, const void* w, const float* shift1, const float* shift2, const void* sc_w,
                           void* y, int y_cs, int y_co, int B, int H, int W, int dt, hipStream_t st, bool m16 = false) {
   RD_REQUIRE(is_h16(dt), RD_EINVAL, "block64: dtype %d (RD_BF16 or RD_F16)", dt);
-  const bool first = block64_first(cin);
+  const int first = block64_first(cin);
   RD_REQUIRE(!m16 || !first, RD_ESHAPE, "block64: the 16 x 16 x 32 form takes 64 input channels");
   RD_REQUIRE(cin == 64 || (first && cin >= 1), RD_ESHAPE, "block64: %d input channels (64, or at most 16 for the network's first block)", cin);
   RD_REQUIRE(!first || sc_w, RD_EINVAL, "block64: a block that changes the channel count needs its projection shortcut");
@@ -654,7 +666,7 @@
   a.y = (bf16_t*)y; a.y_cs = y_cs; a.y_co = y_co; a.y_bs = (long)H * W * y_cs;
   a.zero16 = (const unsigned char*)w + block64_body_bytes(cin);
   a.H = H; a.W = W; a.B = B;
-  a.nslots1 = std::min(2, (x_cs - x_co) / 8);
+  a.nslots1 = first == 3 ? 1 : std::min(2, (x_cs - x_co) / 8);
   a.ncol = (W + 31) / 32; a.nrow = (H + 7) / 8; a.ntiles = a.ncol * a.nrow * B;
   const int grid = std::min(a.ntiles, conv_num_cus() * 2);
   a.xcd = dev_switches().conv_xcd && (a.ncol * B) % 8 == 0 && grid % 8 == 0;
@@ -663,15 +675,17 @@
   once_per_device(seen, [] {
     allow_big_lds(block64_stream_kernel<RD_F16, false>); allow_big_lds(block64_stream_kernel<RD_BF16, false>);
     allow_big_lds(block64_stream_kernel<RD_F16, true>); allow_big_lds(block64_stream_kernel<RD_BF16, true>);
-    allow_big_lds(block64_stream_kernel<RD_F16, true, true>); allow_big_lds(block64_stream_kernel<RD_BF16, true, true>);
-    allow_big_lds(block64_stream_kernel<RD_F16, false, false, true>); allow_big_lds(block64_stream_kernel<RD_BF16, false, false, true>);
-    allow_big_lds(block64_stream_kernel<RD_F16, true, false, true>); allow_big_lds(block64_stream_kernel<RD_BF16, true, false, true>);
+    allow_big_lds(block64_stream_kernel<RD_F16, true, 5>); allow_big_lds(block64_stream_kernel<RD_BF16, true, 5>);
+    allow_big_lds(block64_stream_kernel<RD_F16, true, 3>); allow_big_lds(block64_stream_kernel<RD_BF16, true, 3>);
+    allow_big_lds(block64_stream_kernel<RD_F16, false, 0, true>); allow_big_lds(block64_stream_kernel<RD_BF16, false, 0, true>);
+    allow_big_lds(block64_stream_kernel<RD_F16, true, 0, true>); allow_big_lds(block64_stream_kernel<RD_BF16, true, 0, true>);
   });
 #define BK_GO(DT_)                                                                                                         \
   {                                                                                                                        \
-    if (m16 && sc_w) hipLaunchKernelGGL((block64_stream_kernel<DT_, true, false, true>), dim3(grid), dim3(256), BK_LDS, st, a);  \
-    else if (m16) hipLaunchKernelGGL((block64_stream_kernel<DT_, false, false, true>), dim3(grid), dim3(256), BK_LDS, st, a);    \
-    else if (first) hipLaunchKernelGGL((block64_stream_kernel<DT_, true, true>), dim3(grid), dim3(256), BK_LDS, st, a);    \
+    if (m16 && sc_w) hipLaunchKernelGGL((block64_stream_kernel<DT_, true, 0, true>), dim3(grid), dim3(256), BK_LDS, st, a);  \
+    else if (m16) hipLaunchKernelGGL((block64_stream_kernel<DT_, false, 0, true>), dim3(grid), dim3(256), BK_LDS, st, a);    \
+    else if (first == 3) hipLaunchKernelGGL((block64_stream_kernel<DT_, true, 3>), dim3(grid), dim3(256), BK_LDS, st, a);  \
+    else if (first) hipLaunchKernelGGL((block64_stream_kernel<DT_, true, 5>), dim3(grid), dim3(256), BK_LDS, st, a);       \
     else if (sc_w) hipLaunchKernelGGL((block64_stream_kernel<DT_, true>), dim3(grid), dim3(256), BK_LDS, st, a);           \
     else hipLaunchKernelGGL((block64_stream_kernel<DT_, false>), dim3(grid), dim3(256), BK_LDS, st, a);                    \
   }
diff --git a/rangedet_amd/csrc/k_conv3.h b/rangedet_amd/csrc/k_conv3.h
--- a/rangedet_amd/csrc/k_conv3.h
+++ b/rangedet_amd/csrc/k_conv3.h
@@ -141,17 +141,23 @@
   return n;
 }
 constexpr int C3_BODY_M16 = 16;
-enum { UK_T9 = 0, UK_T6A = 1, UK_T6B = 2, UK_T6R = 3, UK_T3 = 4, UK_P5 = 5 };
-constexpr int uk_nsteps(int k) { return k == UK_T9 ? 9 : k == UK_T3 ? 3 : k == UK_P5 ? 5 : 6; }
-struct C3KStep { int dh, dw, slot; };
+enum { UK_T9 = 0, UK_T6A = 1, UK_T6B = 2, UK_T6R = 3, UK_T3 = 4, UK_P5 = 5, UK_P3 = 6 };
+constexpr int uk_nsteps(int k) { return k == UK_T9 ? 9 : k == UK_T3 || k == UK_P3 ? 3 : k == UK_P5 ? 5 : 6; }
+struct C3KStep { int dh, dw, slot, dh1, dw1; bool pair; };
+constexpr int uk_p3_tap(int s, int ks, int half) { return 4 * s + 2 * ks + half; }
 constexpr C3KStep uk_kstep(int k, int s, int ks) {
-  if (k == UK_P5) { const int t = 2 * s + ks > 8 ? 8 : 2 * s + ks; return C3KStep{t / 3, t % 3, 0}; }
+  if (k == UK_P5) { const int t = 2 * s + ks > 8 ? 8 : 2 * s + ks; return C3KStep{t / 3, t % 3, 0, t / 3, t % 3, false}; }
+  if (k == UK_P3) {
+    const int ta = uk_p3_tap(s, ks, 0) > 8 ? 8 : uk_p3_tap(s, ks, 0), tb = uk_p3_tap(s, ks, 1) > 8 ? 8 : uk_p3_tap(s, ks, 1);
+    return C3KStep{ta / 3, ta % 3, 0, tb / 3, tb % 3, true};
+  }
   const int T = k == UK_T9 ? s : k == UK_T3 ? 3 * s + 1 : 3 * (s / 2) + (s % 2) + (k == UK_T6B ? 1 : 0);
-  return C3KStep{T / 3, T % 3, ks};
+  return C3KStep{T / 3, T % 3, ks, T / 3, T % 3, false};
 }
 struct C3Body { int nu; int kind[4]; };
 constexpr C3Body c3_body(int BODY) {
-  return BODY == 1 ? C3Body{4, {UK_T6A, UK_T3, UK_T3, UK_T6A}} : BODY == 2 ? C3Body{3, {UK_T9, UK_T9, UK_P5, 0}} : C3Body{1, {UK_P5, 0, 0, 0}};
+  return BODY == 1 ? C3Body{4, {UK_T6A, UK_T3, UK_T3, UK_T6A}} : BODY == 2 ? C3Body{3, {UK_T9, UK_T9, UK_P5, 0}} :
+         BODY == 4 ? C3Body{3, {UK_T9, UK_T9, UK_P3, 0}} : BODY == 5 ? C3Body{1, {UK_P3, 0, 0, 0}} : C3Body{1, {UK_P5, 0, 0, 0}};
 }
 constexpr int c3b_steps(int BODY) { int n = 0; for (int u = 0; u < c3_body(BODY).nu; ++u) n += uk_nsteps(c3_body(BODY).kind[u]); return n; }
 constexpr int c3b_unit(int BODY, int g) { int u = 0; while (g >= uk_nsteps(c3_body(BODY).kind[u])) { g -= uk_nsteps(c3_body(BODY).kind[u]); ++u; } return u; }
@@ -190,6 +196,11 @@
           for (int lane = 0; lane < 64; ++lane) {
             const int co = cb * 32 + conv_row_perm(lane & 31);
             for (int j = 0; j < 8; ++j) {
+              if (kind == UK_P3) {
+                const int t = uk_p3_tap(s, ks, lane >> 5), ci = chunk * 32 + j;
+                *o++ = h16_from_f32(dt, (ci < cin && t <= 8) ? get(co, ci, t / 3, t % 3) : 0.f);
+                continue;
+              }
               const int ci = chunk * 32 + k.slot * 16 + (lane >> 5) * 8 + j;
               *o++ = h16_from_f32(dt, (ci < cin && !zero_tap) ? get(co, ci, k.dh, k.dw) : 0.f);
             }
@@ -199,8 +210,8 @@
 }
 inline bool conv3_bodies_on() { return dev_switches().conv_body && !dev_switches().conv_v1; }
 inline int conv3_body_s2(int cin, int x_cstride, bool folded) { return folded && conv3_bodies_on() && x_cstride % 64 == 0 && cin == x_cstride ? 1 : 0; }
-inline int conv3_body_small(int cin, bool folded) { return folded && conv3_bodies_on() && cin <= 16 ? 3 : 0; }
-inline int conv3_body_cat(int cin1, int cin2, bool folded) { return folded && conv3_bodies_on() && cin1 == 64 && cin2 <= 16 ? 2 : 0; }
+inline int conv3_body_small(int cin, bool folded) { return folded && conv3_bodies_on() && cin <= 16 ? (cin <= 8 ? 5 : 3) : 0; }
+inline int conv3_body_cat(int cin1, int cin2, bool folded) { return folded && conv3_bodies_on() && cin1 == 64 && cin2 <= 16 ? (cin2 <= 8 ? 4 : 2) : 0; }
 #define C3_WAIT_IMM(vm, lgkm) (((vm) & 15) | (((vm) >> 4) << 14) | (7 << 4) | ((lgkm) << 8))
 
 template <int NCT, int DBG = 0, int TS = 0, bool HEAD = false, bool SC = false, bool FOLD = false, C3Tile TILE = C3_8x62,
@@ -415,6 +426,12 @@
       aoff[d] = c16 * 64 + ((((lane >> 4) ^ (c16 >> 2)) & 3) << 4) + wave * RW * C3_ROWB;
     }
   }
+  int aoffp[3];
+#pragma unroll
+  for (int d = 0; d < 3; ++d) aoffp[d] = aoff[d] ^ (hi << 4);
+#define C3_KADDR(K, BUF_)                                                                                                          \
+  ((K).pair ? (hi ? aoffp[(K).dw1] + (K).dh1 * C3_ROWB : aoffp[(K).dw] + (K).dh * C3_ROWB) + (BUF_)                                \
+            : ((aoff[(K).dw] + (BUF_) + (K).dh * C3_ROWB) ^ ((K).slot << 5)))
   const int boff = RING + lane * 16;
   auto side2 = [&](int ph) { return (a.ts_mask >> ph) & 1; };
   int pcol[2] = {aoff[0], aoff[1]}, pq0 = aoff[0];
@@ -483,7 +500,7 @@
   }
   C3_SYNC(0, 0)
   C3_TRACE()
-  constexpr C3KStep K00 = BODY ? uk_kstep(c3_body(BODY ? BODY : 3).kind[0], 0, 0) : C3KStep{c3_tap(TS, 0) / 3, c3_tap(TS, 0) % 3, 0};
+  constexpr C3KStep K00 = BODY ? uk_kstep(c3_body(BODY ? BODY : 3).kind[0], 0, 0) : C3KStep{c3_tap(TS, 0) / 3, c3_tap(TS, 0) % 3, 0, 0, 0, false};
   constexpr int K00DW = K00.dw, K00DH = K00.dh;
   int rslot = 0;
   int abuf = 0;
@@ -495,7 +512,7 @@
   } else {
 #pragma unroll
   for (int k = 0; k < NR; ++k)
-    C3_RD(0, k, C3_AO(K00DW) + abuf + K00DH * C3_ROWB, boff + rslot * SLAB, 0)
+    C3_RD(0, k, (K00.pair ? C3_KADDR(K00, abuf) : C3_AO(K00DW) + abuf + K00DH * C3_ROWB), boff + rslot * SLAB, 0)
   }
 
 #define C3_STEP(S) C3_STEP_(S, C3_MM)
@@ -579,10 +596,10 @@
     constexpr C3KStep k1_ = uk_kstep(K_, S_, 1), kn_ = uk_kstep(KN_, c3b_ord(BODY, GN_), 0);                         \
     constexpr bool lastS_ = S_ == NSU_ - 1;                                                                          \
     constexpr int NH_ = c3b_pieces(BODY, (G_)), NP_ = IPW + NH_, HF_ = c3b_first(BODY, (G_)), YG_ = c3b_younger(BODY, R, IPW, (G_)); \
-    const int acur_ = (aoff[k1_.dw] + abuf + k1_.dh * C3_ROWB) ^ (k1_.slot << 5);                                    \
+    const int acur_ = C3_KADDR(k1_, abuf);                                                                           \
     const int bcur_ = boff + rslot * SLAB;                                                                           \
     const int rnext_ = rslot + 1 == R ? 0 : rslot + 1;                                                               \
-    const int anext_ = (aoff[kn_.dw] + (lastS_ ? hflip(abuf) : abuf) + kn_.dh * C3_ROWB) ^ (kn_.slot << 5);          \
+    const int anext_ = C3_KADDR(kn_, (lastS_ ? hflip(abuf) : abuf));                                                 \
     const int bnext_ = boff + rnext_ * SLAB;                                                                         \
     const int hbuf_ = hflip(abuf);                                                                                   \
     C3_FENCE();                                                                                                      \
@@ -1012,6 +1029,7 @@
 #undef C3_RDP16
 #undef C3_RDW16
 #undef C3_GBODY_FROM1
+#undef C3_KADDR
 #undef C3_RDX
 #undef C3_GSTEP
 #undef C3_AO
@@ -1139,7 +1157,9 @@
                "conv3: a two-tensor input needs the 8 x 32 tile form and cin1 a multiple of 32 (cin1 %d, cin2 %d, cin %d)", s2->cin1, s2->cin2, cin);
     a.x2 = (const bf16_t*)s2->x; a.x2_cs = s2->cs; a.x2_co = s2->co; a.x2_bs = (long)H * W * s2->cs;
     a.nchunk1 = s2->cin1 / 32; a.nslots2 = cin_slots(s2->cin2, RD_BF16); a.nslots = a.nchunk1 * 4;
-  }
+    if (body == 4) a.nslots2 = 1;
+  }
+  if (body == 5) a.nslots = 1;
   const int grid = std::min(a.ntiles, conv_num_cus() * (wide ? 2 : 1));
   a.xcd = dev_switches().conv_xcd && !g1 && (a.ncol * B) % 8 == 0 && grid % 8 == 0;
   if (conv_trace_buf() && (size_t)grid * 8 <= (1u << 20)) a.trace = conv_trace_buf();
@@ -1188,9 +1208,14 @@
       return c3_go<2, 1, false, false, true, C3_8x32, DT, false, 1>(grid, st, a);
     }
     RD_REQUIRE(ts == 0 && !sc, RD_ESHAPE, "conv3: tile body %d takes all nine taps, no shortcut", body);
-    if (body == 2) { if (cout == 128) return c3_go<4, 0, false, false, true, C3_8x32, DT, false, 2>(grid, st, a); return c3_go<2, 0, false, false, true, C3_8x32, DT, false, 2>(grid, st, a); }
-    if (cout == 128) return c3_go<4, 0, false, false, true, C3_8x32, DT, false, 3>(grid, st, a);
-    return c3_go<2, 0, false, false, true, C3_8x32, DT, false, 3>(grid, st, a);
+    RD_REQUIRE(body >= 2 && body <= 5 && ((body == 2 || body == 4) == (s2 != nullptr)), RD_ESHAPE, "conv3: tile body %d", body);
+    RD_REQUIRE((body != 4 || s2->cin2 <= 8) && (body != 5 || cin <= 8), RD_ESHAPE, "conv3: tile body %d packs two taps of at most 8 channels per k-step", body);
+#define C3_HET(B_) { if (cout == 128) return c3_go<4, 0, false, false, true, C3_8x32, DT, false, B_>(grid, st, a); return c3_go<2, 0, false, false, true, C3_8x32, DT, false, B_>(grid, st, a); }
+    if (body == 2) C3_HET(2)
+    if (body == 3) C3_HET(3)
+    if (body == 4) C3_HET(4)
+    C3_HET(5)
+#undef C3_HET
   }
   if (ph) {
     RD_REQUIRE(wide && !sc && !head && !g1 && ts == 3 && sw == 1 && ph->nph >= 1 && ph->nph <= 8, RD_ESHAPE,
diff --git a/rangedet_amd/csrc/rd_api.hip b/rangedet_amd/csrc/rd_api.hip
--- a/rangedet_amd/csrc/rd_api.hip
+++ b/rangedet_amd/csrc/rd_api.hip
@@ -234,8 +234,8 @@
     return 0.f;
   };
   if (stride_w == 1) {
-    if (conv3_body_small(cin, fold_scale != nullptr))
-      pack_body_frag(3, cin, cout, out, [&](int co, int ci, int dh, int dw) { return wv(co, ci, dh - 1, dw - 1); }, dtype);
+    if (const int body = conv3_body_small(cin, fold_scale != nullptr))
+      pack_body_frag(body, cin, cout, out, [&](int co, int ci, int dh, int dw) { return wv(co, ci, dh - 1, dw - 1); }, dtype);
     else
       pack_taps_frag(9, cin, cout, out, [&](int co, int ci, int t) { return wv(co, ci, t / 3 - 1, t % 3 - 1); }, dtype);
   } else if (conv3_body_s2(cin, x_cstride, fold_scale != nullptr)) {
diff --git a/rangedet_amd/runtime.py b/rangedet_amd/runtime.py
--- a/rangedet_amd/runtime.py
+++ b/rangedet_amd/runtime.py
@@ -198,7 +198,8 @@
                 b["sc_w"] = A.upload(L.pack_conv1x1_sc(wsc, fold_scale=ss, dtype=dt))
                 b["scale"], b["shift"] = None, A.upload((t.astype(np.float64) + ts).astype(np.float32))
             elif st.get("x2") is not None:
-                b["w"] = A.upload(L.pack_conv3x3_cat(w, st["x"].C, st["x2"].cs, fold_scale=s, dtype=dt))
+                b["cin2"] = min(st["x2"].cs, -(-st["x2"].C // 8) * 8)
+                b["w"] = A.upload(L.pack_conv3x3_cat(w[:, :st["x"].C + b["cin2"]], st["x"].C, b["cin2"], fold_scale=s, dtype=dt))
                 b["scale"], b["shift"] = None, A.upload(t)
                 b["flags"] = st["flags"] | rdlib.RD_SCALE_FOLDED
             elif st.get("ex") and st.get("fold") and st.get("m16") and \
@@ -318,7 +319,7 @@
                        h["N"] * h["nout"], h["n_off"], h["nout"], dt, st_)
             elif k == "conv" and b.get("x2") is not None:
                 x, x2, o = b["x"], b["x2"], b["out"]
-                L.call("rd_conv3x3_bn_act_cat", self.p(x), x.cs, x.co, x.C, self.p(x2), x2.cs, x2.co, x2.cs, A.ptr(b["w"]), A.ptr(b["shift"]),
+                L.call("rd_conv3x3_bn_act_cat", self.p(x), x.cs, x.co, x.C, self.p(x2), x2.cs, x2.co, b["cin2"], A.ptr(b["w"]), A.ptr(b["shift"]),
                        self.p(o), o.cs, o.co, B, x.H, x.W, b["cout"], b["flags"], dt, st_)
             elif k == "conv" and b.get("ex"):
                 x, o, r, sx = b["x"], b["out"], b["res"], b.get("sc_x")
```

After: 997.7 (median of 4 runs). No clear change (+0.2%).
